# introlab/rtabmap

Measured on AMD Instinct MI355X. Metric: loop-closure candidates/sec (49k vocab, 100k signatures, 500 desc/frame), higher is better.
Workload: dtype f32; 1 GPU; SURF-64 fp32 brute-force 2-NN (49k words) + NNDR + TF-IDF likelihood (100000 signatures x 500 words, Zipf), 500 desc/frame, 1 frame/step; world_size_observed=1, collective_backend=none, parallelism=1 GPU, last_frame_top_candidate_ok=True

## Files before the change

include/lcd.h:

```cpp
#ifndef LCD_H_
#define LCD_H_

#include <stddef.h>
#include <stdint.h>

#ifdef __cplusplus
extern "C" {
#endif

#define LCD_ABI_VERSION 7

typedef struct lcd_engine lcd_engine;

enum lcd_status {
    LCD_OK = 0,
    LCD_ERR_INVALID = 1,
    LCD_ERR_HIP = 2,
    LCD_ERR_NOMEM = 3,
    LCD_ERR_STATE = 4,
    LCD_ERR_UNSUPPORTED = 5
};

enum lcd_dtype {
    LCD_F32 = 0,
// ... 79 lines not shown
} lcd_hypothesis;

#define LCD_NEW_WORD_IDS_AUTO (-1)
typedef struct lcd_frame_args {
    int32_t struct_size;
    int32_t q;
    const void* d_descriptors;
    int32_t flags;
    float nndr_ratio;
    int32_t sig_id;
    int32_t first_new_word_id;
    float N;
    int32_t exclude_recent;
    int32_t* d_word_ids;
    float* d_likelihood;
    int64_t likelihood_capacity;
    lcd_hypothesis* d_hypothesis;
    float* d_adjusted;
    float virtual_place_ratio;
    int32_t append_new_words;
    int32_t* d_first_new_word_id;
    float* d_posterior;
    struct lcd_bayes_result* d_bayes;
} lcd_frame_args;
int lcd_frame_dev(lcd_engine* h, const lcd_frame_args* args);

typedef struct lcd_frame_host_args {
    int32_t struct_size;
    int32_t q;
    const void* descriptors;
    int32_t flags;
    float nndr_ratio;
    int32_t sig_id;
    int32_t first_new_word_id;
    float N;
    int32_t append_new_words;
    int32_t* word_ids;
    float* likelihood;
    int64_t likelihood_capacity;
    int64_t* n_slots;
} lcd_frame_host_args;
int lcd_frame_host(lcd_engine* h, const lcd_frame_host_args* args);
int lcd_slot_count(const lcd_engine* h, int64_t* n_slots);

typedef struct lcd_bayes_result {
    int32_t sig_id;
    int32_t slot;
    float posterior;
    float value;
    float virtual_place;
    int32_t n_considered;
    float sum;
    int32_t reserved;
} lcd_bayes_result;
int lcd_bayes_configure(lcd_engine* h, const double* prediction_lc, int n_values, float virtual_place_prior);
int lcd_bayes_reset(lcd_engine* h);
int lcd_bayes_set_neighbors(lcd_engine* h, int n_sigs, const int32_t* sig_ids, const int64_t* offsets, const int32_t* nbr_sig_ids,
                            const int32_t* nbr_margins);
int lcd_bayes_update_dev(lcd_engine* h, const float* d_adjusted, int exclude_recent, float* d_posterior, lcd_bayes_result* d_result);
int lcd_bayes_update(lcd_engine* h, const int32_t* sig_ids, const float* adjusted, int n, lcd_bayes_result* result);
int lcd_bayes_posterior(lcd_engine* h, const int32_t* sig_ids, int n, float* out);
int lcd_knn2_dev(lcd_engine* h, const void* d_queries, int q, int32_t* d_word_ids, float* d_dist);
typedef struct lcd_shard_cand { uint64_t key; int32_t word; int32_t wslot; } lcd_shard_cand;
int lcd_shard_knn2_dev(lcd_engine* h, const void* d_descriptors, int q, lcd_shard_cand* d_cand );
int lcd_shard_frame_dev(lcd_engine* h, const void* d_descriptors, int q, int flags, float nndr_ratio, int32_t sig_id,
                        int32_t first_new_word_id , float N,
                        int rank, int world, const lcd_shard_cand* d_all_cand ,
                        int64_t total_live_rows, int32_t* d_word_ids, int64_t* d_lfix, int64_t lfix_capacity);
int lcd_finalize_dev(lcd_engine* h, int64_t* d_lfix, int64_t n, float* d_likelihood);
int lcd_slots_dev(lcd_engine* h, const int32_t** d_slot_sig, int64_t* n_slots);
int lcd_record_event(lcd_engine* h, void* event);
void* lcd_stream(lcd_engine* h);

int lcd_profile_begin(lcd_engine* h, int max_samples);
int lcd_profile_read(lcd_engine* h, float* avg_ms, int* n_samples, const char** kernel_name);
int lcd_profile_read_likelihood(lcd_engine* h, float* avg_ms, int* n_samples, const char** kernel_name);

int lcd_set_option(lcd_engine* h, const char* key, int64_t value);

int lcd_trace_push(lcd_engine* h, const char* name);
int lcd_trace_pop(lcd_engine* h);

int lcd_profile_score_work(lcd_engine* h, int64_t* out8);

typedef struct lcd_stats {
    int64_t vocab_rows, vocab_live;
    int64_t signatures, postings;
    int64_t knn_launches, likelihood_launches, rebuilds;
    int64_t buckets_sealed;
    int64_t word_slots;
    int64_t dense_words;
    int64_t frame_calls, frame_host_ns;
    int64_t bytes_device;
    int64_t knn_last_fallback_queries;
    double knn_max_err_ratio;
    int64_t clean_divergent_refs;
} lcd_stats;
int lcd_get_stats(lcd_engine* h, lcd_stats* out);

#ifdef __cplusplus
}
#endif
#endif
```

rtabmap_amd/capi.py:

```python
import ctypes as C
import os
import sys

import numpy as np

from . import build as _build

LCD_OK = 0
LCD_F32, LCD_U8 = 0, 1
LCD_Q_INCREMENTAL, LCD_Q_NEW_WORDS_COMPARED = 1, 2
LCD_NEW_WORD_IDS_AUTO = -1
STATUS = {0: "LCD_OK", 1: "LCD_ERR_INVALID", 2: "LCD_ERR_HIP", 3: "LCD_ERR_NOMEM", 4: "LCD_ERR_STATE", 5: "LCD_ERR_UNSUPPORTED"}

SYMBOLS = [
    "lcd_abi_version", "lcd_create", "lcd_destroy", "lcd_last_error", "lcd_synchronize", "lcd_pipeline_depth",
    "lcd_vocab_clear", "lcd_vocab_append", "lcd_vocab_remove", "lcd_vocab_remove_unused", "lcd_vocab_remove_unused_async", "lcd_vocab_rebuild", "lcd_vocab_count", "lcd_vocab_read",
    "lcd_knn2", "lcd_selfdist", "lcd_quantize", "lcd_find_nn",
    "lcd_sig_add", "lcd_sig_remove", "lcd_sig_add_bulk", "lcd_sig_count", "lcd_word_nrefs",
    "lcd_likelihood", "lcd_adjust_likelihood", "lcd_adjust_likelihood_dev", "lcd_frame_dev", "lcd_frame_host", "lcd_slot_count", "lcd_knn2_dev", "lcd_shard_knn2_dev", "lcd_shard_frame_dev", "lcd_finalize_dev", "lcd_slots_dev", "lcd_stream", "lcd_get_stats", "lcd_profile_begin", "lcd_profile_read", "lcd_profile_read_likelihood", "lcd_profile_score_work", "lcd_set_option", "lcd_record_event", "lcd_trace_push", "lcd_trace_pop",
    "lcd_bayes_configure", "lcd_bayes_reset", "lcd_bayes_set_neighbors", "lcd_bayes_update_dev", "lcd_bayes_update", "lcd_bayes_posterior",
]


LCD_KNN_DEFAULT, LCD_KNN_EXACT_VALU, LCD_KNN_F32_MFMA, LCD_KNN_BF16X3, LCD_KNN_F16 = 0, 1, 2, 3, 4
KNN_MODES = {None: 0, "default": 0, "valu": 1, "exact": 1, "mfma32": 2, "f32": 2, "bf16": 3, "bf16x3": 3, "f16": 4, "fp16": 4}


class LcdConfig(C.Structure):
    _fields_ = [("struct_size", C.c_int32), ("device", C.c_int32), ("dtype", C.c_int32), ("dim", C.c_int32),
                ("vocab_capacity", C.c_int64), ("sig_capacity", C.c_int64), ("max_queries", C.c_int32),
                ("knn_mode", C.c_int32), ("stream", C.c_void_p), ("pipeline", C.c_int32), ("reserved1", C.c_int32)]


class LcdHypothesis(C.Structure):
    _fields_ = [("sig_id", C.c_int32), ("slot", C.c_int32), ("likelihood", C.c_float), ("adjusted", C.c_float),
                ("virtual_place", C.c_float), ("mean", C.c_float), ("stddev", C.c_float), ("n_positive", C.c_int32)]


class LcdFrameArgs(C.Structure):
    _fields_ = [("struct_size", C.c_int32), ("q", C.c_int32), ("d_descriptors", C.c_void_p), ("flags", C.c_int32),
                ("nndr_ratio", C.c_float), ("sig_id", C.c_int32), ("first_new_word_id", C.c_int32), ("N", C.c_float),
                ("exclude_recent", C.c_int32), ("d_word_ids", C.c_void_p), ("d_likelihood", C.c_void_p),
                ("likelihood_capacity", C.c_int64), ("d_hypothesis", C.c_void_p), ("d_adjusted", C.c_void_p),
                ("virtual_place_ratio", C.c_float), ("append_new_words", C.c_int32), ("d_first_new_word_id", C.c_void_p),
                ("d_posterior", C.c_void_p), ("d_bayes", C.c_void_p)]


class LcdFrameHostArgs(C.Structure):
    _fields_ = [("struct_size", C.c_int32), ("q", C.c_int32), ("descriptors", C.c_void_p), ("flags", C.c_int32), ("nndr_ratio", C.c_float),
                ("sig_id", C.c_int32), ("first_new_word_id", C.c_int32), ("N", C.c_float), ("append_new_words", C.c_int32),
                ("word_ids", C.c_void_p), ("likelihood", C.c_void_p), ("likelihood_capacity", C.c_int64), ("n_slots", C.c_void_p)]


class LcdBayesResult(C.Structure):
    _fields_ = [("sig_id", C.c_int32), ("slot", C.c_int32), ("posterior", C.c_float), ("value", C.c_float),
                ("virtual_place", C.c_float), ("n_considered", C.c_int32), ("sum", C.c_float), ("reserved", C.c_int32)]


class LcdStats(C.Structure):
    _fields_ = [("vocab_rows", C.c_int64), ("vocab_live", C.c_int64), ("signatures", C.c_int64), ("postings", C.c_int64),
                ("knn_launches", C.c_int64), ("likelihood_launches", C.c_int64), ("rebuilds", C.c_int64),
                ("buckets_sealed", C.c_int64), ("word_slots", C.c_int64), ("dense_words", C.c_int64),
                ("frame_calls", C.c_int64), ("frame_host_ns", C.c_int64),
                ("bytes_device", C.c_int64), ("knn_last_fallback_queries", C.c_int64), ("knn_max_err_ratio", C.c_double),
                ("clean_divergent_refs", C.c_int64)]


class LcdError(RuntimeError):
    def __init__(self, status, msg):
        super().__init__("%s: %s" % (STATUS.get(status, status), msg))
        self.status = status


_lib = None


def library_path():
    return _build.OUT


def load():
    global _lib
    if _lib is not None:
        return _lib
    path = os.environ.get("LCD_LIB_PATH") or _build.build()
    if "torch" not in sys.modules and not os.environ.get("LCD_NO_TORCH_PRELOAD"):
        try:
            import torch
        except Exception:
            pass
    L = C.CDLL(path)
    vp, i32, i64, f32 = C.c_void_p, C.c_int32, C.c_int64, C.c_float
    L.lcd_abi_version.restype = C.c_int
    L.lcd_create.argtypes = [C.POINTER(LcdConfig), C.POINTER(vp)]
    L.lcd_destroy.argtypes = [vp]
    L.lcd_destroy.restype = None
    L.lcd_last_error.argtypes = [vp]
    L.lcd_last_error.restype = C.c_char_p
    L.lcd_synchronize.argtypes = [vp]
    L.lcd_pipeline_depth.argtypes = [vp]
    L.lcd_pipeline_depth.restype = C.c_int
    L.lcd_vocab_clear.argtypes = [vp]
    L.lcd_vocab_append.argtypes = [vp, vp, C.c_int, vp]
    L.lcd_vocab_remove.argtypes = [vp, vp, C.c_int]
    L.lcd_vocab_remove_unused.argtypes = [vp, vp, C.c_int, vp]
    L.lcd_vocab_remove_unused_async.argtypes = [vp]
    L.lcd_vocab_rebuild.argtypes = [vp]
    L.lcd_vocab_count.argtypes = [vp, C.POINTER(i64), C.POINTER(i64)]
    L.lcd_vocab_read.argtypes = [vp, i64, C.c_int, vp, vp]
    L.lcd_knn2.argtypes = [vp, vp, C.c_int, vp, vp]
    L.lcd_selfdist.argtypes = [vp, vp, C.c_int, vp]
    L.lcd_quantize.argtypes = [vp, vp, C.c_int, C.c_int, f32, vp, C.POINTER(i32)]
    L.lcd_find_nn.argtypes = [vp, vp, C.c_int, vp, vp, C.c_int, C.c_int, f32, vp]
    L.lcd_sig_add.argtypes = [vp, i32, vp, C.c_int, i32]
    L.lcd_sig_remove.argtypes = [vp, i32]
    L.lcd_sig_add_bulk.argtypes = [vp, C.c_int, vp, vp, vp, vp]
    L.lcd_sig_count.argtypes = [vp, C.POINTER(i64), C.POINTER(i64)]
    L.lcd_word_nrefs.argtypes = [vp, i32, C.POINTER(i32)]
    L.lcd_likelihood.argtypes = [vp, vp, C.c_int, vp, C.c_int, f32, vp]
    L.lcd_adjust_likelihood.argtypes = [vp, vp, C.c_int, f32]
    L.lcd_adjust_likelihood_dev.argtypes = [vp, vp, C.c_int, f32]
    L.lcd_frame_dev.argtypes = [vp, C.POINTER(LcdFrameArgs)]
    L.lcd_frame_host.argtypes = [vp, C.POINTER(LcdFrameHostArgs)]
    L.lcd_slot_count.argtypes = [vp, C.POINTER(C.c_int64)]
    L.lcd_knn2_dev.argtypes = [vp, vp, C.c_int, vp, vp]
    L.lcd_shard_knn2_dev.argtypes = [vp, vp, C.c_int, vp]
    L.lcd_shard_frame_dev.argtypes = [vp, vp, C.c_int, C.c_int, f32, i32, i32, f32, C.c_int, C.c_int, vp, i64, vp, vp, i64]
    L.lcd_finalize_dev.argtypes = [vp, vp, i64, vp]
    L.lcd_slots_dev.argtypes = [vp, C.POINTER(vp), C.POINTER(i64)]
    L.lcd_stream.argtypes = [vp]
    L.lcd_stream.restype = vp
    L.lcd_profile_begin.argtypes = [vp, C.c_int]
    L.lcd_profile_read.argtypes = [vp, C.POINTER(f32), C.POINTER(C.c_int), C.POINTER(C.c_char_p)]
    L.lcd_profile_read_likelihood.argtypes = [vp, C.POINTER(f32), C.POINTER(C.c_int), C.POINTER(C.c_char_p)]
    L.lcd_get_stats.argtypes = [vp, C.POINTER(LcdStats)]
    L.lcd_profile_score_work.argtypes = [vp, C.POINTER(i64)]
    L.lcd_set_option.argtypes = [vp, C.c_char_p, i64]
    L.lcd_record_event.argtypes = [vp, vp]
    L.lcd_bayes_configure.argtypes = [vp, vp, C.c_int, f32]
    L.lcd_bayes_reset.argtypes = [vp]
    L.lcd_bayes_set_neighbors.argtypes = [vp, C.c_int, vp, vp, vp, vp]
    L.lcd_bayes_update_dev.argtypes = [vp, vp, C.c_int, vp, vp]
    L.lcd_bayes_update.argtypes = [vp, vp, vp, C.c_int, vp]
    L.lcd_bayes_posterior.argtypes = [vp, vp, C.c_int, vp]
    _lib = L
    return L


def _p(a):
    return None if a is None else a.ctypes.data_as(C.c_void_p)


class Engine:

    def __init__(self, dtype, dim, device=0, vocab_capacity=0, sig_capacity=0, stream=None, knn_mode=None, pipeline=False):
        self.L = load()
        self.dtype = LCD_F32 if dtype in (LCD_F32, np.float32, "f32") else LCD_U8
        self.np_dtype = np.float32 if self.dtype == LCD_F32 else np.uint8
        self.dim = int(dim)
        if knn_mode is None:
            knn_mode = os.environ.get("LCD_PY_KNN_MODE") or None
        mode = KNN_MODES[knn_mode] if (knn_mode is None or isinstance(knn_mode, str)) else int(knn_mode)
        cfg = LcdConfig(C.sizeof(LcdConfig), device, self.dtype, self.dim, vocab_capacity, sig_capacity, 0, mode, stream,
                        1 if pipeline else 0, 0)
        h = C.c_void_p()
        rc = self.L.lcd_create(C.byref(cfg), C.byref(h))
        if rc != LCD_OK:
            raise LcdError(rc, "lcd_create failed (no gfx950 device / HIP runtime?)")
        self.h = h
        for kv in filter(None, os.environ.get("LCD_PY_OPTS", "").split(",")):
            self._ck(self.L.lcd_set_option(self.h, kv.split("=")[0].encode(), int(kv.split("=")[1])))

    def close(self):
        if getattr(self, "h", None):
            self.L.lcd_destroy(self.h)
            self.h = None

    def __del__(self):
        try:
            self.close()
        except Exception:
            pass

    def _ck(self, rc):
        if rc != LCD_OK:
            raise LcdError(rc, self.L.lcd_last_error(self.h).decode())

    def _rows(self, a):
        a = np.ascontiguousarray(a, dtype=self.np_dtype)
        if a.ndim != 2 or a.shape[1] != self.dim:
            raise ValueError("expected [n, %d] %s" % (self.dim, self.np_dtype.__name__))
        return a

    def synchronize(self):
        self._ck(self.L.lcd_synchronize(self.h))

    def pipeline_depth(self):
        return int(self.L.lcd_pipeline_depth(self.h))

    def vocab_clear(self):
        self._ck(self.L.lcd_vocab_clear(self.h))

    def vocab_append(self, rows, word_ids):
        rows = self._rows(rows)
        ids = np.ascontiguousarray(word_ids, dtype=np.int32)
        assert ids.shape[0] == rows.shape[0]
        self._ck(self.L.lcd_vocab_append(self.h, _p(rows), rows.shape[0], _p(ids)))

    def vocab_remove(self, word_ids):
        ids = np.ascontiguousarray(word_ids, dtype=np.int32)
        self._ck(self.L.lcd_vocab_remove(self.h, _p(ids), ids.shape[0]))

    def vocab_remove_unused(self, capacity=0):
        out = np.zeros(max(capacity, 1), np.int32)
        n = C.c_int32()
        self._ck(self.L.lcd_vocab_remove_unused(self.h, _p(out) if capacity else None, capacity, C.byref(n)))
        return n.value, out[: min(n.value, capacity)]

    def vocab_remove_unused_async(self):
# ... 134 lines not shown
        s = np.ascontiguousarray(sig_ids, dtype=np.int32)
        o = np.ascontiguousarray(offsets, dtype=np.int64)
        n = np.ascontiguousarray(nbr_sig_ids, dtype=np.int32)
        m = np.ascontiguousarray(nbr_margins, dtype=np.int32)
        assert o.shape[0] == s.shape[0] + 1 and n.shape[0] == m.shape[0]
        self._ck(self.L.lcd_bayes_set_neighbors(self.h, s.shape[0], _p(s), _p(o), _p(n), _p(m)))

    def bayes_neighbors_prepared(self, sig_ids, offsets, nbr_sig_ids, nbr_margins):
        assert sig_ids.dtype == np.int32 and offsets.dtype == np.int64 and nbr_sig_ids.dtype == np.int32 and nbr_margins.dtype == np.int32
        assert offsets.shape[0] == sig_ids.shape[0] + 1 and nbr_sig_ids.shape[0] == nbr_margins.shape[0]
        return (sig_ids.shape[0], _p(sig_ids), _p(offsets), _p(nbr_sig_ids), _p(nbr_margins), (sig_ids, offsets, nbr_sig_ids, nbr_margins))

    def bayes_set_neighbors_prepared(self, prep):
        rc = self.L.lcd_bayes_set_neighbors(self.h, prep[0], prep[1], prep[2], prep[3], prep[4])
        if rc != LCD_OK:
            self._ck(rc)

    def bayes_update_dev(self, d_adjusted_ptr, exclude_recent=0, d_posterior_ptr=None, d_result_ptr=None):
        self._ck(self.L.lcd_bayes_update_dev(self.h, d_adjusted_ptr, exclude_recent, d_posterior_ptr, d_result_ptr))

    def bayes_update(self, sig_ids, adjusted):
        s = np.ascontiguousarray(sig_ids, dtype=np.int32)
        a = np.ascontiguousarray(adjusted, dtype=np.float32)
        assert s.shape[0] == a.shape[0]
        r = LcdBayesResult()
        self._ck(self.L.lcd_bayes_update(self.h, _p(s), _p(a), s.shape[0], C.byref(r)))
        return r

    def bayes_posterior(self, sig_ids):
        s = np.ascontiguousarray(sig_ids, dtype=np.int32)
        out = np.zeros(s.shape[0], np.float32)
        self._ck(self.L.lcd_bayes_posterior(self.h, _p(s), s.shape[0], _p(out)))
        return out

    def knn2_dev(self, d_queries_ptr, q, d_word_ids_ptr, d_dist_ptr):
        self._ck(self.L.lcd_knn2_dev(self.h, d_queries_ptr, q, d_word_ids_ptr, d_dist_ptr))

    def shard_knn2_dev(self, d_desc_ptr, q, d_cand_ptr):
        self._ck(self.L.lcd_shard_knn2_dev(self.h, d_desc_ptr, q, d_cand_ptr))

    def shard_frame_dev(self, d_desc_ptr, q, sig_id, N, rank, world, d_all_cand_ptr, total_live_rows, d_word_ids_ptr, d_lfix_ptr,
                        lfix_capacity, incremental=True, new_words_compared=True, nndr=0.8, first_new_word_id=0):
        flags = (LCD_Q_INCREMENTAL if incremental else 0) | (LCD_Q_NEW_WORDS_COMPARED if new_words_compared else 0)
        self._ck(self.L.lcd_shard_frame_dev(self.h, d_desc_ptr, q, flags, nndr, sig_id, first_new_word_id, float(N), rank, world,
                                            d_all_cand_ptr, total_live_rows, d_word_ids_ptr, d_lfix_ptr, lfix_capacity))

    def finalize_dev(self, d_lfix_ptr, n, d_like_ptr):
        self._ck(self.L.lcd_finalize_dev(self.h, d_lfix_ptr, n, d_like_ptr))

    def slots_dev(self):
        p, n = C.c_void_p(), C.c_int64()
        self._ck(self.L.lcd_slots_dev(self.h, C.byref(p), C.byref(n)))
        return p.value, n.value

    def stream(self):
        return self.L.lcd_stream(self.h)

    def profile_begin(self, max_samples):
        self._ck(self.L.lcd_profile_begin(self.h, max_samples))

    def profile_read(self):
        ms, n, name = C.c_float(), C.c_int(), C.c_char_p()
        self._ck(self.L.lcd_profile_read(self.h, C.byref(ms), C.byref(n), C.byref(name)))
        return ms.value, n.value, (name.value or b"").decode()

    def profile_read_likelihood(self):
        ms, n, name = C.c_float(), C.c_int(), C.c_char_p()
        self._ck(self.L.lcd_profile_read_likelihood(self.h, C.byref(ms), C.byref(n), C.byref(name)))
        return ms.value, n.value, (name.value or b"").decode()

    def record_event(self, event_handle):
        self._ck(self.L.lcd_record_event(self.h, event_handle))

    def set_option(self, key, value):
        self._ck(self.L.lcd_set_option(self.h, key.encode(), int(value)))

    def profile_score_work(self):
        out = (C.c_int64 * 8)()
        self._ck(self.L.lcd_profile_score_work(self.h, out))
        keys = ["dense_row_bytes", "sparse_postings", "directory_lookups", "directory_hits", "open_log_entries", "postings",
                "unique_words", "dense_words"]
        return {k: int(v) for k, v in zip(keys, out)}

    def stats(self):
        s = LcdStats()
        self._ck(self.L.lcd_get_stats(self.h, C.byref(s)))
        return {k: getattr(s, k) for k, _ in LcdStats._fields_}
```

rtabmap_amd/csrc/engine.hip:

```cpp
#include "engine_impl.h"
#include <dlfcn.h>

#include <algorithm>
#include <chrono>
#include <cmath>
#include <cstdlib>
#include <cstring>
#include <new>
#include <numeric>
#include <unordered_map>

using namespace lcd;

static_assert(sizeof(lcd::HypothesisOut) == sizeof(lcd_hypothesis), "lcd_hypothesis is the kernel's output record");

int RowMirror::find(int32_t word_id) {
    if (rows_sorted) {
        auto it = std::lower_bound(h_row_key.begin(), h_row_key.end(), word_id);
        if (it == h_row_key.end() || *it != word_id) return -1;
        const int r = (int)(it - h_row_key.begin());
        return h_row_live[r] ? r : -1;
    }
    if (!word_row_valid) {
        word_row.clear();
// ... 1226 lines not shown
    if (n > h->tfidf.n_slots) return h->fail(LCD_ERR_INVALID, "lcd_finalize_dev: more entries than signature slots");
    LCD_HIP(h, h->tfidf.finalize((const long long*)d_lfix, (long long)n, d_likelihood));
    return LCD_OK;
    LCD_CATCH(h)
}

int lcd_slots_dev(lcd_engine* h, const int32_t** d_slot_sig, int64_t* n_slots) {
    LCD_TRY
    LCD_CHECK_HANDLE(h);
    { int rc = drain_keep_rows_lazy(h); if (rc) return rc; }
    if (d_slot_sig) *d_slot_sig = h->tfidf.slot_sig.as<int32_t>();
    if (n_slots) *n_slots = h->tfidf.n_slots;
    return LCD_OK;
    LCD_CATCH(h)
}

int lcd_profile_begin(lcd_engine* h, int max_samples) {
    LCD_TRY
    LCD_CHECK_HANDLE(h);
    LCD_DEV(h);
    if (max_samples <= 0 || max_samples > (1 << 20)) return h->fail(LCD_ERR_INVALID, "lcd_profile_begin: bad sample count");
    while ((int)h->prof_ev.size() < 2 * max_samples) {
        hipEvent_t e;
        LCD_HIP(h, hipEventCreate(&e));
        h->prof_ev.push_back(e);
        LCD_HIP(h, hipEventCreate(&e));
        h->prof_ev.push_back(e);
        LCD_HIP(h, hipEventCreate(&e));
        h->prof2_ev.push_back(e);
        LCD_HIP(h, hipEventCreate(&e));
        h->prof2_ev.push_back(e);
    }
    h->prof_n = 0;
    h->prof2_n = 0;
    h->prof_cap = max_samples;
    return LCD_OK;
    LCD_CATCH(h)
}

int lcd_profile_read(lcd_engine* h, float* avg_ms, int* n_samples, const char** kernel_name) {
    LCD_TRY
    LCD_CHECK_HANDLE(h);
    LCD_DEV(h);
    { int rc = h->sync_all(); if (rc) return rc; }
    double sum = 0.0;
    for (int i = 0; i < h->prof_n; ++i) {
        float ms = 0.0f;
        LCD_HIP(h, hipEventElapsedTime(&ms, h->prof_ev[2 * i], h->prof_ev[2 * i + 1]));
        sum += ms;
    }
    if (avg_ms) *avg_ms = h->prof_n ? (float)(sum / h->prof_n) : 0.0f;
    if (n_samples) *n_samples = h->prof_n;
    if (kernel_name) *kernel_name = h->prof_kernel;
    h->prof_cap = 0;
    return LCD_OK;
    LCD_CATCH(h)
}

int lcd_profile_read_likelihood(lcd_engine* h, float* avg_ms, int* n_samples, const char** kernel_name) {
    LCD_TRY
    LCD_CHECK_HANDLE(h);
    LCD_DEV(h);
    { int rc = h->sync_all(); if (rc) return rc; }
    double sum = 0.0;
    for (int i = 0; i < h->prof2_n; ++i) {
        float ms = 0.0f;
        LCD_HIP(h, hipEventElapsedTime(&ms, h->prof2_ev[2 * i], h->prof2_ev[2 * i + 1]));
        sum += ms;
    }
    if (avg_ms) *avg_ms = h->prof2_n ? (float)(sum / h->prof2_n) : 0.0f;
    if (n_samples) *n_samples = h->prof2_n;
    if (kernel_name) *kernel_name = h->prof2_kernel;
    h->prof_cap = 0;
    return LCD_OK;
    LCD_CATCH(h)
}

int lcd_set_option(lcd_engine* h, const char* key, int64_t value) {
    LCD_TRY
    LCD_CHECK_HANDLE(h);
    { int rc = h->drain(); if (rc) return rc; }
    if (!key) return h->fail(LCD_ERR_INVALID, "lcd_set_option: null key");
    if (!std::strcmp(key, "score_block") && (value == 256 || value == 512 || value == 1024)) { h->tfidf.score_block = (int)value; return LCD_OK; }
    if (!std::strcmp(key, "filter_units") && value >= -1 && value <= 4096) { h->filter_units = (int)value; return LCD_OK; }
    if (!std::strcmp(key, "strip_tiles") && value >= 0 && value <= 8) { h->strip_tiles = (int)value; return LCD_OK; }
    if (!std::strcmp(key, "shard_growth_first") && value >= 0 && value < (1ll << 28)) { h->shard_first = (int32_t)value; return LCD_OK; }
    if (!std::strcmp(key, "shard_growth_block") && value >= 0 && value <= (1 << 20)) { h->shard_block = (int32_t)value; return LCD_OK; }
    if (!std::strcmp(key, "shard_append") && (value == 0 || value == 1)) { h->shard_append = (int)value; return LCD_OK; }
    if (!std::strcmp(key, "profile_likelihood") && (value == 0 || value == 1)) { h->prof_likelihood = value != 0; return LCD_OK; }
    if (!std::strcmp(key, "append_split_buckets") && value >= -1 && value <= (1 << 24)) { h->popt.append_split_buckets = (int)value; return LCD_OK; }
    if (!std::strcmp(key, "cross_frame_tiles") && value >= -1 && value <= 1) { h->popt.cross_frames = value > 0 ? 1 : 0; return LCD_OK; }
    if (!std::strcmp(key, "append_from_rerank") && value >= -1 && value <= 1) { h->popt.append_from_rerank = value != 0 ? 1 : 0; return LCD_OK; }
    if (!std::strcmp(key, "roctx") && (value == 0 || value == 1)) {
        if (!value) { h->roctx_push = nullptr; h->roctx_pop = nullptr; return LCD_OK; }
        static void* lib = nullptr;
        if (!lib) lib = dlopen("libroctx64.so", RTLD_NOW | RTLD_GLOBAL);
        if (!lib) lib = dlopen("libroctx64.so.4", RTLD_NOW | RTLD_GLOBAL);
        if (!lib) lib = dlopen("/opt/rocm/lib/libroctx64.so", RTLD_NOW | RTLD_GLOBAL);
        if (!lib) return h->fail(LCD_ERR_UNSUPPORTED, "lcd_set_option(roctx): libroctx64.so not found");
        h->roctx_push = reinterpret_cast<int (*)(const char*)>(dlsym(lib, "roctxRangePushA"));
        h->roctx_pop = reinterpret_cast<int (*)()>(dlsym(lib, "roctxRangePop"));
        if (!h->roctx_push || !h->roctx_pop) { h->roctx_push = nullptr; h->roctx_pop = nullptr; return h->fail(LCD_ERR_UNSUPPORTED, "lcd_set_option(roctx): roctxRangePushA / roctxRangePop not exported"); }
        return LCD_OK;
    }
    if (!std::strcmp(key, "filter_delay") && value >= 0 && value <= 127) { h->popt.filter_delay = (int)value; return LCD_OK; }
    if (!std::strcmp(key, "shadow_rows") && value >= -1 && value <= 2) { h->popt.shadow_rows = value < 0 ? 1 : (int)value; return LCD_OK; }
    if (!std::strcmp(key, "mirror_from_b") && value >= -1 && value <= 1) { h->popt.mirror_from_b = value != 0 ? 1 : 0; return LCD_OK; }
    if (!std::strcmp(key, "next_word_id") && value >= 1 && value < (1ll << 28)) { h->mirror.next_word_id = std::max(h->mirror.next_word_id, (int32_t)value); return LCD_OK; }
    if (!std::strcmp(key, "profile_skip") && value >= 0 && value <= (1 << 20)) { h->prof_skip = (int)value; return LCD_OK; }
    if (!std::strcmp(key, "decision_straight") && value >= -1 && value <= 2) { h->popt.decision_straight = value >= 0 ? (int)value : PipeOpts().decision_straight; return LCD_OK; }
    if (!std::strcmp(key, "slots_from_rows") && value >= -1 && value <= 2) { h->popt.slots_from_rows = value >= 0 ? (int)value : PipeOpts().slots_from_rows; return LCD_OK; }
    if (!std::strcmp(key, "row_writer_wgs") && value >= -1 && value <= 256) { h->popt.row_writer_wgs = value >= 0 ? (int)value : PipeOpts().row_writer_wgs; return LCD_OK; }
    return h->fail(LCD_ERR_INVALID, "lcd_set_option: unknown key or value");
    LCD_CATCH(h)
}

int lcd_trace_push(lcd_engine* h, const char* name) {
    if (!h || !name) return LCD_ERR_INVALID;
    if (h->roctx_push) h->roctx_push(name);
    return LCD_OK;
}
int lcd_trace_pop(lcd_engine* h) {
    if (!h) return LCD_ERR_INVALID;
    if (h->roctx_pop) h->roctx_pop();
    return LCD_OK;
}

int lcd_profile_score_work(lcd_engine* h, int64_t* out8) {
    LCD_TRY
    LCD_CHECK_HANDLE(h);
    LCD_DEV(h);
    if (!out8) return h->fail(LCD_ERR_INVALID, "lcd_profile_score_work: null output");
    { int rc = h->sync_all(); if (rc) return rc; }
    LCD_HIP(h, h->tfidf.score_work(out8));
    return LCD_OK;
    LCD_CATCH(h)
}

int lcd_get_stats(lcd_engine* h, lcd_stats* out) {
    LCD_TRY
    LCD_CHECK_HANDLE(h);
    if (!out) return LCD_ERR_INVALID;
    LCD_DEV(h);
    { int rc = h->sync_all(); if (rc) return rc; }
    out->knn_last_fallback_queries = 0;
    out->knn_max_err_ratio = 0.0;
    const void* fc = h->last_fail_count ? h->last_fail_count : h->d_fail_count.p;
    if (fc) {
        int32_t n[3] = {0, 0, 0};
        int rc = download(h, n, fc, 12, h->h_out2);
        if (rc) return rc;
        out->knn_last_fallback_queries = n[0];
        float r;
        std::memcpy(&r, &n[2], 4);
        out->knn_max_err_ratio = r;
    }
    out->vocab_rows = h->n_rows; out->vocab_live = h->n_live;
    out->signatures = h->tfidf.live_sigs; out->postings = h->tfidf.postings_ub;
    out->knn_launches = h->knn_launches; out->likelihood_launches = h->likelihood_launches; out->rebuilds = h->rebuilds;
    h->tfidf.harvest_released(false);
    out->frame_calls = h->frame_calls; out->frame_host_ns = h->frame_host_ns;
    out->buckets_sealed = h->tfidf.seals;
    out->word_slots = (int64_t)h->tfidf.n_wslots - h->tfidf.ws_free_count;
    out->dense_words = h->tfidf.h_n_dense ? (int64_t)*(volatile uint32_t*)h->tfidf.h_n_dense : 0;
    out->bytes_device = h->bytes_device;
    out->clean_divergent_refs = 0;
    if (h->tfidf.q_meta.p) {
        uint32_t n = 0;
        int rc = download(h, &n, h->tfidf.q_meta.as<uint32_t>() + 8, 4, h->h_out2);
        if (rc) return rc;
        out->clean_divergent_refs = (int64_t)n;
    }
    return LCD_OK;
    LCD_CATCH(h)
}

}
```

rtabmap_amd/csrc/knn_mfma_kernels.hip:

```cpp
#include <hip/hip_ext.h>
#include "lcd_kernels.h"
#include "rowpar_body.cuh"
#include "shard_body.cuh"
#include "frame_tail_body.cuh"
#include "score_body.cuh"

#include <cstdlib>

namespace lcd {
namespace {

typedef float f32x16 __attribute__((ext_vector_type(16)));
constexpr int MF_BLOCK = 256;
constexpr int MF_WAVES = 4;
constexpr int MF_KEEP = 4;

__global__ void row_norm_kernel(const float* __restrict__ vocab, const int32_t* __restrict__ row_id, int first, int n, int dim,
                                float* __restrict__ aug, uint32_t* __restrict__ norm_max_bits) {
    const int r = first + blockIdx.x * blockDim.x + threadIdx.x;
    if (r >= first + n) return;
    float s = __int_as_float(0x7f800000);
    if (row_id[r] != 0) {
        s = 0.0f;
        const float* v = vocab + (size_t)r * dim;
// ... 1666 lines not shown
constexpr int PIPE_BLOCK = 256;

struct TailRoles { int has_resolve, has_register, n_redo, n_filter_wgs, n_q_wgs, n_sh_wgs; };
#ifdef LCD_B_TIMING
__device__ unsigned long long g_a_timing[2 * 4096];
#define A_STAMP(i) do { __builtin_amdgcn_s_barrier(); if (threadIdx.x == 0 && blockIdx.x < 4096) g_a_timing[2 * blockIdx.x + (i)] = __builtin_amdgcn_s_memrealtime(); } while (0)
#else
#define A_STAMP(i) do { } while (0)
#endif
template <bool PERSISTENT, int M>
__device__ __forceinline__ void frame_a_body(float* s_dyn, const FilterArgs& f, int px, const TailRoles& tr, const ResolveArgs& r, const FwArgs& a,
                                             const RetireArgs& ret, const QSplitArgs& qs) {
    const int bid = (int)blockIdx.x;
    const int n_front = tr.has_resolve + tr.has_register;
    A_STAMP(0);
    if (bid < tr.has_resolve) { frame_resolve_part<PIPE_BLOCK>((uint32_t*)s_dyn, r, 0, 1 + tr.n_redo); A_STAMP(1); return; }
    if (bid < n_front) { frame_register_part<PIPE_BLOCK>((uint32_t*)s_dyn, a, ret); A_STAMP(1); return; }
    const int after_strips = n_front + tr.n_filter_wgs;
    if (bid >= after_strips && bid < after_strips + tr.n_sh_wgs) {
        if constexpr (!PERSISTENT) shadow_scores_body<M>(s_dyn, bid - after_strips, f.sh_bf, f.sh_norm, f.sh_rows, f.qsplit, f.qnorm, f.nq, f.qpad, f.sh_x, f.sh_ld);
        A_STAMP(1);
        return;
    }
    const int after_filter = after_strips + tr.n_sh_wgs;
    if (bid >= after_filter && bid < after_filter + tr.n_q_wgs) { qsplit_body(qs, bid - after_filter); A_STAMP(1); return; }
    if (bid >= after_filter + tr.n_q_wgs) { frame_resolve_part<PIPE_BLOCK>((uint32_t*)s_dyn, r, bid - after_filter - tr.n_q_wgs + 1, 1 + tr.n_redo); A_STAMP(1); return; }
    for (int i = 0; i < f.delay; ++i) __builtin_amdgcn_s_sleep(1);
    if constexpr (PERSISTENT)
        knn_bf16_filter_body_p<M>(s_dyn, bid - n_front, f.vocab_bf, f.row_norm, f.n_rows, f.queries, f.nq, f.qpad, f.tiles_per_block, f.n_blocks, px, f.pk,
                               f.pl, f.sd, f.n_lo);
    else
        knn_bf16_filter_body_q<M>(s_dyn, bid - n_front, f.vocab_bf, f.row_norm, f.n_rows, f.qsplit, f.qnorm, f.nq, f.qpad, f.tiles_per_block, f.n_blocks, f.pk,
                               f.pl, f.sd, f.n_lo);
    A_STAMP(1);
}
template <int M>
__global__ __launch_bounds__(PIPE_BLOCK, 2) void frame_a_kernel(FilterArgs f, TailRoles tr, ResolveArgs r, FwArgs a, RetireArgs ret, QSplitArgs qs) {
    extern __shared__ __attribute__((aligned(16))) float s_dyn_a[];
    frame_a_body<false, M>(s_dyn_a, f, 0, tr, r, a, ret, qs);
}
template <int M>
__global__ __launch_bounds__(PIPE_BLOCK) void frame_a_kernel_p(FilterArgs f, int px, TailRoles tr, ResolveArgs r, FwArgs a, RetireArgs ret, QSplitArgs qs) {
    extern __shared__ __attribute__((aligned(16))) float s_dyn_ap[];
    frame_a_body<true, M>(s_dyn_ap, f, px, tr, r, a, ret, qs);
}
#ifdef LCD_B_TIMING
__device__ unsigned long long g_b_timing[2 * 4096];
#define B_STAMP(i) do { __builtin_amdgcn_s_barrier(); if (threadIdx.x == 0 && blockIdx.x < 4096) g_b_timing[2 * blockIdx.x + (i)] = __builtin_amdgcn_s_memrealtime(); } while (0)
#else
#define B_STAMP(i) do { } while (0)
#endif
constexpr int PIPE_B_BLOCK = 512;
constexpr uint32_t PIPE_B_STAGE_ROWS = 160;
constexpr int APPEND_SPLIT_BUCKETS = 1024;
static_assert(PIPE_B_BLOCK == 2 * MF_BLOCK, "the re-rank halves");
template <bool WITH_APPEND>
__global__ __launch_bounds__(PIPE_B_BLOCK, 6) void frame_b_kernel(RerankArgs k, int n_rerank_wgs, ScoreArgs A, int n_score_wgs, AppendRowsArgs app, int n_wr) {
    int bid = (int)blockIdx.x;
    B_STAMP(0);
    const bool rows_only = !WITH_APPEND && n_wr > 0 && bid >= n_rerank_wgs && bid < n_rerank_wgs + n_wr;
    const int wr_index = bid - n_rerank_wgs;
    if (!WITH_APPEND && n_wr > 0 && bid >= n_rerank_wgs + n_wr) bid -= n_wr;
    if (WITH_APPEND && bid >= n_rerank_wgs + n_score_wgs) {
        extern __shared__ __attribute__((aligned(16))) float s_dyn_b2[];
        append_rows_body<PIPE_B_BLOCK>(app, bid - n_rerank_wgs - n_score_wgs, app.ap.lds_bytes >= 1024 ? s_dyn_b2 : nullptr, (app.ap.lds_bytes / 256) & ~3);
        B_STAMP(1);
        return;
    }
    if (bid < n_rerank_wgs || rows_only) {
        const int pair = rows_only ? 0 : (bid & 7) * (n_rerank_wgs >> 3) + (bid >> 3);
        if (2 * pair >= k.nq) return;
        extern __shared__ __attribute__((aligned(16))) float s_dyn_b[];
        const bool wr_any = !WITH_APPEND && app.ap.enabled && app.ap.defer_rows;
        knn_mfma_rerank_body<64, BF_KEEP, false, true, 2>(2 * pair, k.pk, k.pl, k.n_blocks, k.nq, k.vocab, k.queries, k.row_id, k.norm_max_bits, k.out_row,
                                                          k.out_word, k.out_dist, k.fail_list, k.fail_count, k.cb, k.n_lo, k.n_hi, k.plan_rows,
                                                          s_dyn_b, k.stage_rows, k.f16, k.pend_desc, k.pend_list, k.pend_first_id, k.cross, k.cross_ld
                                                          , app, wr_any && (n_wr == 0 || rows_only), rows_only ? wr_index : pair, n_wr > 0 ? n_wr : (k.nq + 1) / 2
                                                          , rows_only, k.sh_mask, k.sh_q, k.sh_x, k.sh_ld);
        B_STAMP(1);
        return;
    }
    const int g = bid - n_rerank_wgs;
    if (g < A.n_closed_pad) {
        const int b = (g & 7) * (A.n_closed_pad >> 3) + (g >> 3);
        if (b < A.n_closed) score_sealed_body<PIPE_B_BLOCK>(A, b);
    } else score_open_body<PIPE_B_BLOCK>(A, g - A.n_closed_pad);
    B_STAMP(1);
}

__global__ __launch_bounds__(PIPE_B_BLOCK) void append_rows_kernel(AppendRowsArgs app) {
    extern __shared__ __attribute__((aligned(16))) float s_dyn_ar[];
    append_rows_body<PIPE_B_BLOCK>(app, (int)blockIdx.x, app.ap.lds_bytes >= 1024 ? s_dyn_ar : nullptr, (app.ap.lds_bytes / 256) & ~3);
}

__global__ __launch_bounds__(MF_BLOCK) void knn_rowpar_kernel(RowparArgs a, int32_t* __restrict__ fail_count) {
    rowpar_body<64, MF_BLOCK>(a, (int)blockIdx.x, (int)gridDim.x, fail_count);
}
__global__ __launch_bounds__(256) void shard_merge_bits_kernel(ShardMergeJob mj, CandBits cb) {
    const int lane = threadIdx.x & 63;
    const int qi = (int)blockIdx.x * 4 + (int)(threadIdx.x >> 6);
    if (qi >= cb.nq) return;
    const ShardMerged m = shard_merge_one(mj.cand, mj.world, mj.rank, cb.nq, qi, mj.by_word);
    const bool v0 = m.dist[0] >= 0.0f && m.word[0] != 0, v1 = m.dist[1] >= 0.0f && m.word[1] != 0;
    const float thr = (cb.have_index && v0 && v1) ? m.dist[1] : __int_as_float(0x7f800000);
    if (lane == 0) {
#pragma unroll
        for (int j = 0; j < 2; ++j) { mj.out_word[2 * qi + j] = m.word[j]; mj.out_dist[2 * qi + j] = m.dist[j]; mj.out_wslot[2 * qi + j] = m.wslot[j]; }
    }
    cand_bits_row(cb, qi, thr, lane, 64);
}
__global__ __launch_bounds__(MF_BLOCK) void knn_rowpar_pack_kernel(RowparArgs a, int32_t* __restrict__ fail_count, ShardPackArgs p) {
    const int st = rowpar_body<64, MF_BLOCK>(a, (int)blockIdx.x, (int)gridDim.x, fail_count);
    if (st == 0) {
        for (int i = (int)blockIdx.x * MF_BLOCK + (int)threadIdx.x; i < p.q2; i += (int)gridDim.x * MF_BLOCK) shard_pack_one(p, i);
    } else if (st == 2) {
        asm volatile("s_waitcnt vmcnt(0)" ::: "memory");
        __syncthreads();
        __builtin_amdgcn_fence(__ATOMIC_ACQUIRE, "agent");
        for (int i = (int)threadIdx.x; i < p.q2; i += MF_BLOCK) shard_pack_one(p, i);
        if (threadIdx.x < 4 && threadIdx.x != 2) fail_count[threadIdx.x] = 0;
    }
}

}
}
#ifdef LCD_B_TIMING
extern "C" int lcd_debug_a_timing(unsigned long long* out, int n_words) {
    if (hipDeviceSynchronize() != hipSuccess) return -1;
    return (int)hipMemcpyFromSymbol(out, HIP_SYMBOL(lcd::g_a_timing), (size_t)n_words * 8);
}
extern "C" int lcd_debug_rr_timing(unsigned long long* out, int n_words) {
    if (hipDeviceSynchronize() != hipSuccess) return -1;
    return (int)hipMemcpyFromSymbol(out, HIP_SYMBOL(lcd::g_rr_timing), (size_t)n_words * 8);
}
extern "C" int lcd_debug_b_timing(unsigned long long* out, int n_words) {
    if (hipDeviceSynchronize() != hipSuccess) return -1;
    return (int)hipMemcpyFromSymbol(out, HIP_SYMBOL(lcd::g_b_timing), (size_t)n_words * 8);
}
#endif
#ifdef LCD_MFMA_TIMING
extern "C" int lcd_debug_mfma_timing(unsigned long long* out, int n_words) {
    if (hipDeviceSynchronize() != hipSuccess) return -1;
    return (int)hipMemcpyFromSymbol(out, HIP_SYMBOL(lcd::g_mf_timing), (size_t)n_words * 8);
}
extern "C" int lcd_debug_mfma_timing2(unsigned long long* out, int n_words) {
    if (hipDeviceSynchronize() != hipSuccess) return -1;
    return (int)hipMemcpyFromSymbol(out, HIP_SYMBOL(lcd::g_mf_timing2), (size_t)n_words * 8);
}
#endif
namespace lcd {

bool knn_mfma_supported(int dtype, int dim) { return dtype == 0 && dim == 64; }

static int mfma_ng() {
    return 4;
}

MfmaPlan knn_mfma_plan(int q, int n_rows) {
    MfmaPlan p;
    p.q = q;
    p.qpad = (q + 63) / 64 * 64;
    p.n_rows = n_rows;
    const int n_tiles = (n_rows + 31) / 32;
    const int qw = mfma_ng() * 32;
    const int qgroups = (q + qw - 1) / qw;
    int nb = ((mfma_ng() == 2 ? 512 : 256) + qgroups - 1) / qgroups;
    if (nb > (n_tiles + MF_WAVES - 1) / MF_WAVES) nb = (n_tiles + MF_WAVES - 1) / MF_WAVES;
    if (nb < 1) nb = 1;
// ... 234 lines not shown
    MfmaPlan p;
    p.q = 0; p.qpad = 0; p.n_rows = 0; p.tiles_per_block = 1; p.n_blocks = 0;
    if (kp) {
        const PipeKnn& k = *kp;
        p = k.plan;
        uint64_t* pk = (uint64_t*)k.partial;
        uint32_t* pl = (uint32_t*)(pk + (size_t)(p.n_blocks > 0 ? p.n_blocks : 1) * BF_KEEP * p.qpad);
        if (p.n_shadow > 0 && k.sh_bf && k.sh_norm && k.sh_rows > 0 && k.sh_x) { f.sh_bf = (const float*)k.sh_bf; f.sh_norm = k.sh_norm; f.sh_rows = k.sh_rows; f.sh_x = k.sh_x; f.sh_ld = k.sh_ld; }
        f.vocab_bf = (const float*)k.vocab_bf; f.row_norm = k.row_norm; f.n_rows = p.n_rows; f.queries = (const float*)k.queries; f.nq = p.q; f.qpad = p.qpad;
        f.tiles_per_block = p.tiles_per_block; f.n_blocks = p.n_blocks; f.pk = pk; f.pl = pl; f.n_lo = k.n_lo;
        f.qsplit = (const uint4*)k.qsplit; f.qnorm = k.qnorm;
        if (k.cb.selfdist) {
            f.sd.queries = (const float*)k.queries; f.sd.nq = p.q; f.sd.out = const_cast<float*>(k.cb.selfdist); f.sd.ld = k.cb.ld; f.sd.n_tiles = f.sd.n_self = selfdist_tiles(p.q);
        }
        if (opt.cross_frames && k.cross && k.cross_cols && k.cross_ncols > 0 && p.q > 0) {
            f.sd.queries = (const float*)k.queries; f.sd.nq = p.q;
            f.sd.other = (const float*)k.cross_cols; f.sd.n_other = k.cross_ncols; f.sd.xout = k.cross; f.sd.xld = k.cross_ld;
            f.sd.n_tiles += ((p.q + 63) / 64) * ((k.cross_ncols + 63) / 64);
        }
    }
    f.delay = opt.filter_delay;
    const int px = p.q > 0 ? bf16_persistent_px(p) : 0;
    if (px == 0 && p.q > 0 && (!f.qsplit || !f.qnorm)) return hipErrorInvalidValue;
    if (p.n_shadow > 0 && (px > 0 || !f.sh_x)) return hipErrorInvalidValue;
    TailRoles tr;
    tr.n_filter_wgs = p.q > 0 ? f.sd.n_tiles + (px > 0 ? px : p.n_blocks) * ((p.q + BF_QB - 1) / BF_QB) : 0;
    tr.n_sh_wgs = (p.q > 0 && p.n_shadow > 0) ? ((f.sh_rows + 31) / 32) * ((p.q + BF_QB - 1) / BF_QB) : 0;
    tr.has_resolve = resolve ? 1 : 0; tr.has_register = reg ? 1 : 0; tr.n_redo = resolve ? resolve->n_redo : 0;
    QSplitArgs qs{};
    if (qsp) { qs = *qsp; qs.n_wgs = std::min((qs.qpad * 8 + PIPE_BLOCK - 1) / PIPE_BLOCK, 32); if (qs.n_wgs < 1) qs.n_wgs = 1; }
    tr.n_q_wgs = qsp ? qs.n_wgs : 0;
    const int grid = tr.n_filter_wgs + tr.n_sh_wgs + tr.has_resolve + tr.has_register + tr.n_redo + tr.n_q_wgs;
    if (grid == 0) return hipSuccess;
    const size_t lds = px > 0 ? BF_LDS_BYTES_P : BF_LDS_BYTES_Q;
    if ((resolve && resolve->shmem_resolve > lds) || (reg && reg->shmem + (size_t)reg->a.n * 4 > lds)) return hipErrorInvalidValue;
    ResolveArgs r{}; FwArgs a{}; RetireArgs ret{};
    if (resolve) { r = resolve->r; r.ap.lds_bytes = (int)lds; }
    if (reg) { a = reg->a; ret = reg->ret; }
    const bool timed = ev_begin != nullptr && ev_end != nullptr;
    const bool f16 = kp ? p.f16 != 0 : opt.f16 != 0;
    if (px > 0) {
        static const hipError_t attrp0 = hipFuncSetAttribute(reinterpret_cast<const void*>(&frame_a_kernel_p<0>),
                                                             hipFuncAttributeMaxDynamicSharedMemorySize, (int)BF_LDS_BYTES_P);
        static const hipError_t attrp1 = hipFuncSetAttribute(reinterpret_cast<const void*>(&frame_a_kernel_p<1>),
                                                             hipFuncAttributeMaxDynamicSharedMemorySize, (int)BF_LDS_BYTES_P);
        (void)attrp0; (void)attrp1;
        if (f16) {
            if (timed) hipExtLaunchKernelGGL(frame_a_kernel_p<1>, dim3(grid), dim3(PIPE_BLOCK), (uint32_t)BF_LDS_BYTES_P, s, ev_begin, ev_end, 0u, f, px, tr, r, a, ret, qs);
            else frame_a_kernel_p<1><<<grid, PIPE_BLOCK, BF_LDS_BYTES_P, s>>>(f, px, tr, r, a, ret, qs);
        } else {
            if (timed) hipExtLaunchKernelGGL(frame_a_kernel_p<0>, dim3(grid), dim3(PIPE_BLOCK), (uint32_t)BF_LDS_BYTES_P, s, ev_begin, ev_end, 0u, f, px, tr, r, a, ret, qs);
            else frame_a_kernel_p<0><<<grid, PIPE_BLOCK, BF_LDS_BYTES_P, s>>>(f, px, tr, r, a, ret, qs);
        }
    } else if (f16) {
        if (timed) hipExtLaunchKernelGGL(frame_a_kernel<1>, dim3(grid), dim3(PIPE_BLOCK), (uint32_t)BF_LDS_BYTES_Q, s, ev_begin, ev_end, 0u, f, tr, r, a, ret, qs);
        else frame_a_kernel<1><<<grid, PIPE_BLOCK, BF_LDS_BYTES_Q, s>>>(f, tr, r, a, ret, qs);
    } else {
        if (timed) hipExtLaunchKernelGGL(frame_a_kernel<0>, dim3(grid), dim3(PIPE_BLOCK), (uint32_t)BF_LDS_BYTES_Q, s, ev_begin, ev_end, 0u, f, tr, r, a, ret, qs);
        else frame_a_kernel<0><<<grid, PIPE_BLOCK, BF_LDS_BYTES_Q, s>>>(f, tr, r, a, ret, qs);
    }
    return hipGetLastError();
}


hipError_t launch_frame_b(const PipeKnn* k, const ScoreArgs* score, int score_wgs, hipStream_t s, hipEvent_t ev_begin, hipEvent_t ev_end,
                          const AppendRowsArgs* app, const PipeOpts& opt) {
    RerankArgs rk{};
    int n_rerank = 0;
    if (k) {
        const MfmaPlan& p = k->plan;
        uint64_t* pk = (uint64_t*)k->partial;
        rk.pk = pk; rk.pl = (uint32_t*)(pk + (size_t)(p.n_blocks > 0 ? p.n_blocks : 1) * BF_KEEP * p.qpad);
        rk.n_blocks = p.n_blocks; rk.nq = p.q; rk.vocab = (const float*)k->vocab; rk.queries = (const float*)k->queries; rk.row_id = k->row_id;
        rk.norm_max_bits = k->norm_max_bits; rk.out_row = k->out_row; rk.out_word = k->out_word; rk.out_dist = k->out_dist;
        rk.fail_list = k->fail_list; rk.fail_count = k->fail_count; rk.cb = k->cb; rk.n_lo = k->n_lo; rk.n_hi = k->n_hi; rk.plan_rows = p.n_rows; rk.f16 = p.f16;
        n_rerank = ((p.q + 1) / 2 + 7) & ~7;
    }
    ScoreArgs A{};
    if (score) A = *score; else score_wgs = 0;
    AppendRowsArgs ar{};
    int n_app = 0;
    if (app && app->ap.enabled && app->ap.defer_rows) { ar = *app; n_app = ar.n_wgs = APPEND_ROW_WGS; }
    if (n_rerank + score_wgs + n_app == 0) return hipSuccess;
    const uint32_t dyn = ((k && k->n_hi) || n_app) ? PIPE_B_STAGE_ROWS * 256u + 512u : 0u;
    rk.stage_rows = (dyn && k && k->n_hi) ? (int)PIPE_B_STAGE_ROWS : 0;
    ar.ap.lds_bytes = (int)(PIPE_B_STAGE_ROWS * 256u);
    if (k && n_app) { rk.pend_desc = ar.ap.descriptors; rk.pend_list = ar.ap.list_out; rk.pend_first_id = ar.ap.first_id; }
    if (k && n_app && opt.cross_frames && k->cross && k->cross_cols == (const void*)ar.ap.descriptors) { rk.cross = k->cross; rk.cross_ld = k->cross_ld; }
    const bool writers = opt.append_from_rerank == 0;
    if (!writers && k && n_app > 0 && k->n_hi && k->plan.q > 0 && rk.stage_rows >= 4) n_app = 0;
    const bool shadow = k && k->plan.n_shadow > 0 && k->sh_mask && k->sh_x && k->sh_q > 0 && app && app->ap.enabled && app->ap.defer_rows && rk.pend_desc && !rk.cross;
    if (k && k->plan.n_shadow > 0 && !shadow) return hipErrorInvalidValue;
    if (shadow) { rk.sh_mask = k->sh_mask; rk.sh_q = k->sh_q; rk.sh_x = k->sh_x; rk.sh_ld = k->sh_ld; }
    const int n_wr = (!writers && n_app == 0 && k && app && app->ap.enabled && app->ap.defer_rows && k->n_hi && k->plan.q > 0 && rk.stage_rows >= 4 && !rk.cross &&
                      (opt.row_writer_wgs > 0 || shadow)) ? (opt.row_writer_wgs > 0 ? opt.row_writer_wgs : 16) : 0;
    if (shadow && n_wr == 0) return hipErrorInvalidValue;
    const bool split = n_app > 0 && score && score->n_closed >= (opt.append_split_buckets >= 0 ? opt.append_split_buckets : APPEND_SPLIT_BUCKETS);
    if (split || n_app == 0) {
        if (n_rerank + score_wgs > 0) {
            if (ev_begin != nullptr && ev_end != nullptr)
                hipExtLaunchKernelGGL(frame_b_kernel<false>, dim3(n_rerank + n_wr + score_wgs), dim3(PIPE_B_BLOCK), dyn, s, ev_begin, ev_end, 0u, rk, n_rerank, A, score_wgs, ar, n_wr);
            else frame_b_kernel<false><<<n_rerank + n_wr + score_wgs, PIPE_B_BLOCK, dyn, s>>>(rk, n_rerank, A, score_wgs, ar, n_wr);
        }
        if (n_app > 0) append_rows_kernel<<<n_app, PIPE_B_BLOCK, PIPE_B_STAGE_ROWS * 256u, s>>>(ar);
        return hipGetLastError();
    }
    if (ev_begin != nullptr && ev_end != nullptr)
        hipExtLaunchKernelGGL(frame_b_kernel<true>, dim3(n_rerank + score_wgs + n_app), dim3(PIPE_B_BLOCK), dyn, s, ev_begin, ev_end, 0u, rk, n_rerank, A, score_wgs, ar, 0);
    else frame_b_kernel<true><<<n_rerank + score_wgs + n_app, PIPE_B_BLOCK, dyn, s>>>(rk, n_rerank, A, score_wgs, ar, 0);
    return hipGetLastError();
}

}

extern "C" int lcd_debug_frame_plan(int q, int n_rows, int new_words_compared, int* out) {
    if (q <= 0 || n_rows <= 0 || !out) return -1;
    const int tiles = new_words_compared ? lcd::knn_selfdist_wgs(q) : 0;
    const lcd::MfmaPlan p = lcd::knn_bf16_plan_pipelined(q, n_rows, tiles, -1);
    out[0] = p.tiles_per_block; out[1] = p.n_blocks; out[2] = lcd::bf16_persistent_px(p); out[3] = tiles; out[4] = (q + lcd::BF_QB - 1) / lcd::BF_QB;
    return 0;
}

#ifdef LCD_SCORE_TIMING
extern "C" int lcd_debug_score_timing_pipe(unsigned long long* out, int n_words) {
    if (hipDeviceSynchronize() != hipSuccess) return -1;
    return (int)hipMemcpyFromSymbol(out, HIP_SYMBOL(lcd::g_score_timing), (size_t)n_words * 8);
}
#endif

#ifdef LCD_TAIL_TIMING
extern "C" int lcd_debug_tail_timing_pipe(unsigned long long* out) {
    if (hipDeviceSynchronize() != hipSuccess) return -1;
    if (hipMemcpyFromSymbol(out, HIP_SYMBOL(lcd::g_tail_timing), 64) != hipSuccess) return -2;
    if (hipMemcpyFromSymbol(out + 8, HIP_SYMBOL(lcd::g_resolve_timing), 64) != hipSuccess) return -3;
    return (int)hipMemcpyFromSymbol(out + 16, HIP_SYMBOL(lcd::g_sweep_timing), 256);
}
#endif
```

rtabmap_amd/csrc/score_body.cuh:

```cuda
#pragma once
#include "frame_tail_body.cuh"

namespace lcd {
namespace {

#ifdef LCD_SCORE_TIMING
__device__ unsigned long long g_score_timing[1024 * 8];
#define SC_STAMP(i) do { __syncthreads(); if (threadIdx.x == 0 && blockIdx.x < 1024) g_score_timing[blockIdx.x * 8 + (i)] = __builtin_amdgcn_s_memrealtime(); } while (0)
#else
#define SC_STAMP(i) do { } while (0)
#endif



template <int SCB>
__device__ __forceinline__ void score_segments(const uint32_t* __restrict__ sp_ent, unsigned long long* acc, uint32_t start, uint32_t len, int32_t idf) {
    const int ln = threadIdx.x & 63;
    uint32_t incl = len;
#pragma unroll
    for (int off = 1; off < 64; off <<= 1) { const uint32_t y = __shfl_up(incl, off, 64); if (ln >= off) incl += y; }
    const uint32_t Tw = __shfl(incl, 63, 64);
    for (uint32_t t0 = 0; t0 < Tw; t0 += 128) {
        uint32_t e[2]; int32_t f[2]; bool ok[2];
#pragma unroll
        for (int u = 0; u < 2; ++u) {
            const uint32_t t = t0 + (uint32_t)(u * 64 + ln);
            int pos = 0;
#pragma unroll
            for (int step = 32; step >= 1; step >>= 1) { const uint32_t v = __shfl(incl, pos + step - 1, 64); if (v <= t) pos += step; }
            if (pos > 63) pos = 63;
            const uint32_t i_o = __shfl(incl, pos, 64), l_o = __shfl(len, pos, 64), s_o = __shfl(start, pos, 64);
            f[u] = __shfl(idf, pos, 64);
            ok[u] = t < Tw;
            e[u] = ok[u] ? gload(sp_ent + s_o + (t - (i_o - l_o))) : 0u;
        }
#pragma unroll
        for (int u = 0; u < 2; ++u) {
            if (!ok[u]) continue;
            const long long term = (long long)(int)(e[u] & TF_CNT_MASK) * (long long)f[u];
            atomicAdd(&acc[e[u] >> TF_CNT_BITS], (unsigned long long)term);
        }
    }
}

template <int SCB>
__device__ __forceinline__ void score_sealed_body(const ScoreArgs& A, int b) {
    __shared__ unsigned long long acc[TF_R];
    const int tid = threadIdx.x;
    const BucketDev B = A.tab[b];
    const long long first_slot = (long long)b * TF_R;
    const bool live = B.state == 1u;
    SC_STAMP(0);
    constexpr int NWV = SCB / 64;
#ifndef LCD_SCORE_DR4
#define LCD_SCORE_DR4 16
#endif
    constexpr int DR = NWV == 4 ? LCD_SCORE_DR4 : (128 / NWV > 16 ? 16 : 128 / NWV);
    constexpr int KW = SCB >= 512 ? 1 : 512 / SCB;
    constexpr int NI = TF_R / SCB > 0 ? TF_R / SCB : 1;
    const int wv = __builtin_amdgcn_readfirstlane(tid >> 6), ln = tid & 63;
    const uint32_t D = live ? A.bkt_D[b] : 0u;
    const uint32_t BW = live ? B.W : 0u;
    const uint32_t flags = A.bkt_flags[b];
    const int U = (int)A.q_meta[0];
    const int Ud = (int)A.q_meta[1];
    static_assert(KW * SCB <= TF_MAX_WORDS && DR * NWV <= TF_MAX_WORDS, "the unconditional list reads stay inside the buffers");
    uint32_t w[KW]; int32_t idf[KW], did[KW]; bool look[KW];
#pragma unroll
    for (int u = 0; u < KW; ++u) {
        const int k = tid + u * SCB;
        w[u] = A.q_w[k]; idf[u] = A.q_idf[k]; did[u] = A.q_did[k];
    }
    int32_t dj[DR], fj[DR];
#pragma unroll
    for (int u = 0; u < DR; ++u) {
        const int j = wv + u * NWV;
        dj[u] = A.qd_did[j];
        fj[u] = A.qd_idf[j];
    }
#pragma unroll
    for (int u = 0; u < KW; ++u) { if (tid + u * SCB >= U) { w[u] = 0; idf[u] = 0; did[u] = -1; } }
#pragma unroll
    for (int u = 0; u < DR; ++u) { if (wv + u * NWV >= Ud) { dj[u] = -1; fj[u] = 0; } }
    uint32_t ni_v[NI];
#pragma unroll
    for (int u = 0; u < NI; ++u) { const int i = tid + u * SCB; ni_v[u] = i < TF_R ? A.slot_ni[first_slot + i] : 0u; }
    uint4 r0[KW], r1[KW];
#pragma unroll
    for (int u = 0; u < KW; ++u) {
        const bool dense_here = did[u] >= 0 && (uint32_t)did[u] < D;
        look[u] = idf[u] != 0 && w[u] < BW && (!dense_here || (flags & 1u));
        r0[u] = make_uint4(0u, 0u, 0u, 0u); r1[u] = r0[u];
        if (look[u]) {
            const uint4* rec = reinterpret_cast<const uint4*>(A.dir2 + ((size_t)(w[u] >> 5) * A.dir2_stride + (uint32_t)b) * TF_DIR2_DWORDS);
            r0[u] = gload4(rec); r1[u] = gload4(rec + 1);
        }
    }
    uint32_t c[DR];
#pragma unroll
    for (int u = 0; u < DR; ++u) c[u] = (dj[u] >= 0 && (uint32_t)dj[u] < D) ? gload((const uint32_t*)(B.dense + (size_t)dj[u] * TF_R + 4 * ln)) : 0u;
    uint32_t start[KW], len[KW];
#pragma unroll
    for (int u = 0; u < KW; ++u) {
        start[u] = 0; len[u] = 0;
        if (!look[u]) continue;
        const uint32_t f[6] = {r0[u].z, r0[u].w, r1[u].x, r1[u].y, r1[u].z, r1[u].w};
        const uint32_t p = w[u] & 31u, pd = p / 6u, ps = 5u * (p % 6u);
        if (!(r0[u].y & TF_DIR2_SAT)) {
            uint32_t before = 0;
#pragma unroll
            for (uint32_t d = 0; d < 6u; ++d) {
                const uint32_t x = d < pd ? f[d] : (d == pd ? (f[d] & ((1u << ps) - 1u)) : 0u);
                before += dir2_sum6(x);
            }
            uint32_t fd = f[0];
#pragma unroll
            for (uint32_t d = 1; d < 6u; ++d) fd = d == pd ? f[d] : fd;
            len[u] = (fd >> ps) & 31u;
            start[u] = r0[u].x + before;
        } else {
            const uint2 blk = gload2(B.dirb + (w[u] >> 5));
            const uint32_t bit = 1u << p;
            if (blk.x & bit) {
                const uint32_t r = blk.y + (uint32_t)__popc(blk.x & (bit - 1u));
                const uint32_t s0 = gload(B.sp_off + r), s1 = gload(B.sp_off + r + 1);
                start[u] = s0; len[u] = s1 - s0;
            }
        }
    }
    long long a0 = 0, a1 = 0, a2 = 0, a3 = 0;
#pragma unroll
    for (int u = 0; u < DR; ++u) {
        const long long f64 = (long long)fj[u];
        a0 += (long long)(int)(c[u] & 255u) * f64;
        a1 += (long long)(int)((c[u] >> 8) & 255u) * f64;
        a2 += (long long)(int)((c[u] >> 16) & 255u) * f64;
        a3 += (long long)(int)(c[u] >> 24) * f64;
    }
    for (int j0 = wv + DR * NWV; j0 < Ud; j0 += DR * NWV) {
#pragma unroll
        for (int u = 0; u < DR; ++u) {
            const int j = j0 + u * NWV;
            dj[u] = j < Ud ? A.qd_did[j] : -1;
            fj[u] = j < Ud ? A.qd_idf[j] : 0;
        }
#pragma unroll
        for (int u = 0; u < DR; ++u) c[u] = (dj[u] >= 0 && (uint32_t)dj[u] < D) ? gload((const uint32_t*)(B.dense + (size_t)dj[u] * TF_R + 4 * ln)) : 0u;
#pragma unroll
        for (int u = 0; u < DR; ++u) {
            const long long f64 = (long long)fj[u];
            a0 += (long long)(int)(c[u] & 255u) * f64;
            a1 += (long long)(int)((c[u] >> 8) & 255u) * f64;
            a2 += (long long)(int)((c[u] >> 16) & 255u) * f64;
            a3 += (long long)(int)(c[u] >> 24) * f64;
        }
    }
    for (int i = tid; i < TF_R; i += SCB) acc[i] = 0ull;
    __syncthreads();
    SC_STAMP(1);
    {
        const int ln4 = ln * 4;
        if (a0) atomicAdd(&acc[ln4 + 0], (unsigned long long)a0);
        if (a1) atomicAdd(&acc[ln4 + 1], (unsigned long long)a1);
        if (a2) atomicAdd(&acc[ln4 + 2], (unsigned long long)a2);
        if (a3) atomicAdd(&acc[ln4 + 3], (unsigned long long)a3);
    }
    SC_STAMP(2);
#pragma unroll
    for (int u = 0; u < KW; ++u) score_segments<SCB>(B.sp_ent, acc, start[u], len[u], idf[u]);
    for (int k0 = KW * SCB; k0 < U; k0 += SCB) {
        const int k = k0 + tid;
        uint32_t st2 = 0, ln2 = 0; int32_t idf2 = 0;
        if (k < U) {
            const uint32_t w2 = A.q_w[k];
            idf2 = A.q_idf[k];
            const int32_t d2 = A.q_did[k];
            const bool dh = d2 >= 0 && (uint32_t)d2 < D;
            if (idf2 != 0 && w2 < BW && (!dh || (flags & 1u))) {
                const uint2 bk = gload2(B.dirb + (w2 >> 5));
                const uint32_t bit = 1u << (w2 & 31);
                if (bk.x & bit) {
                    const uint32_t r = bk.y + (uint32_t)__popc(bk.x & (bit - 1u));
                    st2 = gload(B.sp_off + r);
                    ln2 = gload(B.sp_off + r + 1) - st2;
                }
            }
        }
        score_segments<SCB>(B.sp_ent, acc, st2, ln2, idf2);
    }
    __syncthreads();
    SC_STAMP(3);
#pragma unroll
    for (int u = 0; u < NI; ++u) {
        const int i = tid + u * SCB;
        if (i >= TF_R) continue;
        const long long v = (long long)acc[i];
        if (A.out_like) A.out_like[first_slot + i] = fixed_to_like(v, ni_v[u]);
        else A.out_fix[first_slot + i] = ni_v[u] ? v : 0;
    }
}

template <int SCB>
__device__ __forceinline__ void score_open_body(const ScoreArgs& A, int ob) {
    const int wv = threadIdx.x >> 6, ln = threadIdx.x & 63;
    const int sl = ob * (SCB / 64) + wv;
    if (sl >= A.n_open_slots) return;
    const BucketDev B = A.tab[A.n_closed];
    const long long slot = (long long)A.n_closed * TF_R + sl;
    const uint32_t begin = A.slot_begin[slot], cnt = A.slot_cnt[slot], ni = A.slot_ni[slot];
    long long acc = 0;
    if (ni != 0u) {
        for (uint32_t e0 = 0; e0 < cnt; e0 += 4 * 64) {
            uint32_t w[4], pc[4]; uint2 t[4];
#pragma unroll
            for (int u = 0; u < 4; ++u) {
                const uint32_t e = e0 + u * 64 + ln;
                w[u] = e < cnt ? gload(B.coo_w + begin + e) : 0xFFFFFFFFu;
                pc[u] = e < cnt ? gload(B.coo_pc + begin + e) : 0u;
            }
#pragma unroll
            for (int u = 0; u < 4; ++u) t[u] = A.idf_tab[w[u] != 0xFFFFFFFFu ? w[u] : 0u];
#pragma unroll
            for (int u = 0; u < 4; ++u)
                if (w[u] != 0xFFFFFFFFu && t[u].x == A.stamp) acc += (long long)(int)(pc[u] & TF_CNT_MASK) * (long long)(int32_t)t[u].y;
        }
    }
    int lo = (int)(uint32_t)acc, hi = (int)(acc >> 32);
#pragma unroll
    for (int off = 32; off > 0; off >>= 1) {
        const int olo = __shfl_xor(lo, off, 64), ohi = __shfl_xor(hi, off, 64);
        const long long s = (((long long)hi << 32) | (uint32_t)lo) + (((long long)ohi << 32) | (uint32_t)olo);
        lo = (int)(uint32_t)s; hi = (int)(s >> 32);
    }
    if (ln == 0) {
        const long long v = ((long long)hi << 32) | (uint32_t)lo;
        if (A.out_like) A.out_like[slot] = fixed_to_like(v, ni);
        else A.out_fix[slot] = ni ? v : 0;
    }
}


}
}
```

rtabmap_amd/csrc/tfidf.h:

```cpp
#pragma once
#include <hip/hip_runtime.h>
#include <stdint.h>
#include <map>
#include <string>
#include <unordered_map>
#include <vector>

#include "bayes.h"
#include "devbuf.h"
#include "lcd_kernels.h"

namespace lcd {

constexpr int TF_R = 256;
constexpr int TF_CNT_BITS = 22;
constexpr uint32_t TF_CNT_MASK = (1u << TF_CNT_BITS) - 1;
constexpr int TF_MAX_WORDS = 8192;
constexpr int TF_IDF_SHIFT = 26;
constexpr int TF_DENSE_T = 32;
constexpr int TF_DENSE_MAX = 4096;
constexpr int TF_DIR2_DWORDS = 8;
constexpr uint32_t TF_DIR2_SAT = 1u << 31;
__host__ __device__ inline uint32_t dir2_sum6(uint32_t x) {
    const uint32_t t = (x & 0x01F07C1Fu) + ((x >> 5) & 0x01F07C1Fu);
    return (t & 0x3FFu) + ((t >> 10) & 0x3FFu) + (t >> 20);
}

struct BucketDev {
    const uint32_t* coo_w;
    const uint32_t* coo_pc;
    const uint8_t* dense;
    const uint2* dirb;
    const uint32_t* sp_off;
    const uint32_t* sp_ent;
    uint32_t W;
    uint32_t D_alloc;
    uint32_t state;
    uint32_t pad;
};

struct SealJob {
    int bucket;
    const uint32_t* coo_w; const uint32_t* coo_pc; const uint32_t* ne;
    uint8_t* dense; uint32_t D_alloc;
    uint2* dirb; uint32_t* sp_off; uint32_t* sp_ent;
    uint32_t* dir2; uint32_t dir2_stride;
    uint32_t* cntw;
    uint32_t* tile_sums;
    uint32_t W;
    uint32_t ent_cap;
};

struct Bucket {
    int state = 0;
    int n_slots = 0;
    int live = 0;
    int64_t ub_entries = 0;
    DevBuf coo_w, coo_pc, sealed;
    size_t off_dirb = 0, off_spoff = 0, off_spent = 0;
    uint32_t W = 0, D_alloc = 0;
};

struct AppendArgs {
    int enabled = 0;
    const float* descriptors = nullptr;
    int row_dwords = 0;
    int is_f32_64 = 0;
    int f16 = 0;
    uint32_t* vocab = nullptr; int32_t* row_id = nullptr; int32_t* row_wslot = nullptr;
    uint32_t* wrow = nullptr;
    float* row_norm = nullptr; uint32_t* norm_max_bits = nullptr; uint32_t* vocab_bf = nullptr;
    const int32_t* cnt_in = nullptr; int32_t* cnt_out = nullptr;
    int32_t* log_slot = nullptr;
    int32_t first_id = 0;
    int32_t* first_out = nullptr;
    long long capacity = 0;
    int lds_bytes = 0;
    int defer_rows = 0;
    uint32_t* list_out = nullptr;
    unsigned long long* host_mirror = nullptr;
    uint32_t tag = 0;
    uint32_t* mask_out = nullptr;
    int mirror_later = 0;
};
struct ShardAppendJob {
    AppendArgs ap; WsRuns new_ws; const int32_t* codes = nullptr; int q = 0, rank = 0, world = 1; int32_t own_first = 0, own_block = 0;
};

struct AppendRowsArgs { AppendArgs ap; WsRuns new_ws; int n_wgs = 0; };
constexpr int APPEND_ROW_WGS = 8;

struct ResolveArgs {
    int q, flags; float nndr; int have_index;
    const int32_t* knn_word; const float* knn_dist; const float* selfdist; int ld; const uint32_t* cand_bits; int bw;
    int32_t* out_word; int32_t* out_n_new; const int32_t* knn_row; const int32_t* row_wslot; int32_t* out_wslot;
    const uint2* cand_list; const int32_t* cand_cnt;
    int straight = 0;
    int slots_are_rows = 0;
    WsRuns new_ws;
    int32_t* fail_count;
    RowparArgs rp;
    AppendArgs ap;
};

struct FwArgs {
    const int32_t* src; int n;
    const int32_t* xlate; long long xlate_n;
    int H; int do_register; int want_q;
    int32_t sig_id; long long slot; uint32_t slot_local; uint32_t ni; float N; uint32_t stamp;
    uint32_t* nw; const int32_t* did;
    uint32_t* coo_w; uint32_t* coo_pc; uint32_t* ne_counter;
    int32_t* slot_sig; uint32_t* slot_ni; uint32_t* slot_begin; uint32_t* slot_cnt;
    uint32_t* q_w; int32_t* q_idf; int32_t* q_did; int32_t* qd_did; int32_t* qd_idf; uint32_t* q_meta; uint2* idf_tab;
    WsRuns new_ws;
    const int32_t* row_wslot;
    const uint32_t* wrow;
};
struct RetireArgs { long long slot[4]; const uint32_t* coo_w[4]; int n; };
struct ScoreArgs {
    const BucketDev* tab; const uint32_t* bkt_D; const uint32_t* bkt_flags;
    const uint32_t* dir2; uint32_t dir2_stride;
    int n_closed;
    int n_closed_pad;
    int n_open_slots; int wcap;
    const uint32_t* q_w; const int32_t* q_idf; const int32_t* q_did; const int32_t* qd_did; const int32_t* qd_idf; const uint32_t* q_meta;
    const uint32_t* slot_ni; const uint32_t* slot_begin; const uint32_t* slot_cnt;
    const uint2* idf_tab; uint32_t stamp;
    float* out_like; long long* out_fix;
};
struct TailLaunch {
    ResolveArgs r; FwArgs a; RetireArgs ret;
    int n_redo = 0;
    size_t shmem = 0;
    size_t shmem_resolve = 0;
};
struct PipeKnn {
    MfmaPlan plan;
    const void* vocab; const void* vocab_bf; const float* row_norm; const uint32_t* norm_max_bits; const int32_t* row_id; const void* queries;
    void* partial; int32_t* out_row; int32_t* out_word; float* out_dist; int32_t* fail_list; int32_t* fail_count;
    CandBits cb;
    const void* qsplit = nullptr;
    const float* qnorm = nullptr;
    const int32_t* n_lo = nullptr;
    const int32_t* n_hi = nullptr;
    const void* sh_bf = nullptr; const float* sh_norm = nullptr; int sh_rows = 0;
    const uint32_t* sh_mask = nullptr; int sh_q = 0;
    float* sh_x = nullptr; int sh_ld = 0;
    float* cross = nullptr;
    int cross_ld = 0;
    const void* cross_cols = nullptr; int cross_ncols = 0;
};
struct QSplitArgs { const float* queries; int nq, qpad; uint4* qsplit; float* qnorm; int n_wgs; int f16 = 0;
                    uint32_t* shadow_bf = nullptr; float* shadow_norm = nullptr;
                    uint32_t* norm_max_bits = nullptr;
};
size_t knn_qsplit_bytes(int q);
int pipe_block_size();
int pipe_b_block_size();
#ifndef LCD_REDO_WGS_MAX
#define LCD_REDO_WGS_MAX 32
#endif
constexpr int REDO_WGS_MAX = LCD_REDO_WGS_MAX;
void resolve_launch_info(const ResolveArgs& r, int block, int* n_redo, size_t* shmem);
struct PipeOpts {
    int f16 = 0;
    int cross_frames = 0;
    int append_from_rerank = 1;
    int append_split_buckets = -1;
    int filter_delay = 0;
    int shadow_rows = 1;
    int mirror_from_b = 1;
    int slots_from_rows = 1;
    int decision_straight = 1;
    int row_writer_wgs = 16;
};
hipError_t launch_frame_a(const PipeKnn* k, const QSplitArgs* qs, const TailLaunch* resolve, const TailLaunch* reg, hipStream_t s,
                          hipEvent_t ev_begin = nullptr, hipEvent_t ev_end = nullptr, const PipeOpts& opt = PipeOpts());
hipError_t launch_frame_b(const PipeKnn* k, const ScoreArgs* score, int score_wgs, hipStream_t s, hipEvent_t ev_begin = nullptr,
                          hipEvent_t ev_end = nullptr, const AppendRowsArgs* app = nullptr, const PipeOpts& opt = PipeOpts());

struct BufPool {
    std::vector<DevBuf> free_list;
    hipError_t get(size_t bytes, DevBuf* out, int64_t* total);
    void put(DevBuf* b);
    void destroy(int64_t* total);
};

struct Tfidf {
    hipStream_t stream = nullptr;
    int64_t* bytes_device = nullptr;
    DevBuf slot_sig, slot_ni, slot_begin, slot_cnt;
    DevBuf nw, did;
    DevBuf wrow;
    DevBuf idf_tab;
    uint32_t stamp = 0;
    std::vector<int32_t> id2ws;
    DevBuf d_id2ws;
    int64_t d_id2ws_n = 0;
    std::vector<int32_t> id2ws_dirty;
    std::map<int32_t, int32_t> ws_free;
    int64_t ws_free_count = 0;
    struct PinBlock { void* p = nullptr; size_t cap = 0; hipEvent_t ev = nullptr; };
    std::vector<PinBlock> pin_free;
    struct ReleaseBatch { std::vector<int32_t> ws, ids; PinBlock blk; const uint8_t* ok = nullptr; bool recheck = false; };
    std::vector<ReleaseBatch> releasing;
    std::vector<int32_t> held_ws, held_ids;
    std::vector<int32_t> ghost_ws;
    uint32_t flushes = 0;
    hipError_t flush_held();
    struct Reservation { int32_t first_id = 0, n = 0; WsRuns runs; } resv;
    DevBuf bkt_tab, bkt_ne, bkt_D, bkt_flags;
    std::vector<Bucket> buckets;
    int score_block = 512;
    int q_n_ub = 0;
    BufPool pool;
    DevBuf dir2;
    uint32_t dir2_blocks = 0, dir2_stride = 0, dir2_hint_blocks = 0, dir2_hint_stride = 0;
    hipError_t ensure_dir2(uint32_t blocks, uint32_t buckets_needed);
    DevBuf n_dense;
    uint32_t* h_n_dense = nullptr;
    DevBuf seal_cntw, seal_tiles;
    DevBuf q_w, q_idf, q_did, qd_did, qd_idf, q_meta;
    DevBuf d_stage;
    DevBuf d_pairs;
    PinBuf h_stage;
    std::unordered_map<int32_t, int64_t> sig_slot;
    int32_t n_wslots = 0;
    int64_t n_slots = 0, live_sigs = 0;
    int64_t postings_ub = 0;
    int64_t seals = 0;
    std::string err;

    hipError_t init(hipStream_t s, int64_t* bytes, int64_t sig_capacity, int64_t vocab_capacity);
    void destroy();
    hipError_t wslot_of(int32_t word_id, bool create, int32_t* out);
    hipError_t sync_id2ws();
    hipError_t release_words(const int32_t* word_ids, int n);
    hipError_t release_wslots(const std::vector<int32_t>& ws, const std::vector<int32_t>* ids = nullptr, bool recheck = false);
    hipError_t rows_take_keys(const int32_t* d_ws, int n, int64_t first_row);
    hipError_t rows_drop_keys(const int32_t* d_row_wslot, const int32_t* d_rows, int n);
    hipError_t rows_clear();
    hipError_t rows_unlog_keys(const int32_t* d_pairs, int n);
    void forget_word(int32_t word_id, int32_t ws);
    void free_wslot(int32_t w);
    void free_wslot_run(int32_t start, int32_t len);
    int32_t take_wslot();
    void harvest_released(bool wait);
    hipError_t reserve_new_words(int32_t first_id, int n, WsRuns* runs, bool may_flush = true);
    void adopt_key(int32_t word_id, int32_t ws);
    hipError_t flush_held_if_due() { return held_ws.size() >= 16384 ? flush_held() : hipSuccess; }
    hipError_t register_dev(int32_t sig_id, const int32_t* d_wslots, int n, int32_t ni, float N, const ResolveArgs* resolve = nullptr,
                            bool ids_given = false , TailLaunch* defer = nullptr,
                            const WsRuns* new_ws = nullptr, const ShardAppendJob* shard_app = nullptr);
    hipError_t query_dev(const int32_t* d_wslots, int n, float N, const ResolveArgs* resolve = nullptr, bool ids_given = false,
                         TailLaunch* defer = nullptr, const WsRuns* new_ws = nullptr, const ShardAppendJob* shard_app = nullptr);
    hipError_t register_bulk(int n_sigs, const int32_t* sig_ids, const int64_t* offsets, const int32_t* ni, const int32_t* d_ids,
                             int64_t total_ids, int max_n);
    hipError_t flush_retire();
    std::vector<int64_t> pending_retire;
    hipEvent_t prof_b = nullptr, prof_e = nullptr;
    hipError_t score(float* d_likelihood);
    hipError_t score_work(int64_t out[8]);
    hipError_t score_fix(long long* lfix);
    hipError_t finalize(const long long* lfix_src, long long n, float* d_likelihood);
    hipError_t retire(int32_t sig_id);
    hipError_t seal_batch(const std::vector<int>& bucket_ids, bool bulk);
    hipError_t ensure_slots(int64_t n);
    hipError_t ensure_wslots(int32_t n);
    hipError_t ensure_buckets(int n);
    hipError_t set_bucket(int b);
    hipError_t new_bucket();
    hipError_t launch_score(float* d_likelihood, long long* lfix);
    hipError_t score_args(float* d_likelihood, long long* lfix, int block, ScoreArgs* out, int* n_wgs);
};

hipError_t launch_gather_f32(const float* dense, const int64_t* slots, int n, float* out, hipStream_t s);
hipError_t launch_shard_append(const AppendArgs& ap, const WsRuns& new_ws, const int32_t* codes, int q, int rank, int world, int32_t own_first,
                               int32_t own_block, hipStream_t s);


}
```

rtabmap_amd/csrc/tfidf.hip:

```cpp
#include "tfidf.h"
#include "frame_tail_body.cuh"
#include "score_body.cuh"

#include <algorithm>
#include <cmath>
#include <cstdlib>
#include <cstring>
#include <iterator>

namespace lcd {
namespace {

#ifndef LCD_FW_BLOCK
#define LCD_FW_BLOCK 1024
#endif
constexpr int FW_BLOCK = LCD_FW_BLOCK;
constexpr int BR_BLOCK = 256;
constexpr int SEAL_BLOCK = 256;
constexpr int SEAL_TILE = SEAL_BLOCK * 32;

template <int NT>
__device__ __forceinline__ uint32_t block_exclusive_scan(uint32_t* data, int n, uint32_t* scratch) {
    constexpr int NW = NT / 64;
    const int tid = threadIdx.x, lane = tid & 63, wv = tid >> 6;
    const int per = (n + NT - 1) / NT;
    const int lo = min(tid * per, n), hi = min(lo + per, n);
    uint32_t sum = 0;
    for (int i = lo; i < hi; ++i) sum += data[i];
    uint32_t x = sum;
#pragma unroll
    for (int off = 1; off < 64; off <<= 1) { const uint32_t y = __shfl_up(x, off, 64); if (lane >= off) x += y; }
    if (lane == 63) scratch[wv] = x;
    __syncthreads();
    if (wv == 0) {
        const uint32_t t = lane < NW ? scratch[lane] : 0u;
        uint32_t s = t;
#pragma unroll
        for (int off = 1; off < 64; off <<= 1) { const uint32_t y = __shfl_up(s, off, 64); if (lane >= off) s += y; }
        if (lane < NW) scratch[lane] = s - t;
        if (lane == NW - 1) scratch[NW] = s;
    }
    __syncthreads();
    uint32_t run = scratch[wv] + x - sum;
    const uint32_t total = scratch[NW];
    for (int i = lo; i < hi; ++i) { const uint32_t v = data[i]; data[i] = run; run += v; }
    __syncthreads();
    return total;
}

__global__ __launch_bounds__(FW_BLOCK) void frame_words_kernel(FwArgs a, RetireArgs retire) {
    extern __shared__ uint32_t fw_dyn_smem[];
    retire_body(retire, a.slot_begin, a.slot_cnt, a.nw, a.slot_ni, a.slot_sig);
    __syncthreads();
    frame_words_body<FW_BLOCK, true>(fw_dyn_smem, a);
}

__global__ __launch_bounds__(FW_BLOCK) void frame_tail_kernel(ResolveArgs r, FwArgs a, RetireArgs retire) {
    extern __shared__ uint32_t ft_dyn_smem[];
    frame_tail_body<FW_BLOCK>(ft_dyn_smem, r, a, retire, (int)blockIdx.x, (int)gridDim.x);
}

__global__ __launch_bounds__(BR_BLOCK) void bulk_register_kernel(const int32_t* __restrict__ ids, const long long* __restrict__ offsets,
                                                                 const int32_t* __restrict__ sig_ids, const int32_t* __restrict__ ni,
                                                                 long long slot0, const int32_t* __restrict__ xlate, long long xlate_n,
                                                                 const BucketDev* __restrict__ tab, uint32_t* __restrict__ bkt_ne,
                                                                 uint32_t* __restrict__ nw, int32_t* __restrict__ slot_sig,
                                                                 uint32_t* __restrict__ slot_ni, uint32_t* __restrict__ slot_begin,
                                                                 uint32_t* __restrict__ slot_cnt) {
    extern __shared__ uint32_t br_dyn_smem[];
    const long long s = blockIdx.x;
    const long long o0 = offsets[s] - offsets[0], o1 = offsets[s + 1] - offsets[0];
    const int n = (int)(o1 - o0);
    int H = 64;
    while (H < 2 * n) H <<= 1;
    const long long slot = slot0 + s;
    const int b = (int)(slot / TF_R);
    FwArgs a;
    a.src = ids + o0; a.n = n; a.xlate = xlate; a.xlate_n = xlate_n; a.H = H; a.do_register = 1; a.want_q = 0;
    a.sig_id = sig_ids[s]; a.slot = slot; a.slot_local = (uint32_t)(slot % TF_R); a.ni = ni ? (uint32_t)ni[s] : (uint32_t)n;
    a.N = 0.0f; a.stamp = 0u; a.nw = nw; a.did = nullptr;
    a.coo_w = const_cast<uint32_t*>(tab[b].coo_w); a.coo_pc = const_cast<uint32_t*>(tab[b].coo_pc); a.ne_counter = bkt_ne + b;
    a.slot_sig = slot_sig; a.slot_ni = slot_ni; a.slot_begin = slot_begin; a.slot_cnt = slot_cnt;
    a.q_w = nullptr; a.q_idf = nullptr; a.q_did = nullptr; a.qd_did = nullptr; a.qd_idf = nullptr; a.q_meta = nullptr; a.idf_tab = nullptr;
    a.wrow = nullptr; a.row_wslot = nullptr;
    frame_words_body<BR_BLOCK, false>(br_dyn_smem, a);
}

template <int SCB>
__global__ __launch_bounds__(SCB) void score_kernel(ScoreArgs A) {
    const int g = (int)blockIdx.x;
    if (g < A.n_closed_pad) {
        const int b = (g & 7) * (A.n_closed_pad >> 3) + (g >> 3);
        if (b < A.n_closed) score_sealed_body<SCB>(A, b);
    } else score_open_body<SCB>(A, g - A.n_closed_pad);
}

__global__ __launch_bounds__(256) void score_work_kernel(ScoreArgs A, const uint32_t* __restrict__ nw, unsigned long long* __restrict__ cnt) {
    const int b = blockIdx.x, tid = threadIdx.x;
    const int U = (int)A.q_meta[0], Ud = (int)A.q_meta[1];
    unsigned long long c0 = 0, c1 = 0, c2 = 0, c3 = 0, c4 = 0, c5 = 0;
    if (b < A.n_closed) {
        const BucketDev B = A.tab[b];
        if (B.state != 1u) return;
        const uint32_t D = A.bkt_D[b], flags = A.bkt_flags[b];
        for (int j = tid; j < Ud; j += 256) if ((uint32_t)A.qd_did[j] < D) c0 += TF_R;
        for (int k = tid; k < U; k += 256) {
            const uint32_t w = A.q_w[k];
            const int32_t d = A.q_did[k];
            const bool dense_here = d >= 0 && (uint32_t)d < D;
            if (A.q_idf[k] != 0 && w < B.W && (!dense_here || (flags & 1u))) {
                c2 += 1;
                const uint2 blk = B.dirb[w >> 5];
                const uint32_t bit = 1u << (w & 31);
                if (blk.x & bit) {
                    const uint32_t r = blk.y + (uint32_t)__popc(blk.x & (bit - 1u));
                    c1 += B.sp_off[r + 1] - B.sp_off[r];
                    c3 += 1;
                }
            }
        }
    } else {
        for (int sl = tid; sl < A.n_open_slots; sl += 256) {
            const long long slot = (long long)A.n_closed * TF_R + sl;
            if (A.slot_ni[slot] != 0u) c4 += A.slot_cnt[slot];
        }
        for (int k = tid; k < U; k += 256) if (A.q_idf[k] != 0) c5 += nw[A.q_w[k]];
        if (tid == 0) { atomicAdd(&cnt[6], (unsigned long long)U); atomicAdd(&cnt[7], (unsigned long long)Ud); }
    }
    if (c0) atomicAdd(&cnt[0], c0);
    if (c1) atomicAdd(&cnt[1], c1);
    if (c2) atomicAdd(&cnt[2], c2);
    if (c3) atomicAdd(&cnt[3], c3);
    if (c4) atomicAdd(&cnt[4], c4);
    if (c5) atomicAdd(&cnt[5], c5);
}

__global__ void finalize_kernel(const long long* __restrict__ lfix, long long n, const uint32_t* __restrict__ slot_ni, float* __restrict__ out) {
    const long long i = (long long)blockIdx.x * blockDim.x + threadIdx.x;
    if (i < n) out[i] = fixed_to_like(lfix[i], slot_ni[i]);
}
__global__ void gather_f32_kernel(const float* __restrict__ dense, const long long* __restrict__ slots, int n, float* __restrict__ out) {
    const int i = blockIdx.x * blockDim.x + threadIdx.x;
    if (i < n) { const long long s = slots[i]; out[i] = s >= 0 ? dense[s] : 0.0f; }
}

#define SEAL_JOB() const SealJob J = jobs ? jobs[blockIdx.y] : job1

__global__ __launch_bounds__(SEAL_BLOCK) void seal_count_kernel(const SealJob* __restrict__ jobs, SealJob job1) {
    SEAL_JOB();
    const uint32_t ne = min(J.ne[0], J.ent_cap);
    for (uint32_t e = blockIdx.x * SEAL_BLOCK + threadIdx.x; e < ne; e += gridDim.x * SEAL_BLOCK) atomicAdd(&J.cntw[J.coo_w[e]], 1u);
}
__global__ __launch_bounds__(SEAL_BLOCK) void seal_densify_kernel(const SealJob* __restrict__ jobs, SealJob job1, int32_t* __restrict__ did,
                                                                  uint32_t* __restrict__ n_dense) {
    SEAL_JOB();
    for (uint32_t w = blockIdx.x * SEAL_BLOCK + threadIdx.x; w < J.W; w += gridDim.x * SEAL_BLOCK) {
        if (J.cntw[w] < (uint32_t)TF_DENSE_T || did[w] != -1) continue;
        if (__hip_atomic_load(n_dense, __ATOMIC_RELAXED, __HIP_MEMORY_SCOPE_AGENT) >= (uint32_t)TF_DENSE_MAX) continue;
        if (atomicCAS(&did[w], -1, -2) != -1) continue;
        const uint32_t id = atomicAdd(n_dense, 1u);
        did[w] = id < (uint32_t)TF_DENSE_MAX ? (int32_t)id : -1;
    }
}
__global__ __launch_bounds__(SEAL_BLOCK) void seal_classify_kernel(const SealJob* __restrict__ jobs, SealJob job1, const int32_t* __restrict__ did,
                                                                   const uint32_t* __restrict__ n_dense, uint32_t* __restrict__ bkt_D,
                                                                   uint32_t* __restrict__ bkt_flags, uint32_t* __restrict__ h_n_dense) {
    SEAL_JOB();
    const uint32_t nd = min(n_dense[0], (uint32_t)TF_DENSE_MAX);
    const uint32_t D = min(nd, J.D_alloc);
    if (blockIdx.x == 0 && threadIdx.x == 0) { bkt_D[J.bucket] = D; if (h_n_dense && blockIdx.y == 0) h_n_dense[0] = nd; }
    const uint32_t ne = min(J.ne[0], J.ent_cap);
    for (uint32_t e = blockIdx.x * SEAL_BLOCK + threadIdx.x; e < ne; e += gridDim.x * SEAL_BLOCK) {
        const uint32_t w = J.coo_w[e], pc = J.coo_pc[e];
        const int32_t d = did[w];
        if (d < 0 || (uint32_t)d >= D) continue;
        const uint32_t cnt = pc & TF_CNT_MASK, sl = pc >> TF_CNT_BITS;
        J.dense[(size_t)d * TF_R + sl] = (uint8_t)min(cnt, 255u);
        if (cnt <= 255u) atomicSub(&J.cntw[w], 1u);
        else atomicOr(&bkt_flags[J.bucket], 1u);
    }
}
__global__ __launch_bounds__(SEAL_BLOCK) void seal_tile_kernel(const SealJob* __restrict__ jobs, SealJob job1) {
    SEAL_JOB();
    __shared__ uint32_t s_p[SEAL_BLOCK / 64], s_a[SEAL_BLOCK / 64];
    const uint32_t w0 = (blockIdx.x * SEAL_BLOCK + threadIdx.x) * 32u;
    uint32_t p = 0, a = 0;
    for (uint32_t i = 0; i < 32u && w0 + i < J.W; ++i) { const uint32_t c = J.cntw[w0 + i]; p += c ? 1u : 0u; a += c; }
#pragma unroll
    for (int off = 32; off > 0; off >>= 1) { p += __shfl_xor(p, off, 64); a += __shfl_xor(a, off, 64); }
    if ((threadIdx.x & 63) == 0) { s_p[threadIdx.x >> 6] = p; s_a[threadIdx.x >> 6] = a; }
    __syncthreads();
    if (threadIdx.x == 0) {
        uint32_t tp = 0, ta = 0;
        for (int i = 0; i < SEAL_BLOCK / 64; ++i) { tp += s_p[i]; ta += s_a[i]; }
        J.tile_sums[2 * blockIdx.x] = tp; J.tile_sums[2 * blockIdx.x + 1] = ta;
    }
}
__global__ __launch_bounds__(SEAL_BLOCK) void seal_scan_kernel(const SealJob* __restrict__ jobs, SealJob job1) {
    SEAL_JOB();
    __shared__ uint32_t s_p[SEAL_BLOCK], s_a[SEAL_BLOCK], scratch[SEAL_BLOCK / 64 + 1];
    uint32_t base_p = 0, base_a = 0;
    for (uint32_t t = 0; t < blockIdx.x; ++t) { base_p += J.tile_sums[2 * t]; base_a += J.tile_sums[2 * t + 1]; }
    const uint32_t blk = blockIdx.x * SEAL_BLOCK + threadIdx.x;
    const uint32_t w0 = blk * 32u;
    uint32_t bits = 0, p = 0, a = 0;
    uint32_t c[32];
#pragma unroll
    for (uint32_t i = 0; i < 32u; ++i) {
        c[i] = (w0 + i < J.W) ? J.cntw[w0 + i] : 0u;
        if (c[i]) { bits |= 1u << i; p += 1u; }
        a += c[i];
    }
    s_p[threadIdx.x] = p; s_a[threadIdx.x] = a;
    __syncthreads();
    const uint32_t tot_p = block_exclusive_scan<SEAL_BLOCK>(s_p, SEAL_BLOCK, scratch);
    const uint32_t tot_a = block_exclusive_scan<SEAL_BLOCK>(s_a, SEAL_BLOCK, scratch);
    uint32_t rp = base_p + s_p[threadIdx.x], ra = base_a + s_a[threadIdx.x];
    if (w0 < J.W) {
        J.dirb[blk] = make_uint2(bits, rp);
        if (J.dir2) {
            uint32_t f[6] = {0u, 0u, 0u, 0u, 0u, 0u};
            bool sat = false;
#pragma unroll
            for (uint32_t i = 0; i < 32u; ++i) { sat = sat || c[i] > 30u; f[i / 6] |= (c[i] > 30u ? 31u : c[i]) << (5u * (i % 6)); }
            uint4* rec = reinterpret_cast<uint4*>(J.dir2 + ((size_t)blk * J.dir2_stride + (uint32_t)J.bucket) * TF_DIR2_DWORDS);
            rec[0] = make_uint4(ra, rp | (sat ? TF_DIR2_SAT : 0u), f[0], f[1]);
            rec[1] = make_uint4(f[2], f[3], f[4], f[5]);
        }
    }
#pragma unroll
    for (uint32_t i = 0; i < 32u; ++i) if (c[i]) { J.sp_off[rp++] = ra; ra += c[i]; }
    if (blockIdx.x == gridDim.x - 1 && threadIdx.x == 0) J.sp_off[base_p + tot_p] = base_a + tot_a;
}
__global__ __launch_bounds__(SEAL_BLOCK) void seal_scatter_kernel(const SealJob* __restrict__ jobs, SealJob job1, const int32_t* __restrict__ did,
                                                                  const uint32_t* __restrict__ bkt_D) {
    SEAL_JOB();
    const uint32_t D = bkt_D[J.bucket];
    const uint32_t ne = min(J.ne[0], J.ent_cap);
    for (uint32_t e = blockIdx.x * SEAL_BLOCK + threadIdx.x; e < ne; e += gridDim.x * SEAL_BLOCK) {
        const uint32_t w = J.coo_w[e];
        uint32_t pc = J.coo_pc[e];
        const int32_t d = did[w];
        if (d >= 0 && (uint32_t)d < D) {
            const uint32_t cnt = pc & TF_CNT_MASK;
            if (cnt <= 255u) continue;
            pc = (pc & ~TF_CNT_MASK) | (cnt - 255u);
        }
        const uint2 blk = J.dirb[w >> 5];
        const uint32_t r = blk.y + (uint32_t)__popc(blk.x & ((1u << (w & 31)) - 1u));
        const uint32_t pos = J.sp_off[r] + atomicSub(&J.cntw[w], 1u) - 1u;
        J.sp_ent[pos] = pc;
    }
}

__global__ void set_bucket_kernel(BucketDev* tab, int b, BucketDev v) { tab[b] = v; }

__global__ void retire_kernel(long long slot, const uint32_t* __restrict__ coo_w, const uint32_t* __restrict__ slot_begin,
                              const uint32_t* __restrict__ slot_cnt, uint32_t* __restrict__ nw, uint32_t* __restrict__ slot_ni,
                              int32_t* __restrict__ slot_sig) {
    const uint32_t begin = slot_begin[slot], cnt = slot_cnt[slot];
    for (uint32_t k = threadIdx.x; k < cnt; k += blockDim.x) atomicSub(&nw[coo_w[begin + k]], 1u);
    if (threadIdx.x == 0) { slot_ni[slot] = 0u; slot_sig[slot] = 0; }
}

__global__ void wslot_release_kernel(const int32_t* __restrict__ ws, int n, const uint32_t* __restrict__ nw, const uint32_t* __restrict__ wrow,
                                     int32_t* __restrict__ did, uint2* __restrict__ idf_tab, uint8_t* __restrict__ ok) {
    const int i = blockIdx.x * blockDim.x + threadIdx.x;
    if (i >= n) return;
    const int32_t w = ws[i];
    const bool is_row = wrow[w] != 0u;
    const bool free_now = !is_row && nw[w] == 0u;
    if (free_now) { did[w] = -1; idf_tab[w] = make_uint2(0u, 0u); }
    ok[i] = free_now ? 1 : (is_row ? 2 : 0);
}
__global__ void wrow_set_kernel(const int32_t* __restrict__ ws, int n, long long first_row, uint32_t* __restrict__ wrow) {
    const int i = blockIdx.x * blockDim.x + threadIdx.x;
    if (i < n && ws[i] >= 0) wrow[ws[i]] = (uint32_t)(first_row + i) + 1u;
}
__global__ void wrow_unlog_kernel(const int32_t* __restrict__ pairs, int n, uint32_t* __restrict__ wrow) {
    const int i = blockIdx.x * blockDim.x + threadIdx.x;
    if (i >= n) return;
    const int32_t w = pairs[2 * i + 1];
    if (w >= 0 && wrow[w] == 0xFFFFFFFFu) wrow[w] = 0u;
}
__global__ void wrow_clear_kernel(const int32_t* __restrict__ row_wslot, const int32_t* __restrict__ rows, int n, uint32_t* __restrict__ wrow) {
    const int i = blockIdx.x * blockDim.x + threadIdx.x;
    if (i >= n) return;
    const int32_t w = row_wslot[rows[i]];
    if (w >= 0) wrow[w] = 0u;
}
__global__ void scatter_pairs_kernel(const int32_t* __restrict__ pairs, int n, int32_t* __restrict__ table) {
    const int i = blockIdx.x * blockDim.x + threadIdx.x;
    if (i < n) table[pairs[2 * i]] = pairs[2 * i + 1];
}
__global__ void iota_i32_kernel(int32_t* dst, int n, int32_t first) {
    const int i = blockIdx.x * blockDim.x + threadIdx.x;
    if (i < n) dst[i] = first + i;
}

inline int next_pow2(int v) { int p = 2; while (p < v) p <<= 1; return p; }

}

__device__ __forceinline__ int shard_owned_below(int32_t id, int32_t first, int32_t block, int rank, int world) {
    if (id <= first) return 0;
    const long long x = (long long)id - first, cyc = (long long)block * world;
    const long long rem = x % cyc - (long long)rank * block;
    return (int)((x / cyc) * block + (rem < 0 ? 0 : (rem > block ? block : rem)));
}
__device__ __forceinline__ void shard_append_body(int* s_first , const AppendArgs& ap,
                                                  const WsRuns& new_ws, const int32_t* __restrict__ codes, int q, int rank, int world,
                                                  int32_t own_first, int32_t own_block) {
    __shared__ int s_n_new;
    const int tid = threadIdx.x;
    if (tid == 0) s_n_new = 0;
    for (int k = tid; k < q; k += blockDim.x) s_first[k] = 0x7fffffff;
    __syncthreads();
    for (int i = tid; i < q; i += blockDim.x) {
        const int c = codes[i];
        if (c < 0) { atomicMin(&s_first[-c - 1], i); atomicMax(&s_n_new, -c); }
    }
    __syncthreads();
    const int n_new = s_n_new, n_in = ap.cnt_in[0];
    auto below = [&](int k) -> int {
        if (own_block > 0) return shard_owned_below(ap.first_id + k, own_first, own_block, rank, world) - shard_owned_below(ap.first_id, own_first, own_block, rank, world);
        return rank == world - 1 ? k : 0;
    };
    const int n_own = below(n_new);
    const int n_take = (long long)n_in + n_own <= ap.capacity ? n_own : 0;
    const int c = tid & 15;
    float norm_max = 0.0f;
    for (int k = tid >> 4; k < n_new && n_take > 0; k += (int)blockDim.x >> 4) {
        const int j = below(k);
        if (below(k + 1) == j) continue;
        const size_t row = (size_t)n_in + (size_t)j;
        const uint32_t* src = reinterpret_cast<const uint32_t*>(ap.descriptors) + (size_t)s_first[k] * ap.row_dwords;
        if (ap.is_f32_64) append_write_row(ap, row, c, reinterpret_cast<const uint4*>(src)[c], norm_max);
        else { uint32_t* dst = ap.vocab + row * ap.row_dwords; for (int d = c; d < ap.row_dwords; d += 16) dst[d] = src[d]; }
// ... 28 lines not shown
    shard_append_kernel<<<1, 1024, (size_t)q * 4, s>>>(ap, new_ws, codes, q, rank, world, own_first, own_block);
    return hipGetLastError();
}

hipError_t launch_gather_f32(const float* dense, const int64_t* slots, int n, float* out, hipStream_t s) {
    if (n <= 0) return hipSuccess;
    gather_f32_kernel<<<(n + 255) / 256, 256, 0, s>>>(dense, (const long long*)slots, n, out);
    return hipGetLastError();
}

#define TF_TRY(x) do { hipError_t e__ = (x); if (e__ != hipSuccess) return e__; } while (0)

hipError_t BufPool::get(size_t bytes, DevBuf* out, int64_t* total) {
    int best = -1;
    for (size_t i = 0; i < free_list.size(); ++i) {
        if (free_list[i].cap >= bytes && free_list[i].cap <= 4 * std::max<size_t>(bytes, 4096) && (best < 0 || free_list[i].cap < free_list[best].cap)) best = (int)i;
    }
    if (best >= 0) { *out = free_list[best]; free_list.erase(free_list.begin() + best); return hipSuccess; }
    size_t cap = 4096;
    while (cap < bytes) cap *= 2;
    void* p = nullptr;
    hipError_t e = hipMalloc(&p, cap);
    if (e != hipSuccess) return e;
    out->p = p; out->cap = cap;
    if (total) *total += (int64_t)cap;
    return hipSuccess;
}
void BufPool::put(DevBuf* b) {
    if (b->p) free_list.push_back(*b);
    b->p = nullptr; b->cap = 0;
}
void BufPool::destroy(int64_t* total) {
    for (DevBuf& b : free_list) b.release(total);
    free_list.clear();
}

static hipError_t grow_filled(DevBuf& buf, size_t bytes, int byte, hipStream_t s, int64_t* total) {
    const size_t old = buf.cap;
    if (bytes <= old) return hipSuccess;
    hipError_t e = buf.reserve(bytes, old, s, total);
    if (e != hipSuccess) return e;
    return hipMemsetAsync((char*)buf.p + old, byte, buf.cap - old, s);
}
static hipError_t grow_zeroed(DevBuf& buf, size_t bytes, hipStream_t s, int64_t* total) { return grow_filled(buf, bytes, 0, s, total); }

static hipError_t set_max_lds(const void* fn) {
    hipFuncAttributes attr;
    size_t fixed = 1024;
    if (hipFuncGetAttributes(&attr, fn) == hipSuccess) fixed = (attr.sharedSizeBytes + 255) & ~(size_t)255;
    if (hipFuncSetAttribute(fn, hipFuncAttributeMaxDynamicSharedMemorySize, (int)(160 * 1024 - fixed)) != hipSuccess) (void)hipGetLastError();
    return hipSuccess;
}

hipError_t Tfidf::init(hipStream_t s, int64_t* bytes, int64_t sig_capacity, int64_t vocab_capacity) {
    stream = s;
    bytes_device = bytes;
    TF_TRY(ensure_slots(sig_capacity > 0 ? sig_capacity : TF_R));
    TF_TRY(ensure_buckets((int)((sig_capacity > 0 ? sig_capacity : TF_R) / TF_R) + 64));
    TF_TRY(ensure_wslots((int32_t)std::min<int64_t>(std::max<int64_t>(65536, 4 * vocab_capacity), 1 << 27)));
    dir2_hint_blocks = (uint32_t)std::min<int64_t>((2 * std::max<int64_t>(vocab_capacity, 8192) + 65536) / 32, 1 << 22);
    dir2_hint_stride = (uint32_t)std::min<int64_t>((sig_capacity > 0 ? sig_capacity : TF_R) / TF_R + 64, 1 << 20);
    TF_TRY(q_w.reserve(TF_MAX_WORDS * 4, 0, stream, bytes_device));
    TF_TRY(q_idf.reserve(TF_MAX_WORDS * 4, 0, stream, bytes_device));
    TF_TRY(q_did.reserve(TF_MAX_WORDS * 4, 0, stream, bytes_device));
    TF_TRY(qd_did.reserve(TF_MAX_WORDS * 4, 0, stream, bytes_device));
    TF_TRY(qd_idf.reserve(TF_MAX_WORDS * 4, 0, stream, bytes_device));
    TF_TRY(q_meta.reserve(64, 0, stream, bytes_device));
    TF_TRY(hipMemsetAsync(q_meta.p, 0, 64, stream));
    TF_TRY(n_dense.reserve(64, 0, stream, bytes_device));
    TF_TRY(hipMemsetAsync(n_dense.p, 0, 64, stream));
    TF_TRY(hipHostMalloc((void**)&h_n_dense, 64, hipHostMallocDefault));
    h_n_dense[0] = 0;
    TF_TRY(set_max_lds(reinterpret_cast<const void*>(&frame_words_kernel)));
    TF_TRY(set_max_lds(reinterpret_cast<const void*>(&frame_tail_kernel)));
    TF_TRY(set_max_lds(reinterpret_cast<const void*>(&frame_words_append_kernel)));
    TF_TRY(set_max_lds(reinterpret_cast<const void*>(&bulk_register_kernel)));
    return hipSuccess;
}

void Tfidf::destroy() {
    harvest_released(true);
    for (PinBlock& b : pin_free) { (void)hipEventDestroy(b.ev); (void)hipHostFree(b.p); }
    pin_free.clear();
    for (Bucket& b : buckets) { b.coo_w.release(bytes_device); b.coo_pc.release(bytes_device); b.sealed.release(bytes_device); }
    buckets.clear();
    pool.destroy(bytes_device);
    DevBuf* all[] = {&slot_sig, &slot_ni, &slot_begin, &slot_cnt, &nw, &did, &wrow, &idf_tab, &d_id2ws, &bkt_tab, &bkt_ne, &bkt_D, &bkt_flags,
                     &n_dense, &dir2, &seal_cntw, &seal_tiles, &q_w, &q_idf, &q_did, &qd_did, &qd_idf, &q_meta, &d_stage, &d_pairs};
    for (DevBuf* d : all) d->release(bytes_device);
    h_stage.release();
    if (h_n_dense) { (void)hipHostFree(h_n_dense); h_n_dense = nullptr; }
}

hipError_t Tfidf::ensure_slots(int64_t n) {
    TF_TRY(grow_zeroed(slot_sig, (size_t)n * 4, stream, bytes_device));
    TF_TRY(grow_zeroed(slot_ni, (size_t)n * 4, stream, bytes_device));
    TF_TRY(grow_zeroed(slot_begin, (size_t)n * 4, stream, bytes_device));
    TF_TRY(grow_zeroed(slot_cnt, (size_t)n * 4, stream, bytes_device));
    return hipSuccess;
}

hipError_t Tfidf::ensure_wslots(int32_t n) {
    TF_TRY(grow_zeroed(nw, (size_t)n * 4, stream, bytes_device));
    TF_TRY(grow_filled(did, (size_t)n * 4, 0xFF, stream, bytes_device));
    TF_TRY(grow_zeroed(wrow, (size_t)n * 4, stream, bytes_device));
    TF_TRY(grow_zeroed(idf_tab, (size_t)n * 8, stream, bytes_device));
    return hipSuccess;
}

hipError_t Tfidf::ensure_buckets(int n) {
    TF_TRY(grow_zeroed(bkt_tab, (size_t)n * sizeof(BucketDev), stream, bytes_device));
    TF_TRY(grow_zeroed(bkt_ne, (size_t)n * 4, stream, bytes_device));
    TF_TRY(grow_zeroed(bkt_D, (size_t)n * 4, stream, bytes_device));
    TF_TRY(grow_zeroed(bkt_flags, (size_t)n * 4, stream, bytes_device));
    return hipSuccess;
}

void Tfidf::free_wslot(int32_t w) {
    int32_t start = w, len = 1;
    auto next = ws_free.lower_bound(w);
    if (next != ws_free.begin()) {
        auto prev = std::prev(next);
        if (prev->first + prev->second > w) return;
        if (prev->first + prev->second == w) { start = prev->first; len += prev->second; ws_free.erase(prev); }
    }
    if (next != ws_free.end() && next->first == w + 1) { len += next->second; ws_free.erase(next); }
    ws_free[start] = len;
    ws_free_count += 1;
}

void Tfidf::free_wslot_run(int32_t start, int32_t len) {
    if (len <= 0) return;
    auto next = ws_free.lower_bound(start);
    const bool clash_next = next != ws_free.end() && next->first < start + len;
    const bool clash_prev = next != ws_free.begin() && std::prev(next)->first + std::prev(next)->second > start;
    if (len == 1 || clash_next || clash_prev) {
        for (int32_t k = 0; k < len; ++k) free_wslot(start + k);
        return;
    }
    int32_t s0 = start, l0 = len;
    if (next != ws_free.begin()) {
        auto prev = std::prev(next);
        if (prev->first + prev->second == start) { s0 = prev->first; l0 += prev->second; ws_free.erase(prev); }
    }
    if (next != ws_free.end() && next->first == start + len) { l0 += next->second; ws_free.erase(next); }
    ws_free[s0] = l0;
    ws_free_count += len;
}

int32_t Tfidf::take_wslot() {
    if (ws_free.empty()) return -1;
    auto it = std::prev(ws_free.end());
    const int32_t w = it->first + it->second - 1;
    if (--it->second == 0) ws_free.erase(it);
    ws_free_count -= 1;
    return w;
}

hipError_t Tfidf::wslot_of(int32_t word_id, bool create, int32_t* out) {
    *out = -1;
    if (word_id <= 0) return hipSuccess;
    if ((size_t)word_id < id2ws.size() && id2ws[word_id] >= 0) { *out = id2ws[word_id]; return hipSuccess; }
    int32_t w = -1;
    if (resv.n > 0 && resv.first_id > 0 && word_id >= resv.first_id && word_id < resv.first_id + resv.n) {
        w = ws_runs_at(resv.runs, word_id - resv.first_id);
    } else {
        if (std::find(held_ids.begin(), held_ids.end(), word_id) != held_ids.end()) { TF_TRY(flush_held()); harvest_released(true); }
        for (size_t i = 0; i < releasing.size(); ++i) {
            const ReleaseBatch& r = releasing[i];
            if (std::find(r.ids.begin(), r.ids.end(), word_id) != r.ids.end()) { harvest_released(true); break; }
        }
        if ((size_t)word_id < id2ws.size() && id2ws[word_id] >= 0) { *out = id2ws[word_id]; return hipSuccess; }
        if (!create) return hipSuccess;
        if (word_id >= (1 << 28)) return hipErrorInvalidValue;
        harvest_released(false);
        w = take_wslot();
        if (w < 0) { w = n_wslots++; TF_TRY(ensure_wslots(n_wslots)); }
    }
    if ((size_t)word_id >= id2ws.size()) id2ws.resize((size_t)word_id + 1 + id2ws.size() / 2, -1);
    id2ws[word_id] = w;
    id2ws_dirty.push_back(word_id);
    *out = w;
    return hipSuccess;
}

hipError_t Tfidf::sync_id2ws() {
    TF_TRY(grow_filled(d_id2ws, std::max<size_t>(id2ws.size(), 1) * 4, 0xFF, stream, bytes_device));
    d_id2ws_n = (int64_t)(d_id2ws.cap / 4);
    if (id2ws_dirty.empty()) return hipSuccess;
    const size_t m = id2ws_dirty.size();
    TF_TRY(h_stage.reserve(m * 8));
    int32_t* st = h_stage.as<int32_t>();
    for (size_t i = 0; i < m; ++i) { st[2 * i] = id2ws_dirty[i]; st[2 * i + 1] = id2ws[id2ws_dirty[i]]; }
    TF_TRY(d_pairs.reserve(m * 8, 0, stream, bytes_device));
    TF_TRY(hipMemcpyAsync(d_pairs.p, st, m * 8, hipMemcpyHostToDevice, stream));
    scatter_pairs_kernel<<<(unsigned)((m + 255) / 256), 256, 0, stream>>>(d_pairs.as<int32_t>(), (int)m, d_id2ws.as<int32_t>());
    TF_TRY(hipGetLastError());
// ... 78 lines not shown
hipError_t Tfidf::rows_drop_keys(const int32_t* d_row_wslot, const int32_t* d_rows, int n) {
    if (n <= 0) return hipSuccess;
    wrow_clear_kernel<<<(unsigned)((n + 255) / 256), 256, 0, stream>>>(d_row_wslot, d_rows, n, wrow.as<uint32_t>());
    return hipGetLastError();
}
void Tfidf::adopt_key(int32_t word_id, int32_t ws) {
    if (word_id <= 0 || ws < 0) return;
    if ((size_t)word_id >= id2ws.size()) id2ws.resize((size_t)word_id + 1 + id2ws.size() / 2, -1);
    if (id2ws[word_id] < 0) { id2ws[word_id] = ws; id2ws_dirty.push_back(word_id); }
}
void Tfidf::forget_word(int32_t word_id, int32_t ws) {
    if (word_id <= 0 || ws < 0 || (size_t)word_id >= id2ws.size() || id2ws[word_id] != ws) return;
    id2ws[word_id] = -1;
    id2ws_dirty.push_back(word_id);
    held_ws.push_back(ws); held_ids.push_back(0);
}
hipError_t Tfidf::rows_unlog_keys(const int32_t* d_pairs, int n) {
    if (n <= 0) return hipSuccess;
    wrow_unlog_kernel<<<(unsigned)((n + 255) / 256), 256, 0, stream>>>(d_pairs, n, wrow.as<uint32_t>());
    return hipGetLastError();
}
hipError_t Tfidf::rows_clear() {
    return (wrow.p && n_wslots > 0) ? hipMemsetAsync(wrow.p, 0, (size_t)n_wslots * 4, stream) : hipSuccess;
}

hipError_t Tfidf::release_words(const int32_t* word_ids, int n) {
    TF_TRY(flush_retire());
    std::vector<int32_t> ws;
    for (int i = 0; i < n; ++i) {
        int32_t w = -1;
        TF_TRY(wslot_of(word_ids[i], false, &w));
        if (w < 0) continue;
        id2ws[word_ids[i]] = -1;
        id2ws_dirty.push_back(word_ids[i]);
        ws.push_back(w);
    }
    return release_wslots(ws);
}

hipError_t Tfidf::reserve_new_words(int32_t first_id, int n, WsRuns* runs, bool may_flush) {
    runs->n = 0;
    if ((first_id <= 0 && first_id != -1) || n <= 0) return hipSuccess;
    if (first_id > 0 && (int64_t)first_id + n >= (1 << 28)) return hipErrorInvalidValue;
    if (resv.n > 0) {
        int32_t k = 0;
        for (int i = 0; i < resv.runs.n; ++i) {
            for (int32_t j = 0; j < resv.runs.len[i]; ++j, ++k) {
                const int32_t id = resv.first_id > 0 ? resv.first_id + k : 0;
                if (id > 0 && (size_t)id < id2ws.size() && id2ws[id] >= 0) continue;
                held_ws.push_back(resv.runs.start[i] + j);
                held_ids.push_back((id > 0 && (first_id <= 0 || id < first_id)) ? id : 0);
            }
        }
        resv.n = 0;
        if (may_flush && held_ws.size() >= 16384) TF_TRY(flush_held());
    }
    harvest_released(false);
    int left = n;
    while (left > 0 && runs->n < 15 && !ws_free.empty()) {
        auto it = std::prev(ws_free.end());
        const int32_t take = std::min(it->second, left);
        const int32_t start = it->first + it->second - take;
        runs->start[runs->n] = start; runs->len[runs->n] = take; runs->n += 1;
        if ((it->second -= take) == 0) ws_free.erase(it);
        ws_free_count -= take;
        left -= take;
    }
    if (left > 0) {
        runs->start[runs->n] = n_wslots; runs->len[runs->n] = left; runs->n += 1;
        n_wslots += left;
        TF_TRY(ensure_wslots(n_wslots));
    }
    resv.first_id = first_id; resv.n = n; resv.runs = *runs;
    return hipSuccess;
}

hipError_t Tfidf::set_bucket(int b) {
    const Bucket& k = buckets[b];
    BucketDev d;
    d.coo_w = k.coo_w.as<uint32_t>(); d.coo_pc = k.coo_pc.as<uint32_t>();
    d.dense = k.sealed.as<uint8_t>();
    d.dirb = k.sealed.p ? (const uint2*)((const char*)k.sealed.p + k.off_dirb) : nullptr;
    d.sp_off = k.sealed.p ? (const uint32_t*)((const char*)k.sealed.p + k.off_spoff) : nullptr;
    d.sp_ent = k.sealed.p ? (const uint32_t*)((const char*)k.sealed.p + k.off_spent) : nullptr;
    d.W = k.W; d.D_alloc = k.D_alloc; d.state = (uint32_t)k.state; d.pad = 0;
    set_bucket_kernel<<<1, 1, 0, stream>>>(bkt_tab.as<BucketDev>(), b, d);
    return hipGetLastError();
}

hipError_t Tfidf::new_bucket() {
    const int b = (int)buckets.size();
    buckets.emplace_back();
    TF_TRY(ensure_buckets(b + 1));
    return hipSuccess;
}

static hipError_t ensure_log(Tfidf& t, int b, int64_t entries) {
    Bucket& k = t.buckets[b];
    const size_t need = (size_t)std::max<int64_t>(entries, 1) * 4;
    if (need <= k.coo_w.cap) return hipSuccess;
    if (!k.coo_w.p) {
        TF_TRY(t.pool.get(std::max(need, (size_t)TF_R * 512 * 4), &k.coo_w, t.bytes_device));
        TF_TRY(t.pool.get(std::max(need, (size_t)TF_R * 512 * 4), &k.coo_pc, t.bytes_device));
    } else {
        TF_TRY(k.coo_w.reserve(need, (size_t)k.ub_entries * 4, t.stream, t.bytes_device));
        TF_TRY(k.coo_pc.reserve(need, (size_t)k.ub_entries * 4, t.stream, t.bytes_device));
    }
    return t.set_bucket(b);
}

hipError_t Tfidf::ensure_dir2(uint32_t blocks, uint32_t buckets_needed) {
    if (blocks <= dir2_blocks && buckets_needed <= dir2_stride) return hipSuccess;
    uint32_t nb = std::max<uint32_t>(dir2_blocks, 256), ns = std::max<uint32_t>(dir2_stride, 64);
    if (!dir2.p) { while (nb < dir2_hint_blocks) nb *= 2; while (ns < dir2_hint_stride) ns *= 2; }
    while (nb < blocks) nb *= 2;
    while (ns < buckets_needed) ns *= 2;
    DevBuf nd;
    const size_t rec = (size_t)TF_DIR2_DWORDS * 4;
    TF_TRY(nd.reserve((size_t)nb * ns * rec, 0, stream, bytes_device));
    TF_TRY(hipMemsetAsync(nd.p, 0, (size_t)nb * ns * rec, stream));
    if (dir2.p && dir2_blocks && dir2_stride)
        TF_TRY(hipMemcpy2DAsync(nd.p, (size_t)ns * rec, dir2.p, (size_t)dir2_stride * rec, (size_t)dir2_stride * rec, dir2_blocks, hipMemcpyDeviceToDevice, stream));
    if (dir2.p) { TF_TRY(hipStreamSynchronize(stream)); dir2.release(bytes_device); }
    dir2 = nd; dir2_blocks = nb; dir2_stride = ns;
    return hipSuccess;
}

hipError_t Tfidf::seal_batch(const std::vector<int>& ids, bool bulk) {
    if (ids.empty()) return hipSuccess;
    const uint32_t W = (uint32_t)n_wslots;
    TF_TRY(ensure_dir2((W + 31) / 32, (uint32_t)buckets.size() + 1));
    const int tiles = std::max(1, (int)((W + SEAL_TILE - 1) / SEAL_TILE));
    const size_t BATCH = 64;
    TF_TRY(seal_cntw.reserve(std::min(BATCH, ids.size()) * std::max<size_t>(W, 1) * 4, 0, stream, bytes_device));
    TF_TRY(seal_tiles.reserve(std::min(BATCH, ids.size()) * (size_t)tiles * 8, 0, stream, bytes_device));
    DevBuf d_jobs;
    bool have_dense_count = false;
    for (size_t i0 = 0; i0 < ids.size(); i0 += BATCH) {
        const size_t nb = std::min(BATCH, ids.size() - i0);
        std::vector<SealJob> jobs(nb);
        uint32_t max_e = 1;
        TF_TRY(hipMemsetAsync(seal_cntw.p, 0, nb * std::max<size_t>(W, 1) * 4, stream));
        for (size_t j = 0; j < nb; ++j) {
            Bucket& k = buckets[ids[i0 + j]];
            SealJob& J = jobs[j];
            J.bucket = ids[i0 + j];
            J.coo_w = k.coo_w.as<uint32_t>(); J.coo_pc = k.coo_pc.as<uint32_t>(); J.ne = bkt_ne.as<uint32_t>() + J.bucket;
            J.cntw = seal_cntw.as<uint32_t>() + j * (size_t)W; J.tile_sums = seal_tiles.as<uint32_t>() + j * (size_t)tiles * 2;
            J.W = W; J.ent_cap = (uint32_t)std::max<int64_t>(k.ub_entries, 1);
            J.dense = nullptr; J.D_alloc = 0; J.dirb = nullptr; J.sp_off = nullptr; J.sp_ent = nullptr;
            J.dir2 = dir2.as<uint32_t>(); J.dir2_stride = dir2_stride;
            max_e = std::max(max_e, J.ent_cap);
        }
        const SealJob* dj = nullptr;
        auto upload_jobs = [&]() -> hipError_t {
            if (nb == 1) return hipSuccess;
            TF_TRY(d_jobs.reserve(nb * sizeof(SealJob), 0, stream, bytes_device));
            TF_TRY(hipMemcpyAsync(d_jobs.p, jobs.data(), nb * sizeof(SealJob), hipMemcpyHostToDevice, stream));
            TF_TRY(hipStreamSynchronize(stream));
            dj = (const SealJob*)d_jobs.p;
            return hipSuccess;
        };
        TF_TRY(upload_jobs());
        const dim3 ge((unsigned)std::min<uint32_t>((max_e + SEAL_BLOCK - 1) / SEAL_BLOCK, 512), (unsigned)nb);
        const dim3 gw((unsigned)std::min<uint32_t>((W + SEAL_BLOCK - 1) / SEAL_BLOCK + 1, 512), (unsigned)nb);
        seal_count_kernel<<<ge, SEAL_BLOCK, 0, stream>>>(dj, jobs[0]);
        seal_densify_kernel<<<gw, SEAL_BLOCK, 0, stream>>>(dj, jobs[0], did.as<int32_t>(), n_dense.as<uint32_t>());
        TF_TRY(hipGetLastError());
        uint32_t D_alloc;
        if (bulk) {
            if (!have_dense_count) {
                uint32_t nd = 0;
                TF_TRY(hipMemcpyAsync(&nd, n_dense.p, 4, hipMemcpyDeviceToHost, stream));
                TF_TRY(hipStreamSynchronize(stream));
                h_n_dense[0] = std::min<uint32_t>(nd, TF_DENSE_MAX);
                have_dense_count = true;
            }
            D_alloc = std::min<uint32_t>(TF_DENSE_MAX, h_n_dense[0] + 32);
        } else {
            const uint32_t hv = *(volatile uint32_t*)h_n_dense;
            D_alloc = std::min<uint32_t>(TF_DENSE_MAX, hv + (hv ? 128u : 1024u));
        }
        for (size_t j = 0; j < nb; ++j) {
            Bucket& k = buckets[ids[i0 + j]];
            SealJob& J = jobs[j];
            const size_t a256 = 255;
            const size_t sz_dense = ((size_t)D_alloc * TF_R + a256) & ~a256;
            const size_t sz_dirb = ((((size_t)W + 31) / 32) * 8 + a256) & ~a256;
            const size_t sz_off = ((std::min<size_t>(J.ent_cap, W) + 1) * 4 + a256) & ~a256;
            const size_t sz_ent = ((size_t)J.ent_cap * 4 + a256) & ~a256;
            TF_TRY(pool.get(sz_dense + sz_dirb + sz_off + sz_ent, &k.sealed, bytes_device));
            k.off_dirb = sz_dense; k.off_spoff = sz_dense + sz_dirb; k.off_spent = sz_dense + sz_dirb + sz_off;
            k.W = W; k.D_alloc = D_alloc;
            J.dense = k.sealed.as<uint8_t>(); J.D_alloc = D_alloc;
            J.dirb = (uint2*)((char*)k.sealed.p + k.off_dirb);
            J.sp_off = (uint32_t*)((char*)k.sealed.p + k.off_spoff);
            J.sp_ent = (uint32_t*)((char*)k.sealed.p + k.off_spent);
            if (sz_dense) TF_TRY(hipMemsetAsync(J.dense, 0, sz_dense, stream));
        }
        TF_TRY(upload_jobs());
        const dim3 gt((unsigned)tiles, (unsigned)nb);
        seal_classify_kernel<<<ge, SEAL_BLOCK, 0, stream>>>(dj, jobs[0], did.as<int32_t>(), n_dense.as<uint32_t>(), bkt_D.as<uint32_t>(),
                                                           bkt_flags.as<uint32_t>(), h_n_dense);
        seal_tile_kernel<<<gt, SEAL_BLOCK, 0, stream>>>(dj, jobs[0]);
        seal_scan_kernel<<<gt, SEAL_BLOCK, 0, stream>>>(dj, jobs[0]);
        seal_scatter_kernel<<<ge, SEAL_BLOCK, 0, stream>>>(dj, jobs[0], did.as<int32_t>(), bkt_D.as<uint32_t>());
        TF_TRY(hipGetLastError());
        for (size_t j = 0; j < nb; ++j) {
            Bucket& k = buckets[ids[i0 + j]];
            k.state = 1;
            pool.put(&k.coo_pc);
            TF_TRY(set_bucket(ids[i0 + j]));
            seals += 1;
        }
    }
    if (d_jobs.p) { TF_TRY(hipStreamSynchronize(stream)); d_jobs.release(bytes_device); }
    return hipSuccess;
}

static RetireArgs take_pending(Tfidf& t) {
    RetireArgs r;
    r.n = 0;
    for (int i = 0; i < 4; ++i) { r.slot[i] = 0; r.coo_w[i] = nullptr; }
    while (r.n < 4 && !t.pending_retire.empty()) {
        const int64_t slot = t.pending_retire.back();
        t.pending_retire.pop_back();
        r.slot[r.n] = slot;
        r.coo_w[r.n] = t.buckets[(size_t)(slot / TF_R)].coo_w.as<uint32_t>();
        r.n += 1;
    }
    return r;
}

hipError_t Tfidf::flush_retire() {
    while (!pending_retire.empty()) {
        const int64_t slot = pending_retire.back();
        pending_retire.pop_back();
        retire_kernel<<<1, 256, 0, stream>>>((long long)slot, buckets[(size_t)(slot / TF_R)].coo_w.as<uint32_t>(), slot_begin.as<uint32_t>(),
                                             slot_cnt.as<uint32_t>(), nw.as<uint32_t>(), slot_ni.as<uint32_t>(), slot_sig.as<int32_t>());
        TF_TRY(hipGetLastError());
    }
    return hipSuccess;
}

static hipError_t run_frame_words(Tfidf& t, const int32_t* d_src, int n, bool ids_given, bool reg, int32_t sig_id, int64_t slot, int32_t ni,
                                  float N, const ResolveArgs* resolve, TailLaunch* defer, const WsRuns* new_ws = nullptr,
                                  const ShardAppendJob* shard_app = nullptr) {
    if (shard_app && (resolve || defer || shard_app->q <= 0 || shard_app->q > 8192)) return hipErrorInvalidValue;
    const int H = next_pow2(std::max(2 * n, 128));
    size_t shmem = ((size_t)H * 2 + H / 64 + 8) * 4;
    if (ids_given) TF_TRY(t.sync_id2ws());
    FwArgs a;
    a.src = d_src; a.n = n; a.xlate = ids_given ? t.d_id2ws.as<int32_t>() : nullptr; a.xlate_n = ids_given ? t.d_id2ws_n : 0;
    a.H = H; a.do_register = reg ? 1 : 0; a.want_q = 1;
    a.sig_id = sig_id; a.slot = (long long)slot; a.slot_local = (uint32_t)(slot % TF_R); a.ni = (uint32_t)ni; a.N = N;
    a.coo_w = nullptr; a.coo_pc = nullptr; a.ne_counter = nullptr;
    if (reg) {
        const int bi = (int)(slot / TF_R);
        a.coo_w = t.buckets[bi].coo_w.as<uint32_t>();
        a.coo_pc = t.buckets[bi].coo_pc.as<uint32_t>();
        a.ne_counter = t.bkt_ne.as<uint32_t>() + bi;
    }
    if (t.pending_retire.size() > 4) TF_TRY(t.flush_retire());
    const RetireArgs ret = take_pending(t);
    t.stamp += 1;
    if (t.stamp == 0) t.stamp = 1;
    a.stamp = t.stamp;
    a.nw = t.nw.as<uint32_t>(); a.did = t.did.as<int32_t>();
    a.slot_sig = t.slot_sig.as<int32_t>(); a.slot_ni = t.slot_ni.as<uint32_t>(); a.slot_begin = t.slot_begin.as<uint32_t>();
    a.slot_cnt = t.slot_cnt.as<uint32_t>();
    a.q_w = t.q_w.as<uint32_t>(); a.q_idf = t.q_idf.as<int32_t>(); a.q_did = t.q_did.as<int32_t>(); a.qd_did = t.qd_did.as<int32_t>();
    a.qd_idf = t.qd_idf.as<int32_t>(); a.q_meta = t.q_meta.as<uint32_t>(); a.idf_tab = t.idf_tab.as<uint2>();
    a.new_ws = new_ws ? *new_ws : WsRuns();
    a.wrow = t.wrow.as<uint32_t>();
    a.row_wslot = nullptr;
    if (defer && !resolve) {
        defer->a = a; defer->ret = ret; defer->shmem = shmem;
        t.q_n_ub = n;
        return hipSuccess;
    }
    if (resolve) {
        a.src = resolve->out_wslot;
        const int mw = (resolve->q + 63) / 64 * 2;
        shmem = std::max(shmem, (size_t)(3 * mw + 2) * 4) + (size_t)n * 8;
        const int block = defer ? pipe_block_size() : FW_BLOCK;
        const int n_redo = (resolve->rp.enabled && resolve->fail_count) ? std::min((resolve->rp.n_rows + block - 1) / block, defer ? REDO_WGS_MAX : (1 << 30)) : 0;
        if (defer) {
            defer->r = *resolve; defer->a = a; defer->ret = ret; defer->n_redo = n_redo; defer->shmem = shmem;
            t.q_n_ub = n;
            return hipSuccess;
        }
        frame_tail_kernel<<<1 + n_redo, FW_BLOCK, shmem, t.stream>>>(*resolve, a, ret);
    } else if (shard_app) {
        frame_words_append_kernel<<<2, FW_BLOCK, std::max(shmem, (size_t)shard_app->q * 4), t.stream>>>(a, ret, *shard_app);
    } else {
        frame_words_kernel<<<1, FW_BLOCK, shmem, t.stream>>>(a, ret);
    }
    t.q_n_ub = n;
    return hipGetLastError();
}
// ... 20 lines not shown
    sig_slot[sig_id] = slot;
    return hipSuccess;
}

hipError_t Tfidf::query_dev(const int32_t* d_wslots, int n, float N, const ResolveArgs* resolve, bool ids_given, TailLaunch* defer,
                            const WsRuns* new_ws, const ShardAppendJob* shard_app) {
    if (n > TF_MAX_WORDS) return hipErrorInvalidValue;
    return run_frame_words(*this, d_wslots, n, ids_given, false, 0, 0, 0, N, resolve, defer, new_ws, shard_app);
}

void resolve_launch_info(const ResolveArgs& r, int block, int* n_redo, size_t* shmem) {
    const int mw = (r.q + 63) / 64 * 2;
    *shmem = (size_t)(3 * mw + 4) * 4 + (size_t)r.q * 4;
    *n_redo = (r.rp.enabled && r.fail_count) ? std::min((r.rp.n_rows + block - 1) / block, REDO_WGS_MAX) : 0;
}

hipError_t Tfidf::register_bulk(int n_sigs, const int32_t* sig_ids, const int64_t* offsets, const int32_t* ni, const int32_t* d_ids,
                                int64_t total_ids, int max_n) {
    if (n_sigs <= 0) return hipSuccess;
    (void)total_ids;
    TF_TRY(sync_id2ws());
    const int64_t slot0 = n_slots;
    TF_TRY(ensure_slots(slot0 + n_sigs));
    const int b_first = (int)(slot0 / TF_R), b_last = (int)((slot0 + n_sigs - 1) / TF_R);
    if (b_first > 0 && b_first >= (int)buckets.size() && buckets[b_first - 1].state == 0)
        TF_TRY(seal_batch(std::vector<int>(1, b_first - 1), false));
    while ((int)buckets.size() <= b_last) TF_TRY(new_bucket());
    std::vector<int64_t> add(b_last - b_first + 1, 0);
    for (int s = 0; s < n_sigs; ++s) add[(size_t)((slot0 + s) / TF_R - b_first)] += offsets[s + 1] - offsets[s];
    for (int b = b_first; b <= b_last; ++b) TF_TRY(ensure_log(*this, b, buckets[b].ub_entries + add[b - b_first]));
    DevBuf d_off, d_sig, d_ni;
    TF_TRY(d_off.reserve((size_t)(n_sigs + 1) * 8, 0, stream, bytes_device));
    TF_TRY(d_sig.reserve((size_t)n_sigs * 4, 0, stream, bytes_device));
    TF_TRY(hipMemcpyAsync(d_off.p, offsets, (size_t)(n_sigs + 1) * 8, hipMemcpyHostToDevice, stream));
    TF_TRY(hipMemcpyAsync(d_sig.p, sig_ids, (size_t)n_sigs * 4, hipMemcpyHostToDevice, stream));
    if (ni) {
        TF_TRY(d_ni.reserve((size_t)n_sigs * 4, 0, stream, bytes_device));
        TF_TRY(hipMemcpyAsync(d_ni.p, ni, (size_t)n_sigs * 4, hipMemcpyHostToDevice, stream));
    }
    const int H = next_pow2(std::max(2 * max_n, 64));
    const size_t shmem = ((size_t)H * 2 + H / 64 + 8) * 4;
    bulk_register_kernel<<<(unsigned)n_sigs, BR_BLOCK, shmem, stream>>>(d_ids, (const long long*)d_off.p, d_sig.as<int32_t>(),
                                                                         ni ? d_ni.as<int32_t>() : nullptr, (long long)slot0,
                                                                         d_id2ws.as<int32_t>(), d_id2ws_n, bkt_tab.as<BucketDev>(),
                                                                         bkt_ne.as<uint32_t>(), nw.as<uint32_t>(), slot_sig.as<int32_t>(),
                                                                         slot_ni.as<uint32_t>(), slot_begin.as<uint32_t>(), slot_cnt.as<uint32_t>());
    TF_TRY(hipGetLastError());
    std::vector<int> full;
    for (int s = 0; s < n_sigs; ++s) {
        const int64_t slot = slot0 + s;
        Bucket& b = buckets[(size_t)(slot / TF_R)];
        b.n_slots += 1; b.live += 1;
        sig_slot[sig_ids[s]] = slot;
    }
    for (int b = b_first; b <= b_last; ++b) {
        buckets[b].ub_entries += add[b - b_first];
        if (buckets[b].n_slots == TF_R && b < b_last) full.push_back(b);
    }
    postings_ub += offsets[n_sigs] - offsets[0];
    n_slots += n_sigs;
    live_sigs += n_sigs;
    TF_TRY(seal_batch(full, true));
    TF_TRY(hipStreamSynchronize(stream));
    d_off.release(bytes_device); d_sig.release(bytes_device); d_ni.release(bytes_device);
    return hipSuccess;
}

hipError_t Tfidf::score_args(float* d_likelihood, long long* lfix, int block, ScoreArgs* out, int* n_wgs) {
    *n_wgs = 0;
    if (n_slots == 0) return hipSuccess;
    TF_TRY(flush_retire());
    const bool has_open = !buckets.empty() && buckets.back().state == 0;
    ScoreArgs& A = *out;
    A.tab = bkt_tab.as<BucketDev>(); A.bkt_D = bkt_D.as<uint32_t>(); A.bkt_flags = bkt_flags.as<uint32_t>();
    A.n_closed = (int)buckets.size() - (has_open ? 1 : 0);
    A.n_open_slots = has_open ? buckets.back().n_slots : 0;
    A.wcap = std::max(q_n_ub, 1);
    A.q_w = q_w.as<uint32_t>(); A.q_idf = q_idf.as<int32_t>(); A.q_did = q_did.as<int32_t>(); A.qd_did = qd_did.as<int32_t>();
    A.qd_idf = qd_idf.as<int32_t>(); A.q_meta = q_meta.as<uint32_t>();
    A.slot_ni = slot_ni.as<uint32_t>(); A.slot_begin = slot_begin.as<uint32_t>(); A.slot_cnt = slot_cnt.as<uint32_t>();
    A.idf_tab = idf_tab.as<uint2>(); A.stamp = stamp;
    A.out_like = d_likelihood; A.out_fix = lfix;
    A.dir2 = dir2.as<uint32_t>(); A.dir2_stride = dir2_stride;
    A.n_closed_pad = (A.n_closed + 7) / 8 * 8;
    *n_wgs = A.n_closed_pad + (A.n_open_slots + block / 64 - 1) / (block / 64);
    return hipSuccess;
}

hipError_t Tfidf::launch_score(float* d_likelihood, long long* lfix) {
    const int scb = score_block == 256 || score_block == 1024 ? score_block : 512;
    ScoreArgs A;
    int grid = 0;
    TF_TRY(score_args(d_likelihood, lfix, scb, &A, &grid));
    if (grid == 0) return hipSuccess;
    if (prof_b) TF_TRY(hipEventRecord(prof_b, stream));
    if (scb == 256) score_kernel<256><<<grid, 256, 0, stream>>>(A);
    else if (scb == 512) score_kernel<512><<<grid, 512, 0, stream>>>(A);
    else score_kernel<1024><<<grid, 1024, 0, stream>>>(A);
    TF_TRY(hipGetLastError());
    if (prof_e) TF_TRY(hipEventRecord(prof_e, stream));
    prof_b = prof_e = nullptr;
    return hipSuccess;
}

hipError_t Tfidf::score_work(int64_t out[8]) {
    for (int i = 0; i < 8; ++i) out[i] = 0;
    if (n_slots == 0) return hipSuccess;
    TF_TRY(flush_retire());
    const bool has_open = !buckets.empty() && buckets.back().state == 0;
    ScoreArgs A;
    A.tab = bkt_tab.as<BucketDev>(); A.bkt_D = bkt_D.as<uint32_t>(); A.bkt_flags = bkt_flags.as<uint32_t>();
    A.n_closed = (int)buckets.size() - (has_open ? 1 : 0);
    A.n_open_slots = has_open ? buckets.back().n_slots : 0;
    A.wcap = std::max(q_n_ub, 1);
    A.q_w = q_w.as<uint32_t>(); A.q_idf = q_idf.as<int32_t>(); A.q_did = q_did.as<int32_t>(); A.qd_did = qd_did.as<int32_t>();
    A.qd_idf = qd_idf.as<int32_t>(); A.q_meta = q_meta.as<uint32_t>();
    A.slot_ni = slot_ni.as<uint32_t>(); A.slot_begin = slot_begin.as<uint32_t>(); A.slot_cnt = slot_cnt.as<uint32_t>();
    A.idf_tab = idf_tab.as<uint2>(); A.stamp = stamp; A.out_like = nullptr; A.out_fix = nullptr;
    DevBuf cnt;
    TF_TRY(cnt.reserve(64, 0, stream, bytes_device));
    TF_TRY(hipMemsetAsync(cnt.p, 0, 64, stream));
    score_work_kernel<<<A.n_closed + 1, 256, 0, stream>>>(A, nw.as<uint32_t>(), (unsigned long long*)cnt.p);
    TF_TRY(hipGetLastError());
    TF_TRY(hipMemcpyAsync(out, cnt.p, 64, hipMemcpyDeviceToHost, stream));
    TF_TRY(hipStreamSynchronize(stream));
    cnt.release(bytes_device);
    return hipSuccess;
}

hipError_t Tfidf::score(float* d_likelihood) { return launch_score(d_likelihood, nullptr); }
hipError_t Tfidf::score_fix(long long* lfix) { return launch_score(nullptr, lfix); }

hipError_t Tfidf::finalize(const long long* lfix_src, long long n, float* d_likelihood) {
    if (n <= 0) return hipSuccess;
    finalize_kernel<<<(unsigned)((n + 255) / 256), 256, 0, stream>>>(lfix_src, n, slot_ni.as<uint32_t>(), d_likelihood);
    return hipGetLastError();
}

hipError_t Tfidf::retire(int32_t sig_id) {
    auto it = sig_slot.find(sig_id);
    if (it == sig_slot.end()) return hipErrorInvalidValue;
    const int64_t slot = it->second;
    const int bi = (int)(slot / TF_R);
    Bucket& b = buckets[bi];
    pending_retire.push_back(slot);
    sig_slot.erase(it);
    live_sigs -= 1;
    b.live -= 1;
    if (b.live == 0 && b.state == 1) {
        TF_TRY(flush_retire());
        postings_ub -= b.ub_entries;
        pool.put(&b.coo_w); pool.put(&b.coo_pc); pool.put(&b.sealed);
        b.W = 0; b.D_alloc = 0; b.ub_entries = 0; b.state = 2;
        TF_TRY(set_bucket(bi));
    }
    return hipSuccess;
}

}

extern "C" int lcd_debug_key_intervals(const int32_t* keys, const unsigned char* ok, int n, int by_runs, int take, int32_t* out, int cap, long long* count) {
    lcd::Tfidf t;
    int32_t run_start = 0, run_len = 0;
    for (int i = 0; i < n; ++i) {
        if (!ok[i]) { if (by_runs) { t.free_wslot_run(run_start, run_len); run_len = 0; } continue; }
        if (!by_runs) { t.free_wslot(keys[i]); continue; }
        if (run_len > 0 && keys[i] == run_start + run_len) { run_len += 1; continue; }
        t.free_wslot_run(run_start, run_len);
        run_start = keys[i]; run_len = 1;
    }
    if (by_runs) t.free_wslot_run(run_start, run_len);
    for (int i = 0; i < take; ++i) (void)t.take_wslot();
    if ((int)t.ws_free.size() > cap) return -1;
    int k = 0;
    for (const auto& kv : t.ws_free) { out[2 * k] = kv.first; out[2 * k + 1] = kv.second; k += 1; }
    if (count) *count = (long long)t.ws_free_count;
    return k;
}

#ifdef LCD_SCORE_TIMING
extern "C" int lcd_debug_score_timing(unsigned long long* out, int n_words) {
    if (hipDeviceSynchronize() != hipSuccess) return -1;
    return (int)hipMemcpyFromSymbol(out, HIP_SYMBOL(lcd::g_score_timing), (size_t)n_words * 8);
}
#endif
#ifdef LCD_TAIL_TIMING
extern "C" int lcd_debug_tail_timing(unsigned long long* out) {
    if (hipDeviceSynchronize() != hipSuccess) return -1;
    if (hipMemcpyFromSymbol(out, HIP_SYMBOL(lcd::g_tail_timing), 64) != hipSuccess) return -2;
    return (int)hipMemcpyFromSymbol(out + 8, HIP_SYMBOL(lcd::g_resolve_timing), 64);
}
#endif
```

Before: 3.352 billion candidates/s.

## Merge sealed buckets into groups with a shared sparse index for scoring

Adds bucket groups: once TF_G consecutive buckets are sealed, their sparse postings are merged into one group index with its own directory. The score kernel then processes one work unit per group, using a dynamic LDS accumulator sized for TF_G*TF_R slots and double-buffered dense-row loads across the group's buckets. The aim is to cut per-bucket directory lookups and workgroup overhead for sparse words, and to amortise query-list loads. In exchange it adds merge kernels at seal time, extra device memory, and more LDS per workgroup, which may lower occupancy.

```diff
diff --git a/include/lcd.h b/include/lcd.h
--- a/include/lcd.h
+++ b/include/lcd.h
@@ -185,6 +185,7 @@
 int lcd_trace_pop(lcd_engine* h);
 
 int lcd_profile_score_work(lcd_engine* h, int64_t* out8);
+int lcd_index_info(lcd_engine* h, int64_t* out, int n);
 
 typedef struct lcd_stats {
     int64_t vocab_rows, vocab_live;
diff --git a/rtabmap_amd/capi.py b/rtabmap_amd/capi.py
--- a/rtabmap_amd/capi.py
+++ b/rtabmap_amd/capi.py
@@ -17,7 +17,7 @@
     "lcd_vocab_clear", "lcd_vocab_append", "lcd_vocab_remove", "lcd_vocab_remove_unused", "lcd_vocab_remove_unused_async", "lcd_vocab_rebuild", "lcd_vocab_count", "lcd_vocab_read",
     "lcd_knn2", "lcd_selfdist", "lcd_quantize", "lcd_find_nn",
     "lcd_sig_add", "lcd_sig_remove", "lcd_sig_add_bulk", "lcd_sig_count", "lcd_word_nrefs",
-    "lcd_likelihood", "lcd_adjust_likelihood", "lcd_adjust_likelihood_dev", "lcd_frame_dev", "lcd_frame_host", "lcd_slot_count", "lcd_knn2_dev", "lcd_shard_knn2_dev", "lcd_shard_frame_dev", "lcd_finalize_dev", "lcd_slots_dev", "lcd_stream", "lcd_get_stats", "lcd_profile_begin", "lcd_profile_read", "lcd_profile_read_likelihood", "lcd_profile_score_work", "lcd_set_option", "lcd_record_event", "lcd_trace_push", "lcd_trace_pop",
+    "lcd_likelihood", "lcd_adjust_likelihood", "lcd_adjust_likelihood_dev", "lcd_frame_dev", "lcd_frame_host", "lcd_slot_count", "lcd_knn2_dev", "lcd_shard_knn2_dev", "lcd_shard_frame_dev", "lcd_finalize_dev", "lcd_slots_dev", "lcd_stream", "lcd_get_stats", "lcd_profile_begin", "lcd_profile_read", "lcd_profile_read_likelihood", "lcd_profile_score_work", "lcd_index_info", "lcd_set_option", "lcd_record_event", "lcd_trace_push", "lcd_trace_pop",
     "lcd_bayes_configure", "lcd_bayes_reset", "lcd_bayes_set_neighbors", "lcd_bayes_update_dev", "lcd_bayes_update", "lcd_bayes_posterior",
 ]
 
@@ -135,6 +135,7 @@
     L.lcd_profile_read_likelihood.argtypes = [vp, C.POINTER(f32), C.POINTER(C.c_int), C.POINTER(C.c_char_p)]
     L.lcd_get_stats.argtypes = [vp, C.POINTER(LcdStats)]
     L.lcd_profile_score_work.argtypes = [vp, C.POINTER(i64)]
+    L.lcd_index_info.argtypes = [vp, C.POINTER(i64), C.c_int]
     L.lcd_set_option.argtypes = [vp, C.c_char_p, i64]
     L.lcd_record_event.argtypes = [vp, vp]
     L.lcd_bayes_configure.argtypes = [vp, vp, C.c_int, f32]
@@ -435,6 +436,12 @@
                 "unique_words", "dense_words"]
         return {k: int(v) for k, v in zip(keys, out)}
 
+    def index_info(self):
+        out = (C.c_int64 * 5)()
+        self._ck(self.L.lcd_index_info(self.h, out, 5))
+        keys = ["groups", "group_bytes", "group_merges", "buckets_per_group", "group_directory_bytes"]
+        return {k: int(v) for k, v in zip(keys, out)}
+
     def stats(self):
         s = LcdStats()
         self._ck(self.L.lcd_get_stats(self.h, C.byref(s)))
diff --git a/rtabmap_amd/csrc/engine.hip b/rtabmap_amd/csrc/engine.hip
--- a/rtabmap_amd/csrc/engine.hip
+++ b/rtabmap_amd/csrc/engine.hip
@@ -1332,6 +1332,8 @@
     { int rc = h->drain(); if (rc) return rc; }
     if (!key) return h->fail(LCD_ERR_INVALID, "lcd_set_option: null key");
     if (!std::strcmp(key, "score_block") && (value == 256 || value == 512 || value == 1024)) { h->tfidf.score_block = (int)value; return LCD_OK; }
+    if (!std::strcmp(key, "sparse_groups") && value >= -1 && value <= 2) { h->tfidf.sparse_groups = value < 0 ? 1 : (int)value; return LCD_OK; }
+    if (!std::strcmp(key, "sparse_groups_from") && value >= -1 && value <= (1 << 24)) { h->tfidf.sparse_groups_from = value < 0 ? lcd::SPARSE_GROUPS_FROM : (int)value; return LCD_OK; }
     if (!std::strcmp(key, "filter_units") && value >= -1 && value <= 4096) { h->filter_units = (int)value; return LCD_OK; }
     if (!std::strcmp(key, "strip_tiles") && value >= 0 && value <= 8) { h->strip_tiles = (int)value; return LCD_OK; }
     if (!std::strcmp(key, "shard_growth_first") && value >= 0 && value < (1ll << 28)) { h->shard_first = (int32_t)value; return LCD_OK; }
@@ -1387,6 +1389,17 @@
     LCD_CATCH(h)
 }
 
+int lcd_index_info(lcd_engine* h, int64_t* out, int n) {
+    LCD_TRY
+    LCD_CHECK_HANDLE(h);
+    if (!out || n < 0) return h->fail(LCD_ERR_INVALID, "lcd_index_info: null output");
+    int64_t v[5];
+    h->tfidf.index_info(v);
+    for (int i = 0; i < n; ++i) out[i] = i < 5 ? v[i] : 0;
+    return LCD_OK;
+    LCD_CATCH(h)
+}
+
 int lcd_get_stats(lcd_engine* h, lcd_stats* out) {
     LCD_TRY
     LCD_CHECK_HANDLE(h);
diff --git a/rtabmap_amd/csrc/knn_mfma_kernels.hip b/rtabmap_amd/csrc/knn_mfma_kernels.hip
--- a/rtabmap_amd/csrc/knn_mfma_kernels.hip
+++ b/rtabmap_amd/csrc/knn_mfma_kernels.hip
@@ -1772,8 +1772,9 @@
     }
     const int g = bid - n_rerank_wgs;
     if (g < A.n_closed_pad) {
-        const int b = (g & 7) * (A.n_closed_pad >> 3) + (g >> 3);
-        if (b < A.n_closed) score_sealed_body<PIPE_B_BLOCK>(A, b);
+        extern __shared__ __attribute__((aligned(16))) float s_dyn_sc[];
+        const int u = (g & 7) * (A.n_closed_pad >> 3) + (g >> 3);
+        if (u < A.n_units) score_sealed_body<PIPE_B_BLOCK>(A, u, reinterpret_cast<unsigned long long*>(s_dyn_sc));
     } else score_open_body<PIPE_B_BLOCK>(A, g - A.n_closed_pad);
     B_STAMP(1);
 }
@@ -2174,7 +2175,7 @@
     int n_app = 0;
     if (app && app->ap.enabled && app->ap.defer_rows) { ar = *app; n_app = ar.n_wgs = APPEND_ROW_WGS; }
     if (n_rerank + score_wgs + n_app == 0) return hipSuccess;
-    const uint32_t dyn = ((k && k->n_hi) || n_app) ? PIPE_B_STAGE_ROWS * 256u + 512u : 0u;
+    const uint32_t dyn = ((k && k->n_hi) || n_app) ? PIPE_B_STAGE_ROWS * 256u + 512u : (score_wgs > 0 ? (uint32_t)SCORE_LDS_BYTES : 0u);
     rk.stage_rows = (dyn && k && k->n_hi) ? (int)PIPE_B_STAGE_ROWS : 0;
     ar.ap.lds_bytes = (int)(PIPE_B_STAGE_ROWS * 256u);
     if (k && n_app) { rk.pend_desc = ar.ap.descriptors; rk.pend_list = ar.ap.list_out; rk.pend_first_id = ar.ap.first_id; }
diff --git a/rtabmap_amd/csrc/score_body.cuh b/rtabmap_amd/csrc/score_body.cuh
--- a/rtabmap_amd/csrc/score_body.cuh
+++ b/rtabmap_amd/csrc/score_body.cuh
@@ -13,6 +13,7 @@
 
 
 
+constexpr size_t SCORE_LDS_BYTES = (size_t)TF_G * TF_R * 8;
 template <int SCB>
 __device__ __forceinline__ void score_segments(const uint32_t* __restrict__ sp_ent, unsigned long long* acc, uint32_t start, uint32_t len, int32_t idf) {
     const int ln = threadIdx.x & 63;
@@ -38,136 +39,172 @@
         for (int u = 0; u < 2; ++u) {
             if (!ok[u]) continue;
             const long long term = (long long)(int)(e[u] & TF_CNT_MASK) * (long long)f[u];
-            atomicAdd(&acc[e[u] >> TF_CNT_BITS], (unsigned long long)term);
-        }
-    }
+            atomicAdd(&acc[(e[u] >> TF_CNT_BITS) & (uint32_t)(TF_G * TF_R - 1)], (unsigned long long)term);
+        }
+    }
+}
+
+__device__ __forceinline__ bool dir2_decode(const uint4& r0, const uint4& r1, uint32_t p, uint32_t* start, uint32_t* len) {
+    const unsigned long long q[4] = {((unsigned long long)r0.y << 32) | r0.x, ((unsigned long long)r0.w << 32) | r0.z,
+                                     ((unsigned long long)r1.y << 32) | r1.x, ((unsigned long long)r1.w << 32) | r1.z};
+    const uint32_t pd = p / 9u, ps = (uint32_t)TF_DIR2_FBITS * (p % 9u);
+    uint32_t before = 0;
+    unsigned long long fd = q[0];
+#pragma unroll
+    for (uint32_t d = 0; d < 4u; ++d) {
+        const unsigned long long x = (d == 0 ? q[0] & ~TF_DIR2_SAT : (d == 3 ? q[3] & ((1ull << TF_DIR2_OFF_SHIFT) - 1ull) : q[d]));
+        before += dir2_sum9(d < pd ? x : (d == pd ? (x & ((1ull << ps) - 1ull)) : 0ull));
+        fd = d == pd ? x : fd;
+    }
+    *len = (uint32_t)(fd >> ps) & TF_DIR2_FMAX;
+    *start = (uint32_t)(q[3] >> TF_DIR2_OFF_SHIFT) + before;
+    return !(q[0] & TF_DIR2_SAT);
 }
 
 template <int SCB>
-__device__ __forceinline__ void score_sealed_body(const ScoreArgs& A, int b) {
-    __shared__ unsigned long long acc[TF_R];
+__device__ __forceinline__ void score_sealed_body(const ScoreArgs& A, int unit, unsigned long long* acc) {
     const int tid = threadIdx.x;
-    const BucketDev B = A.tab[b];
-    const long long first_slot = (long long)b * TF_R;
-    const bool live = B.state == 1u;
+    constexpr int NWV = SCB / 64;
+    constexpr int DR = NWV == 4 ? 8 : (64 / NWV > 8 ? 8 : 64 / NWV);
+    constexpr int DSTEP = DR * NWV;
+    constexpr int KW = SCB >= 512 ? 1 : 512 / SCB;
+    constexpr int NI = (TF_G * TF_R + SCB - 1) / SCB;
+    const int wv = __builtin_amdgcn_readfirstlane(tid >> 6), ln = tid & 63;
+    const bool grp = unit < A.n_grouped;
+    const int nb = grp ? TF_G : 1;
+    const int b0 = grp ? unit * TF_G : unit + A.n_grouped * (TF_G - 1);
+    const long long first_slot = (long long)b0 * TF_R;
+    for (int i = tid; i < nb * TF_R; i += SCB) acc[i] = 0ull;
+    __syncthreads();
     SC_STAMP(0);
-    constexpr int NWV = SCB / 64;
-#ifndef LCD_SCORE_DR4
-#define LCD_SCORE_DR4 16
-#endif
-    constexpr int DR = NWV == 4 ? LCD_SCORE_DR4 : (128 / NWV > 16 ? 16 : 128 / NWV);
-    constexpr int KW = SCB >= 512 ? 1 : 512 / SCB;
-    constexpr int NI = TF_R / SCB > 0 ? TF_R / SCB : 1;
-    const int wv = __builtin_amdgcn_readfirstlane(tid >> 6), ln = tid & 63;
-    const uint32_t D = live ? A.bkt_D[b] : 0u;
-    const uint32_t BW = live ? B.W : 0u;
-    const uint32_t flags = A.bkt_flags[b];
+    const uint8_t* dn[TF_G]; uint32_t Dm[TF_G];
+#pragma unroll
+    for (int m = 0; m < TF_G; ++m) {
+        const int bm = b0 + (m < nb ? m : 0);
+        const BucketDev Bm = A.tab[bm];
+        dn[m] = Bm.dense;
+        Dm[m] = (m < nb && Bm.state == 1u) ? A.bkt_D[bm] : 0u;
+    }
+    const uint2* s_dirb; const uint32_t* s_off; const uint32_t* s_ent; const uint32_t* rec_base;
+    uint32_t SW, D, flags, rec_stride, rec_idx;
+    if (grp) {
+        const GroupDev Gd = A.gtab[unit];
+        s_dirb = Gd.dirb; s_off = Gd.sp_off; s_ent = Gd.sp_ent; SW = Gd.state == 1u ? Gd.W : 0u;
+        D = A.grp_D[unit]; flags = A.grp_flags[unit];
+        rec_base = A.gdir; rec_stride = A.gdir_stride; rec_idx = (uint32_t)unit;
+    } else {
+        const BucketDev B = A.tab[b0];
+        s_dirb = B.dirb; s_off = B.sp_off; s_ent = B.sp_ent; SW = B.state == 1u ? B.W : 0u;
+        D = Dm[0]; flags = A.bkt_flags[b0];
+        rec_base = A.dir2; rec_stride = A.dir2_stride; rec_idx = (uint32_t)b0;
+    }
     const int U = (int)A.q_meta[0];
     const int Ud = (int)A.q_meta[1];
-    static_assert(KW * SCB <= TF_MAX_WORDS && DR * NWV <= TF_MAX_WORDS, "the unconditional list reads stay inside the buffers");
+    static_assert(KW * SCB <= TF_MAX_WORDS && 2 * DSTEP <= TF_MAX_WORDS, "the unconditional list reads stay inside the buffers");
     uint32_t w[KW]; int32_t idf[KW], did[KW]; bool look[KW];
 #pragma unroll
     for (int u = 0; u < KW; ++u) {
         const int k = tid + u * SCB;
         w[u] = A.q_w[k]; idf[u] = A.q_idf[k]; did[u] = A.q_did[k];
     }
-    int32_t dj[DR], fj[DR];
-#pragma unroll
-    for (int u = 0; u < DR; ++u) {
-        const int j = wv + u * NWV;
-        dj[u] = A.qd_did[j];
-        fj[u] = A.qd_idf[j];
-    }
+    int32_t dj[2][DR], fj[2][DR];
+#pragma unroll
+    for (int h = 0; h < 2; ++h)
+#pragma unroll
+        for (int u = 0; u < DR; ++u) {
+            const int j = wv + (u + h * DR) * NWV;
+            dj[h][u] = A.qd_did[j];
+            fj[h][u] = A.qd_idf[j];
+        }
 #pragma unroll
     for (int u = 0; u < KW; ++u) { if (tid + u * SCB >= U) { w[u] = 0; idf[u] = 0; did[u] = -1; } }
 #pragma unroll
-    for (int u = 0; u < DR; ++u) { if (wv + u * NWV >= Ud) { dj[u] = -1; fj[u] = 0; } }
+    for (int h = 0; h < 2; ++h)
+#pragma unroll
+        for (int u = 0; u < DR; ++u) { if (wv + (u + h * DR) * NWV >= Ud) { dj[h][u] = -1; fj[h][u] = 0; } }
     uint32_t ni_v[NI];
 #pragma unroll
-    for (int u = 0; u < NI; ++u) { const int i = tid + u * SCB; ni_v[u] = i < TF_R ? A.slot_ni[first_slot + i] : 0u; }
+    for (int u = 0; u < NI; ++u) { const int i = tid + u * SCB; ni_v[u] = i < nb * TF_R ? A.slot_ni[first_slot + i] : 0u; }
     uint4 r0[KW], r1[KW];
 #pragma unroll
     for (int u = 0; u < KW; ++u) {
         const bool dense_here = did[u] >= 0 && (uint32_t)did[u] < D;
-        look[u] = idf[u] != 0 && w[u] < BW && (!dense_here || (flags & 1u));
+        look[u] = idf[u] != 0 && w[u] < SW && (!dense_here || (flags & 1u));
+#ifdef LCD_EXP_NO_SPARSE
+        look[u] = false;
+#endif
         r0[u] = make_uint4(0u, 0u, 0u, 0u); r1[u] = r0[u];
         if (look[u]) {
-            const uint4* rec = reinterpret_cast<const uint4*>(A.dir2 + ((size_t)(w[u] >> 5) * A.dir2_stride + (uint32_t)b) * TF_DIR2_DWORDS);
+            const uint4* rec = reinterpret_cast<const uint4*>(rec_base + ((size_t)(w[u] >> 5) * rec_stride + rec_idx) * TF_DIR2_DWORDS);
             r0[u] = gload4(rec); r1[u] = gload4(rec + 1);
         }
     }
-    uint32_t c[DR];
-#pragma unroll
-    for (int u = 0; u < DR; ++u) c[u] = (dj[u] >= 0 && (uint32_t)dj[u] < D) ? gload((const uint32_t*)(B.dense + (size_t)dj[u] * TF_R + 4 * ln)) : 0u;
+    uint32_t cA[DR], cB[DR];
+#define SC_ROWS(c, m, h) _Pragma("unroll") for (int u = 0; u < DR; ++u) \
+        c[u] = (m < nb && dj[h][u] >= 0 && (uint32_t)dj[h][u] < Dm[m]) ? gload((const uint32_t*)(dn[m] + (size_t)dj[h][u] * TF_R + 4 * ln)) : 0u
+#define SC_MAC(c, h) _Pragma("unroll") for (int u = 0; u < DR; ++u) { \
+        const long long f64 = (long long)fj[h][u]; \
+        a0 += (long long)(int)(c[u] & 255u) * f64; a1 += (long long)(int)((c[u] >> 8) & 255u) * f64; \
+        a2 += (long long)(int)((c[u] >> 16) & 255u) * f64; a3 += (long long)(int)(c[u] >> 24) * f64; }
+    SC_ROWS(cA, 0, 0);
+    SC_ROWS(cB, 0, 1);
     uint32_t start[KW], len[KW];
 #pragma unroll
     for (int u = 0; u < KW; ++u) {
         start[u] = 0; len[u] = 0;
         if (!look[u]) continue;
-        const uint32_t f[6] = {r0[u].z, r0[u].w, r1[u].x, r1[u].y, r1[u].z, r1[u].w};
-        const uint32_t p = w[u] & 31u, pd = p / 6u, ps = 5u * (p % 6u);
-        if (!(r0[u].y & TF_DIR2_SAT)) {
-            uint32_t before = 0;
-#pragma unroll
-            for (uint32_t d = 0; d < 6u; ++d) {
-                const uint32_t x = d < pd ? f[d] : (d == pd ? (f[d] & ((1u << ps) - 1u)) : 0u);
-                before += dir2_sum6(x);
-            }
-            uint32_t fd = f[0];
-#pragma unroll
-            for (uint32_t d = 1; d < 6u; ++d) fd = d == pd ? f[d] : fd;
-            len[u] = (fd >> ps) & 31u;
-            start[u] = r0[u].x + before;
-        } else {
-            const uint2 blk = gload2(B.dirb + (w[u] >> 5));
+        const uint32_t p = w[u] & 31u;
+        uint32_t st = 0, l = 0;
+        if (dir2_decode(r0[u], r1[u], p, &st, &l)) { start[u] = st; len[u] = l; }
+        else {
+            const uint2 blk = gload2(s_dirb + (w[u] >> 5));
             const uint32_t bit = 1u << p;
             if (blk.x & bit) {
                 const uint32_t r = blk.y + (uint32_t)__popc(blk.x & (bit - 1u));
-                const uint32_t s0 = gload(B.sp_off + r), s1 = gload(B.sp_off + r + 1);
+                const uint32_t s0 = gload(s_off + r), s1 = gload(s_off + r + 1);
                 start[u] = s0; len[u] = s1 - s0;
             }
         }
     }
-    long long a0 = 0, a1 = 0, a2 = 0, a3 = 0;
-#pragma unroll
-    for (int u = 0; u < DR; ++u) {
-        const long long f64 = (long long)fj[u];
-        a0 += (long long)(int)(c[u] & 255u) * f64;
-        a1 += (long long)(int)((c[u] >> 8) & 255u) * f64;
-        a2 += (long long)(int)((c[u] >> 16) & 255u) * f64;
-        a3 += (long long)(int)(c[u] >> 24) * f64;
-    }
-    for (int j0 = wv + DR * NWV; j0 < Ud; j0 += DR * NWV) {
-#pragma unroll
-        for (int u = 0; u < DR; ++u) {
-            const int j = j0 + u * NWV;
-            dj[u] = j < Ud ? A.qd_did[j] : -1;
-            fj[u] = j < Ud ? A.qd_idf[j] : 0;
-        }
-#pragma unroll
-        for (int u = 0; u < DR; ++u) c[u] = (dj[u] >= 0 && (uint32_t)dj[u] < D) ? gload((const uint32_t*)(B.dense + (size_t)dj[u] * TF_R + 4 * ln)) : 0u;
-#pragma unroll
-        for (int u = 0; u < DR; ++u) {
-            const long long f64 = (long long)fj[u];
-            a0 += (long long)(int)(c[u] & 255u) * f64;
-            a1 += (long long)(int)((c[u] >> 8) & 255u) * f64;
-            a2 += (long long)(int)((c[u] >> 16) & 255u) * f64;
-            a3 += (long long)(int)(c[u] >> 24) * f64;
-        }
-    }
-    for (int i = tid; i < TF_R; i += SCB) acc[i] = 0ull;
-    __syncthreads();
     SC_STAMP(1);
-    {
-        const int ln4 = ln * 4;
+#pragma unroll
+    for (int m = 0; m < TF_G; ++m) {
+        if (m >= nb) break;
+        long long a0 = 0, a1 = 0, a2 = 0, a3 = 0;
+        SC_MAC(cA, 0);
+        if (m + 1 < TF_G) { SC_ROWS(cA, m + 1, 0); }
+        SC_MAC(cB, 1);
+        if (m + 1 < TF_G) { SC_ROWS(cB, m + 1, 1); }
+        for (int j0 = wv + 2 * DSTEP; j0 < Ud; j0 += DSTEP) {
+            int32_t dx[DR], fx[DR]; uint32_t cx[DR];
+#pragma unroll
+            for (int u = 0; u < DR; ++u) {
+                const int j = j0 + u * NWV;
+                dx[u] = j < Ud ? A.qd_did[j] : -1;
+                fx[u] = j < Ud ? A.qd_idf[j] : 0;
+            }
+#pragma unroll
+            for (int u = 0; u < DR; ++u) cx[u] = (dx[u] >= 0 && (uint32_t)dx[u] < Dm[m]) ? gload((const uint32_t*)(dn[m] + (size_t)dx[u] * TF_R + 4 * ln)) : 0u;
+#pragma unroll
+            for (int u = 0; u < DR; ++u) {
+                const long long f64 = (long long)fx[u];
+                a0 += (long long)(int)(cx[u] & 255u) * f64;
+                a1 += (long long)(int)((cx[u] >> 8) & 255u) * f64;
+                a2 += (long long)(int)((cx[u] >> 16) & 255u) * f64;
+                a3 += (long long)(int)(cx[u] >> 24) * f64;
+            }
+        }
+        const int ln4 = m * TF_R + ln * 4;
         if (a0) atomicAdd(&acc[ln4 + 0], (unsigned long long)a0);
         if (a1) atomicAdd(&acc[ln4 + 1], (unsigned long long)a1);
         if (a2) atomicAdd(&acc[ln4 + 2], (unsigned long long)a2);
         if (a3) atomicAdd(&acc[ln4 + 3], (unsigned long long)a3);
     }
+#undef SC_ROWS
+#undef SC_MAC
     SC_STAMP(2);
 #pragma unroll
-    for (int u = 0; u < KW; ++u) score_segments<SCB>(B.sp_ent, acc, start[u], len[u], idf[u]);
+    for (int u = 0; u < KW; ++u) score_segments<SCB>(s_ent, acc, start[u], len[u], idf[u]);
     for (int k0 = KW * SCB; k0 < U; k0 += SCB) {
         const int k = k0 + tid;
         uint32_t st2 = 0, ln2 = 0; int32_t idf2 = 0;
@@ -176,24 +213,28 @@
             idf2 = A.q_idf[k];
             const int32_t d2 = A.q_did[k];
             const bool dh = d2 >= 0 && (uint32_t)d2 < D;
-            if (idf2 != 0 && w2 < BW && (!dh || (flags & 1u))) {
-                const uint2 bk = gload2(B.dirb + (w2 >> 5));
+#ifdef LCD_EXP_NO_SPARSE
+            if (false) {
+#else
+            if (idf2 != 0 && w2 < SW && (!dh || (flags & 1u))) {
+#endif
+                const uint2 bk = gload2(s_dirb + (w2 >> 5));
                 const uint32_t bit = 1u << (w2 & 31);
                 if (bk.x & bit) {
                     const uint32_t r = bk.y + (uint32_t)__popc(bk.x & (bit - 1u));
-                    st2 = gload(B.sp_off + r);
-                    ln2 = gload(B.sp_off + r + 1) - st2;
+                    st2 = gload(s_off + r);
+                    ln2 = gload(s_off + r + 1) - st2;
                 }
             }
         }
-        score_segments<SCB>(B.sp_ent, acc, st2, ln2, idf2);
+        score_segments<SCB>(s_ent, acc, st2, ln2, idf2);
     }
     __syncthreads();
     SC_STAMP(3);
 #pragma unroll
     for (int u = 0; u < NI; ++u) {
         const int i = tid + u * SCB;
-        if (i >= TF_R) continue;
+        if (i >= nb * TF_R) continue;
         const long long v = (long long)acc[i];
         if (A.out_like) A.out_like[first_slot + i] = fixed_to_like(v, ni_v[u]);
         else A.out_fix[first_slot + i] = ni_v[u] ? v : 0;
diff --git a/rtabmap_amd/csrc/tfidf.h b/rtabmap_amd/csrc/tfidf.h
--- a/rtabmap_amd/csrc/tfidf.h
+++ b/rtabmap_amd/csrc/tfidf.h
@@ -20,11 +20,24 @@
 constexpr int TF_DENSE_T = 32;
 constexpr int TF_DENSE_MAX = 4096;
 constexpr int TF_DIR2_DWORDS = 8;
-constexpr uint32_t TF_DIR2_SAT = 1u << 31;
-__host__ __device__ inline uint32_t dir2_sum6(uint32_t x) {
-    const uint32_t t = (x & 0x01F07C1Fu) + ((x >> 5) & 0x01F07C1Fu);
-    return (t & 0x3FFu) + ((t >> 10) & 0x3FFu) + (t >> 20);
+constexpr int TF_DIR2_FBITS = 7;
+constexpr uint32_t TF_DIR2_FMAX = (1u << TF_DIR2_FBITS) - 1u;
+constexpr int TF_DIR2_OFF_SHIFT = 35;
+constexpr unsigned long long TF_DIR2_SAT = 1ull << 63;
+__host__ __device__ inline uint32_t dir2_sum9(unsigned long long x) {
+    const unsigned long long M = 0x7Full | (0x7Full << 14) | (0x7Full << 28) | (0x7Full << 42) | (0x7Full << 56);
+    const unsigned long long t = (x & M) + ((x >> 7) & M);
+    return (uint32_t)((t & 0x3FFFull) + ((t >> 14) & 0x3FFFull) + ((t >> 28) & 0x3FFFull) + ((t >> 42) & 0x3FFFull) + (t >> 56));
 }
+#ifndef LCD_TF_G
+#define LCD_TF_G 4
+#endif
+constexpr int TF_G = LCD_TF_G;
+#ifndef LCD_SPARSE_GROUPS_FROM
+#define LCD_SPARSE_GROUPS_FROM 1024
+#endif
+constexpr int SPARSE_GROUPS_FROM = LCD_SPARSE_GROUPS_FROM;
+static_assert(TF_G == 1 || TF_G == 2 || TF_G == 4, "slot_local << 22 | count has ten slot bits: at most four buckets of 256 slots");
 
 struct BucketDev {
     const uint32_t* coo_w;
@@ -38,6 +51,13 @@
     uint32_t state;
     uint32_t pad;
 };
+struct GroupDev {
+    const uint2* dirb;
+    const uint32_t* sp_off;
+    const uint32_t* sp_ent;
+    uint32_t W;
+    uint32_t state;
+};
 
 struct SealJob {
     int bucket;
@@ -57,8 +77,15 @@
     int live = 0;
     int64_t ub_entries = 0;
     DevBuf coo_w, coo_pc, sealed;
-    size_t off_dirb = 0, off_spoff = 0, off_spent = 0;
+    DevBuf spent;
+    size_t off_dirb = 0, off_spoff = 0;
     uint32_t W = 0, D_alloc = 0;
+};
+struct Group {
+    int state = 0;
+    DevBuf buf;
+    size_t off_spoff = 0, off_spent = 0;
+    uint32_t W = 0;
 };
 
 struct AppendArgs {
@@ -120,7 +147,11 @@
 struct ScoreArgs {
     const BucketDev* tab; const uint32_t* bkt_D; const uint32_t* bkt_flags;
     const uint32_t* dir2; uint32_t dir2_stride;
+    const GroupDev* gtab; const uint32_t* grp_D; const uint32_t* grp_flags;
+    const uint32_t* gdir; uint32_t gdir_stride;
+    int n_grouped;
     int n_closed;
+    int n_units;
     int n_closed_pad;
     int n_open_slots; int wcap;
     const uint32_t* q_w; const int32_t* q_idf; const int32_t* q_did; const int32_t* qd_did; const int32_t* qd_idf; const uint32_t* q_meta;
@@ -217,6 +248,18 @@
     DevBuf dir2;
     uint32_t dir2_blocks = 0, dir2_stride = 0, dir2_hint_blocks = 0, dir2_hint_stride = 0;
     hipError_t ensure_dir2(uint32_t blocks, uint32_t buckets_needed);
+    int sparse_groups = 1;
+    int sparse_groups_from = SPARSE_GROUPS_FROM;
+    bool want_gdir = false;
+    std::vector<Group> groups;
+    int n_grouped = 0;
+    DevBuf grp_tab, grp_D, grp_flags;
+    DevBuf gdir;
+    uint32_t gdir_stride = 0;
+    int64_t group_merges = 0;
+    hipError_t merge_groups();
+    hipError_t set_group(int g);
+    void index_info(int64_t out[5]) const;
     DevBuf n_dense;
     uint32_t* h_n_dense = nullptr;
     DevBuf seal_cntw, seal_tiles;
diff --git a/rtabmap_amd/csrc/tfidf.hip b/rtabmap_amd/csrc/tfidf.hip
--- a/rtabmap_amd/csrc/tfidf.hip
+++ b/rtabmap_amd/csrc/tfidf.hip
@@ -88,10 +88,11 @@
 
 template <int SCB>
 __global__ __launch_bounds__(SCB) void score_kernel(ScoreArgs A) {
+    extern __shared__ __attribute__((aligned(16))) unsigned long long s_score_acc[];
     const int g = (int)blockIdx.x;
     if (g < A.n_closed_pad) {
-        const int b = (g & 7) * (A.n_closed_pad >> 3) + (g >> 3);
-        if (b < A.n_closed) score_sealed_body<SCB>(A, b);
+        const int u = (g & 7) * (A.n_closed_pad >> 3) + (g >> 3);
+        if (u < A.n_units) score_sealed_body<SCB>(A, u, s_score_acc);
     } else score_open_body<SCB>(A, g - A.n_closed_pad);
 }
 
@@ -219,13 +220,17 @@
     if (w0 < J.W) {
         J.dirb[blk] = make_uint2(bits, rp);
         if (J.dir2) {
-            uint32_t f[6] = {0u, 0u, 0u, 0u, 0u, 0u};
+            unsigned long long q[4] = {0ull, 0ull, 0ull, (unsigned long long)ra << TF_DIR2_OFF_SHIFT};
             bool sat = false;
 #pragma unroll
-            for (uint32_t i = 0; i < 32u; ++i) { sat = sat || c[i] > 30u; f[i / 6] |= (c[i] > 30u ? 31u : c[i]) << (5u * (i % 6)); }
+            for (uint32_t i = 0; i < 32u; ++i) {
+                sat = sat || c[i] >= TF_DIR2_FMAX;
+                q[i / 9] |= (unsigned long long)(c[i] >= TF_DIR2_FMAX ? TF_DIR2_FMAX : c[i]) << ((uint32_t)TF_DIR2_FBITS * (i % 9));
+            }
+            if (sat) q[0] |= TF_DIR2_SAT;
             uint4* rec = reinterpret_cast<uint4*>(J.dir2 + ((size_t)blk * J.dir2_stride + (uint32_t)J.bucket) * TF_DIR2_DWORDS);
-            rec[0] = make_uint4(ra, rp | (sat ? TF_DIR2_SAT : 0u), f[0], f[1]);
-            rec[1] = make_uint4(f[2], f[3], f[4], f[5]);
+            rec[0] = make_uint4((uint32_t)q[0], (uint32_t)(q[0] >> 32), (uint32_t)q[1], (uint32_t)(q[1] >> 32));
+            rec[1] = make_uint4((uint32_t)q[2], (uint32_t)(q[2] >> 32), (uint32_t)q[3], (uint32_t)(q[3] >> 32));
         }
     }
 #pragma unroll
@@ -254,6 +259,51 @@
 }
 
 __global__ void set_bucket_kernel(BucketDev* tab, int b, BucketDev v) { tab[b] = v; }
+__global__ void set_group_kernel(GroupDev* tab, int g, GroupDev v) { tab[g] = v; }
+
+__global__ __launch_bounds__(SEAL_BLOCK) void group_count_kernel(const BucketDev* __restrict__ tab, const uint32_t* __restrict__ bkt_D,
+                                                                 const uint32_t* __restrict__ bkt_flags, int g, uint32_t W, uint32_t* __restrict__ cntw,
+                                                                 uint32_t* __restrict__ grp_D, uint32_t* __restrict__ grp_flags) {
+    const uint32_t w = blockIdx.x * SEAL_BLOCK + threadIdx.x;
+    if (w == 0) {
+        uint32_t dmin = 0xFFFFFFFFu, fl = 0u;
+        for (int m = 0; m < TF_G; ++m) {
+            const int b = g * TF_G + m;
+            if (tab[b].state != 1u) continue;
+            dmin = min(dmin, bkt_D[b]); fl |= bkt_flags[b];
+        }
+        grp_D[g] = dmin == 0xFFFFFFFFu ? 0u : dmin; grp_flags[g] = fl;
+    }
+    if (w >= W) return;
+    uint32_t c = 0;
+    for (int m = 0; m < TF_G; ++m) {
+        const BucketDev B = tab[g * TF_G + m];
+        if (B.state != 1u || w >= B.W) continue;
+        const uint2 blk = B.dirb[w >> 5];
+        const uint32_t bit = 1u << (w & 31);
+        if (!(blk.x & bit)) continue;
+        const uint32_t r = blk.y + (uint32_t)__popc(blk.x & (bit - 1u));
+        c += B.sp_off[r + 1] - B.sp_off[r];
+    }
+    cntw[w] = c;
+}
+__global__ __launch_bounds__(SEAL_BLOCK) void group_scatter_kernel(const BucketDev* __restrict__ tab, int g, SealJob J) {
+    const uint32_t w = blockIdx.x * SEAL_BLOCK + threadIdx.x;
+    if (w >= J.W) return;
+    const uint2 gb = J.dirb[w >> 5];
+    const uint32_t bit = 1u << (w & 31);
+    if (!(gb.x & bit)) return;
+    uint32_t pos = J.sp_off[gb.y + (uint32_t)__popc(gb.x & (bit - 1u))];
+    for (int m = 0; m < TF_G; ++m) {
+        const BucketDev B = tab[g * TF_G + m];
+        if (B.state != 1u || w >= B.W) continue;
+        const uint2 blk = B.dirb[w >> 5];
+        if (!(blk.x & bit)) continue;
+        const uint32_t r = blk.y + (uint32_t)__popc(blk.x & (bit - 1u));
+        const uint32_t s0 = B.sp_off[r], s1 = B.sp_off[r + 1];
+        for (uint32_t e = s0; e < s1 && pos < J.ent_cap; ++e) J.sp_ent[pos++] = B.sp_ent[e] + ((uint32_t)m << (TF_CNT_BITS + 8));
+    }
+}
 
 __global__ void retire_kernel(long long slot, const uint32_t* __restrict__ coo_w, const uint32_t* __restrict__ slot_begin,
                               const uint32_t* __restrict__ slot_cnt, uint32_t* __restrict__ nw, uint32_t* __restrict__ slot_ni,
@@ -448,11 +498,14 @@
     harvest_released(true);
     for (PinBlock& b : pin_free) { (void)hipEventDestroy(b.ev); (void)hipHostFree(b.p); }
     pin_free.clear();
-    for (Bucket& b : buckets) { b.coo_w.release(bytes_device); b.coo_pc.release(bytes_device); b.sealed.release(bytes_device); }
+    for (Bucket& b : buckets) { b.coo_w.release(bytes_device); b.coo_pc.release(bytes_device); b.sealed.release(bytes_device); b.spent.release(bytes_device); }
     buckets.clear();
+    for (Group& g : groups) g.buf.release(bytes_device);
+    groups.clear();
+    n_grouped = 0;
     pool.destroy(bytes_device);
     DevBuf* all[] = {&slot_sig, &slot_ni, &slot_begin, &slot_cnt, &nw, &did, &wrow, &idf_tab, &d_id2ws, &bkt_tab, &bkt_ne, &bkt_D, &bkt_flags,
-                     &n_dense, &dir2, &seal_cntw, &seal_tiles, &q_w, &q_idf, &q_did, &qd_did, &qd_idf, &q_meta, &d_stage, &d_pairs};
+                     &n_dense, &dir2, &gdir, &grp_tab, &grp_D, &grp_flags, &seal_cntw, &seal_tiles, &q_w, &q_idf, &q_did, &qd_did, &qd_idf, &q_meta, &d_stage, &d_pairs};
     for (DevBuf* d : all) d->release(bytes_device);
     h_stage.release();
     if (h_n_dense) { (void)hipHostFree(h_n_dense); h_n_dense = nullptr; }
@@ -479,6 +532,12 @@
     TF_TRY(grow_zeroed(bkt_ne, (size_t)n * 4, stream, bytes_device));
     TF_TRY(grow_zeroed(bkt_D, (size_t)n * 4, stream, bytes_device));
     TF_TRY(grow_zeroed(bkt_flags, (size_t)n * 4, stream, bytes_device));
+    if (TF_G > 1) {
+        const size_t ng = (size_t)n / TF_G + 1;
+        TF_TRY(grow_zeroed(grp_tab, ng * sizeof(GroupDev), stream, bytes_device));
+        TF_TRY(grow_zeroed(grp_D, ng * 4, stream, bytes_device));
+        TF_TRY(grow_zeroed(grp_flags, ng * 4, stream, bytes_device));
+    }
     return hipSuccess;
 }
 
@@ -723,9 +782,20 @@
     d.dense = k.sealed.as<uint8_t>();
     d.dirb = k.sealed.p ? (const uint2*)((const char*)k.sealed.p + k.off_dirb) : nullptr;
     d.sp_off = k.sealed.p ? (const uint32_t*)((const char*)k.sealed.p + k.off_spoff) : nullptr;
-    d.sp_ent = k.sealed.p ? (const uint32_t*)((const char*)k.sealed.p + k.off_spent) : nullptr;
+    d.sp_ent = k.spent.as<uint32_t>();
     d.W = k.W; d.D_alloc = k.D_alloc; d.state = (uint32_t)k.state; d.pad = 0;
     set_bucket_kernel<<<1, 1, 0, stream>>>(bkt_tab.as<BucketDev>(), b, d);
+    return hipGetLastError();
+}
+
+hipError_t Tfidf::set_group(int g) {
+    const Group& k = groups[g];
+    GroupDev d;
+    d.dirb = (const uint2*)k.buf.p;
+    d.sp_off = k.buf.p ? (const uint32_t*)((const char*)k.buf.p + k.off_spoff) : nullptr;
+    d.sp_ent = k.buf.p ? (const uint32_t*)((const char*)k.buf.p + k.off_spent) : nullptr;
+    d.W = k.W; d.state = (uint32_t)k.state;
+    set_group_kernel<<<1, 1, 0, stream>>>(grp_tab.as<GroupDev>(), g, d);
     return hipGetLastError();
 }
 
@@ -750,21 +820,97 @@
     return t.set_bucket(b);
 }
 
+static hipError_t grow_dir(Tfidf& t, DevBuf& d, uint32_t ob, uint32_t os, uint32_t nb, uint32_t ns) {
+    DevBuf nd;
+    const size_t rec = (size_t)TF_DIR2_DWORDS * 4;
+    TF_TRY(nd.reserve((size_t)nb * ns * rec, 0, t.stream, t.bytes_device));
+    TF_TRY(hipMemsetAsync(nd.p, 0, (size_t)nb * ns * rec, t.stream));
+    if (d.p && ob && os)
+        TF_TRY(hipMemcpy2DAsync(nd.p, (size_t)ns * rec, d.p, (size_t)os * rec, (size_t)os * rec, ob, hipMemcpyDeviceToDevice, t.stream));
+    if (d.p) { TF_TRY(hipStreamSynchronize(t.stream)); d.release(t.bytes_device); }
+    d = nd;
+    return hipSuccess;
+}
 hipError_t Tfidf::ensure_dir2(uint32_t blocks, uint32_t buckets_needed) {
-    if (blocks <= dir2_blocks && buckets_needed <= dir2_stride) return hipSuccess;
+    const uint32_t groups_needed = (TF_G > 1 && (want_gdir || gdir.p)) ? buckets_needed / TF_G + 1 : 0;
+    if (blocks <= dir2_blocks && buckets_needed <= dir2_stride && groups_needed <= gdir_stride) return hipSuccess;
     uint32_t nb = std::max<uint32_t>(dir2_blocks, 256), ns = std::max<uint32_t>(dir2_stride, 64);
     if (!dir2.p) { while (nb < dir2_hint_blocks) nb *= 2; while (ns < dir2_hint_stride) ns *= 2; }
     while (nb < blocks) nb *= 2;
     while (ns < buckets_needed) ns *= 2;
-    DevBuf nd;
-    const size_t rec = (size_t)TF_DIR2_DWORDS * 4;
-    TF_TRY(nd.reserve((size_t)nb * ns * rec, 0, stream, bytes_device));
-    TF_TRY(hipMemsetAsync(nd.p, 0, (size_t)nb * ns * rec, stream));
-    if (dir2.p && dir2_blocks && dir2_stride)
-        TF_TRY(hipMemcpy2DAsync(nd.p, (size_t)ns * rec, dir2.p, (size_t)dir2_stride * rec, (size_t)dir2_stride * rec, dir2_blocks, hipMemcpyDeviceToDevice, stream));
-    if (dir2.p) { TF_TRY(hipStreamSynchronize(stream)); dir2.release(bytes_device); }
-    dir2 = nd; dir2_blocks = nb; dir2_stride = ns;
-    return hipSuccess;
+    uint32_t ngs = gdir_stride;
+    if (groups_needed) {
+        ngs = std::max<uint32_t>(gdir_stride, 16);
+        if (!gdir.p) while (ngs < dir2_hint_stride / TF_G + 1) ngs *= 2;
+        while (ngs < groups_needed) ngs *= 2;
+    }
+    if (nb != dir2_blocks || ns != dir2_stride) TF_TRY(grow_dir(*this, dir2, dir2_blocks, dir2_stride, nb, ns));
+    if (ngs && (nb != dir2_blocks || ngs != gdir_stride)) TF_TRY(grow_dir(*this, gdir, dir2_blocks, gdir_stride, nb, ngs));
+    dir2_blocks = nb; dir2_stride = ns; gdir_stride = ngs;
+    return hipSuccess;
+}
+
+hipError_t Tfidf::merge_groups() {
+    while (TF_G > 1 && sparse_groups) {
+        const int g = n_grouped, b0 = g * TF_G;
+        if (b0 + TF_G > (int)buckets.size()) break;
+        const int n_closed = (int)buckets.size() - ((!buckets.empty() && buckets.back().state == 0) ? 1 : 0);
+        if (sparse_groups == 1 && g == 0 && n_closed < sparse_groups_from) break;
+        uint32_t W = 0; int64_t cap = 0; int sealed = 0;
+        bool complete = true;
+        for (int m = 0; m < TF_G; ++m) {
+            const Bucket& k = buckets[b0 + m];
+            if (k.state == 0) complete = false;
+            if (k.state == 1) { W = std::max(W, k.W); cap += std::max<int64_t>(k.ub_entries, 1); sealed += 1; }
+        }
+        if (!complete) break;
+        want_gdir = true;
+        TF_TRY(ensure_dir2((W + 31) / 32, (uint32_t)buckets.size() + 1));
+        if ((int)groups.size() <= g) groups.resize(g + 1);
+        Group& G = groups[g];
+        if (sealed == 0 || W == 0) {
+            G.state = 2; G.W = 0;
+        } else {
+            if (cap >= (1ll << 29)) break;
+            const size_t a256 = 255;
+            const size_t sz_dirb = ((((size_t)W + 31) / 32) * 8 + a256) & ~a256;
+            const size_t sz_off = ((std::min<size_t>((size_t)cap, W) + 1) * 4 + a256) & ~a256;
+            const size_t sz_ent = ((size_t)cap * 4 + a256) & ~a256;
+            TF_TRY(pool.get(sz_dirb + sz_off + sz_ent, &G.buf, bytes_device));
+            G.off_spoff = sz_dirb; G.off_spent = sz_dirb + sz_off; G.W = W;
+            const int tiles = std::max(1, (int)((W + SEAL_TILE - 1) / SEAL_TILE));
+            TF_TRY(seal_cntw.reserve((size_t)W * 4, 0, stream, bytes_device));
+            TF_TRY(seal_tiles.reserve((size_t)tiles * 8, 0, stream, bytes_device));
+            SealJob J;
+            J.bucket = g; J.coo_w = nullptr; J.coo_pc = nullptr; J.ne = nullptr; J.dense = nullptr; J.D_alloc = 0;
+            J.dirb = (uint2*)G.buf.p; J.sp_off = (uint32_t*)((char*)G.buf.p + G.off_spoff); J.sp_ent = (uint32_t*)((char*)G.buf.p + G.off_spent);
+            J.dir2 = gdir.as<uint32_t>(); J.dir2_stride = gdir_stride;
+            J.cntw = seal_cntw.as<uint32_t>(); J.tile_sums = seal_tiles.as<uint32_t>(); J.W = W; J.ent_cap = (uint32_t)cap;
+            const unsigned gw = (unsigned)((W + SEAL_BLOCK - 1) / SEAL_BLOCK);
+            group_count_kernel<<<gw, SEAL_BLOCK, 0, stream>>>(bkt_tab.as<BucketDev>(), bkt_D.as<uint32_t>(), bkt_flags.as<uint32_t>(), g, W,
+                                                              J.cntw, grp_D.as<uint32_t>(), grp_flags.as<uint32_t>());
+            seal_tile_kernel<<<dim3((unsigned)tiles, 1), SEAL_BLOCK, 0, stream>>>(nullptr, J);
+            seal_scan_kernel<<<dim3((unsigned)tiles, 1), SEAL_BLOCK, 0, stream>>>(nullptr, J);
+            group_scatter_kernel<<<gw, SEAL_BLOCK, 0, stream>>>(bkt_tab.as<BucketDev>(), g, J);
+            TF_TRY(hipGetLastError());
+            for (int m = 0; m < TF_G; ++m) {
+                Bucket& k = buckets[b0 + m];
+                if (k.state != 1) continue;
+                pool.put(&k.spent);
+                TF_TRY(set_bucket(b0 + m));
+            }
+            G.state = 1;
+            group_merges += 1;
+        }
+        TF_TRY(set_group(g));
+        n_grouped = g + 1;
+    }
+    return hipSuccess;
+}
+
+void Tfidf::index_info(int64_t out[5]) const {
+    out[0] = 0; out[1] = 0; out[2] = group_merges; out[3] = TF_G; out[4] = (int64_t)gdir.cap;
+    for (const Group& g : groups) if (g.state == 1) { out[0] += 1; out[1] += (int64_t)g.buf.cap; }
 }
 
 hipError_t Tfidf::seal_batch(const std::vector<int>& ids, bool bulk) {
@@ -830,13 +976,14 @@
             const size_t sz_dirb = ((((size_t)W + 31) / 32) * 8 + a256) & ~a256;
             const size_t sz_off = ((std::min<size_t>(J.ent_cap, W) + 1) * 4 + a256) & ~a256;
             const size_t sz_ent = ((size_t)J.ent_cap * 4 + a256) & ~a256;
-            TF_TRY(pool.get(sz_dense + sz_dirb + sz_off + sz_ent, &k.sealed, bytes_device));
-            k.off_dirb = sz_dense; k.off_spoff = sz_dense + sz_dirb; k.off_spent = sz_dense + sz_dirb + sz_off;
+            TF_TRY(pool.get(sz_dense + sz_dirb + sz_off, &k.sealed, bytes_device));
+            TF_TRY(pool.get(sz_ent, &k.spent, bytes_device));
+            k.off_dirb = sz_dense; k.off_spoff = sz_dense + sz_dirb;
             k.W = W; k.D_alloc = D_alloc;
             J.dense = k.sealed.as<uint8_t>(); J.D_alloc = D_alloc;
             J.dirb = (uint2*)((char*)k.sealed.p + k.off_dirb);
             J.sp_off = (uint32_t*)((char*)k.sealed.p + k.off_spoff);
-            J.sp_ent = (uint32_t*)((char*)k.sealed.p + k.off_spent);
+            J.sp_ent = k.spent.as<uint32_t>();
             if (sz_dense) TF_TRY(hipMemsetAsync(J.dense, 0, sz_dense, stream));
         }
         TF_TRY(upload_jobs());
@@ -856,7 +1003,7 @@
         }
     }
     if (d_jobs.p) { TF_TRY(hipStreamSynchronize(stream)); d_jobs.release(bytes_device); }
-    return hipSuccess;
+    return merge_groups();
 }
 
 static RetireArgs take_pending(Tfidf& t) {
@@ -1043,7 +1190,11 @@
     A.idf_tab = idf_tab.as<uint2>(); A.stamp = stamp;
     A.out_like = d_likelihood; A.out_fix = lfix;
     A.dir2 = dir2.as<uint32_t>(); A.dir2_stride = dir2_stride;
-    A.n_closed_pad = (A.n_closed + 7) / 8 * 8;
+    A.gtab = grp_tab.as<GroupDev>(); A.grp_D = grp_D.as<uint32_t>(); A.grp_flags = grp_flags.as<uint32_t>();
+    A.gdir = gdir.as<uint32_t>(); A.gdir_stride = gdir_stride;
+    A.n_grouped = std::min(n_grouped, A.n_closed / TF_G);
+    A.n_units = A.n_grouped + (A.n_closed - A.n_grouped * TF_G);
+    A.n_closed_pad = (A.n_units + 7) / 8 * 8;
     *n_wgs = A.n_closed_pad + (A.n_open_slots + block / 64 - 1) / (block / 64);
     return hipSuccess;
 }
@@ -1055,9 +1206,9 @@
     TF_TRY(score_args(d_likelihood, lfix, scb, &A, &grid));
     if (grid == 0) return hipSuccess;
     if (prof_b) TF_TRY(hipEventRecord(prof_b, stream));
-    if (scb == 256) score_kernel<256><<<grid, 256, 0, stream>>>(A);
-    else if (scb == 512) score_kernel<512><<<grid, 512, 0, stream>>>(A);
-    else score_kernel<1024><<<grid, 1024, 0, stream>>>(A);
+    if (scb == 256) score_kernel<256><<<grid, 256, SCORE_LDS_BYTES, stream>>>(A);
+    else if (scb == 512) score_kernel<512><<<grid, 512, SCORE_LDS_BYTES, stream>>>(A);
+    else score_kernel<1024><<<grid, 1024, SCORE_LDS_BYTES, stream>>>(A);
     TF_TRY(hipGetLastError());
     if (prof_e) TF_TRY(hipEventRecord(prof_e, stream));
     prof_b = prof_e = nullptr;
@@ -1078,6 +1229,8 @@
     A.qd_idf = qd_idf.as<int32_t>(); A.q_meta = q_meta.as<uint32_t>();
     A.slot_ni = slot_ni.as<uint32_t>(); A.slot_begin = slot_begin.as<uint32_t>(); A.slot_cnt = slot_cnt.as<uint32_t>();
     A.idf_tab = idf_tab.as<uint2>(); A.stamp = stamp; A.out_like = nullptr; A.out_fix = nullptr;
+    A.dir2 = nullptr; A.dir2_stride = 0; A.gtab = nullptr; A.grp_D = nullptr; A.grp_flags = nullptr; A.gdir = nullptr; A.gdir_stride = 0;
+    A.n_grouped = 0; A.n_units = A.n_closed; A.n_closed_pad = 0;
     DevBuf cnt;
     TF_TRY(cnt.reserve(64, 0, stream, bytes_device));
     TF_TRY(hipMemsetAsync(cnt.p, 0, 64, stream));
@@ -1111,9 +1264,20 @@
     if (b.live == 0 && b.state == 1) {
         TF_TRY(flush_retire());
         postings_ub -= b.ub_entries;
-        pool.put(&b.coo_w); pool.put(&b.coo_pc); pool.put(&b.sealed);
+        pool.put(&b.coo_w); pool.put(&b.coo_pc); pool.put(&b.sealed); pool.put(&b.spent);
         b.W = 0; b.D_alloc = 0; b.ub_entries = 0; b.state = 2;
         TF_TRY(set_bucket(bi));
+        const int g = bi / TF_G;
+        if (TF_G > 1 && g < n_grouped && groups[g].state == 1) {
+            bool dead = true;
+            for (int m = 0; m < TF_G; ++m) dead = dead && buckets[g * TF_G + m].state == 2;
+            if (dead) {
+                groups[g].state = 2; groups[g].W = 0;
+                TF_TRY(hipStreamSynchronize(stream));
+                groups[g].buf.release(bytes_device);
+                TF_TRY(set_group(g));
+            }
+        }
     }
     return hipSuccess;
 }
```

Result: slower. 3.318 billion candidates/s (-1.0%).
